# SeanChenxy/TDRN

Hardware: AMD Instinct MI355X
Metric: frames/sec/GPU @320x320 dualrefinedet_vggbn; box Linf vs CPU ref (higher is better)
Workload: dtype bf16; 1 GPU; dualrefinedet_vggbn 320x320 multihead, bf16, batch 32 per GPU, forward + Detect(top_k 200, conf 0.01, nms 0.45), synthetic VOC-shaped frames + synthetic weights; global_batch=32, parallelism=frame-sharded x1, no per-frame collective, launch=eager, resident_batches=4, steps_in_flight=2

## Files before the change

### include/tdrn_hip.h

```cpp
#ifndef TDRN_HIP_H
#define TDRN_HIP_H

#include <stddef.h>
#include <stdint.h>

#ifdef __cplusplus
extern "C" {
#endif

#define TDRN_API __attribute__((visibility("default")))

#define TDRN_OK 0
#define TDRN_E_ARG (-1)
#define TDRN_E_SHAPE (-2)
#define TDRN_E_WORKSPACE (-3)
#define TDRN_E_UNSUPPORTED (-4)
#define TDRN_E_PARAM (-5)
#define TDRN_E_STATE (-6)
#define TDRN_E_VALUE (-7)
#define TDRN_E_DEVICE (-8)

TDRN_API const char *tdrn_version(void);
TDRN_API const char *tdrn_error_string(int code);

// ... 47 lines not shown
TDRN_API int tdrn_batch_norm_backward(const float *input, const float *grad_output, const float *weight, const float *bias,
                                      const float *save_mean, const float *save_invstd, float *grad_input, float *grad_weight,
                                      float *grad_bias, int N, int C, int H, int W, int training, int relu, float scale,
                                      void *workspace, size_t workspace_bytes, void *stream);


TDRN_API size_t tdrn_nms_workspace_bytes(int n);
TDRN_API int tdrn_nms(const float *dets, int n, double thresh, int strict_gt, int32_t *keep_out,
                      int32_t *num_out, void *workspace, size_t workspace_bytes, void *stream);

TDRN_API int tdrn_nms_topk(const float *dets, int n, float overlap, float min_score, int top_k,
                           int32_t *keep_out, int32_t *num_out, void *workspace,
                           size_t workspace_bytes, void *stream);

TDRN_API size_t tdrn_nms_topk_classes_workspace_bytes(int n, int num_classes);
TDRN_API int tdrn_nms_topk_classes(const float *boxes, const float *scores, int n, int num_classes, int first_class,
                                   float overlap, float min_score, int top_k, int32_t *keep_out, int32_t *num_out,
                                   void *workspace, size_t workspace_bytes, void *stream);

TDRN_API int tdrn_roi_resample(const float *feature, int C, int H, int W, const int32_t *cells, int n, int S, float *out,
                               void *stream);
TDRN_API int tdrn_ota_similarity(const float *boxes, const float *roi, int n, int F, const float *rows, const int32_t *row_off,
                                 int m, float *best, int32_t *arg, void *stream);

TDRN_API int tdrn_gpu_nms_host(int *keep_out, int *num_out, const float *boxes_host,
                               int boxes_num, int boxes_dim, float nms_overlap_thresh,
                               int device_id);

TDRN_API int tdrn_decode(const float *loc, const float *priors, int P, float var0, float var1,
                         float *boxes_out, void *stream);
TDRN_API int tdrn_center_size(const float *boxes, int P, float *out, void *stream);

TDRN_API int tdrn_encode(const float *matched, const float *priors, int P, float var0, float var1, float *out, void *stream);
TDRN_API size_t tdrn_match_workspace_bytes(int B, int P, int max_truths);
TDRN_API int tdrn_match(const float *truths, const int32_t *truth_off, int T_total, int max_truths, int B,
                        const float *priors, int P, const float *arm_loc, float threshold, float var0, float var1,
                        float *loc_t, int32_t *conf_t, void *workspace, size_t workspace_bytes, void *stream);
TDRN_API size_t tdrn_multibox_loss_workspace_bytes(int B, int P, int C);
TDRN_API int tdrn_multibox_loss_forward(const float *loc, const float *conf, const float *loc_t, const int32_t *conf_t,
                                        int B, int P, int C, int negpos_ratio, float *loss_out, uint8_t *sel,
                                        int32_t *num_pos, void *workspace, size_t workspace_bytes, void *stream);
TDRN_API int tdrn_multibox_loss_backward(const float *loc, const float *conf, const float *loc_t, const int32_t *conf_t,
                                         const uint8_t *sel, const int32_t *num_pos, const float *grad_loss, int B,
                                         int P, int C, float *grad_loc, float *grad_conf, void *stream);

#define TDRN_AUGMENT_MAX_TRUTHS 512
#define TDRN_AUGMENT_MAX_ROUNDS 32
#define TDRN_AUGMENT_MAX_SIZE 2048
#define TDRN_AUGMENT_CROP_FALLBACK 1
#define TDRN_AUGMENT_TAPE_EXHAUSTED 2
typedef struct {
    float brightness;
    float contrast_pre;
    float contrast_post;
    float saturation;
    float hue;
    int32_t perm[3];
    int32_t canvas_w, canvas_h, img_x, img_y;
    int32_t crop_x0, crop_y0, crop_x1, crop_y1;
    int32_t cropped;
    int32_t mirror;
    int32_t kept;
    int32_t status;
} tdrn_augment_params;
typedef struct {
    const uint8_t *data;
    int32_t h, w;
} tdrn_augment_image;
TDRN_API int tdrn_augment_sample(const int32_t *hw, const double *truths, const int32_t *truth_off, int T_total, int max_truths,
                                 int B, uint64_t seed, const int64_t *sample_ids, const double *tape, const int32_t *tape_off,
                                 tdrn_augment_params *params, float *out_truths, int32_t *out_off, void *stream);
TDRN_API int tdrn_augment_apply(const tdrn_augment_image *images, const tdrn_augment_params *params, int B, const float *mean,
                                int S, int to_rgb, float *out, void *stream);

#define TDRN_AUGMENT_TRANS_FALLBACK 4
typedef struct {
    tdrn_augment_params base;
    double shift_x, shift_y;
    int32_t trans_x, trans_y;
    int32_t attempts;
    int32_t reserved;
} tdrn_augment_pair_params;
TDRN_API int tdrn_augment_pair_sample(const int32_t *hw, const double *truths, const double *truths_t, const int32_t *truth_off,
                                      int T_total, int max_truths, int B, double max_trans_ratio, uint64_t seed,
                                      const int64_t *sample_ids, const double *tape, const int32_t *tape_off,
                                      tdrn_augment_pair_params *params, float *out_truths, float *out_truths_t,
                                      int32_t *out_off, void *stream);
TDRN_API int tdrn_augment_pair_apply(const tdrn_augment_image *images, const tdrn_augment_image *images_t,
                                     const tdrn_augment_pair_params *params, int B, const float *mean, int S, int to_rgb,
                                     float *out, float *out_t, void *stream);

TDRN_API int tdrn_prior_box(int n_maps, const int *feature_maps, double image_size,
                            const double *steps, const double *min_sizes,
                            const double *max_sizes, int n_max_sizes, const int *ar_count,
                            const double *ars, int clip, int flip, float *out_host);

TDRN_API size_t tdrn_detect_workspace_bytes(int B, int P, int C, int top_k);
TDRN_API int tdrn_detect(const float *loc, const float *conf, const float *priors,
                         const float *arm_loc, const float *scale_host, int B, int P, int C,
                         int top_k, float conf_thresh, double nms_thresh, float *out,
                         int32_t *counts_out, void *workspace, size_t workspace_bytes,
                         void *stream);
TDRN_API int tdrn_detect_dev_scale(const float *loc, const float *conf, const float *priors,
                                   const float *arm_loc, const float *scale_dev, int B, int P, int C,
                                   int top_k, float conf_thresh, double nms_thresh, float *out,
                                   int32_t *counts_out, void *workspace, size_t workspace_bytes,
                                   void *stream);

TDRN_API int tdrn_preprocess(const uint8_t *frames, int B, int H0, int W0, int S, const float mean_bgr[3],
                             int to_rgb, float *out, void *stream);
TDRN_API int tdrn_preprocess_u8(const uint8_t *frames, int B, int H0, int W0, int S, int to_rgb, uint8_t *out, void *stream);

typedef enum {
    TDRN_DRN_VGGBN = 0,
    TDRN_DRN_MOBILENET = 1,
    TDRN_SSD4SCALE_MOBILE = 2,
    TDRN_REFINEDET_VGG = 3,
    TDRN_SSD4SCALE_VGG = 4
} tdrn_model;

typedef struct {
    int model;
    int size;
    int num_classes;
    int c7_channel;
    int def_groups;
    int bn;
    int multihead;
    int deform;
    int test_phase;
    int dtype;
    int use_refine;
    int plan_flags;
    int reserved[4];
} tdrn_net_config;

#define TDRN_PLAN_NO_FUSE_FIRST 1
#define TDRN_PLAN_NO_LATE_SIDE  2
#define TDRN_PLAN_ONE_STREAM    4
#define TDRN_PLAN_NO_DEFORM_TS  8
#define TDRN_PLAN_CHAIN         16
#define TDRN_PLAN_NO_CONV_PP    32
#define TDRN_PLAN_NO_PP_SK      64
#define TDRN_PLAN_NO_CONV_PATCH 128
#define TDRN_PLAN_DWPW          512
#define TDRN_PLAN_NO_PW1X1      1024
#define TDRN_PLAN_NO_DW_SLIDE   2048
#define TDRN_PLAN_DW_SLIDE_ALL  4096
#define TDRN_PLAN_NO_CONV_WS    8192
#define TDRN_PLAN_NO_YGEMM_V2  16384
#define TDRN_PLAN_NO_HEAD3X3   32768
#define TDRN_PLAN_TS_ONE_RANGE  65536
#define TDRN_PLAN_NO_PATCH_TAIL 131072
#define TDRN_PLAN_FAULT_HANDOFF 256

typedef struct tdrn_net tdrn_net;

TDRN_API int tdrn_net_create(const tdrn_net_config *cfg, tdrn_net **out);
TDRN_API void tdrn_net_destroy(tdrn_net *net);

TDRN_API int tdrn_net_param_count(const tdrn_net *net);
TDRN_API int tdrn_net_param_info(const tdrn_net *net, int index, const char **name,
                                 int64_t shape[4], int *ndim);
TDRN_API int tdrn_net_set_param(tdrn_net *net, const char *name, const float *data_host,
                                int64_t numel);

TDRN_API size_t tdrn_net_weight_bytes(const tdrn_net *net);
TDRN_API size_t tdrn_net_workspace_bytes(const tdrn_net *net, int batch);
TDRN_API int tdrn_net_num_priors(const tdrn_net *net);

TDRN_API int tdrn_net_pack_weights(tdrn_net *net, void *weights_dev, size_t weights_bytes,
                                   void *stream);
TDRN_API int tdrn_net_adopt_weights(tdrn_net *net);

typedef struct {
    const float *x;
    int batch;
    float *arm_loc;
    float *odm_loc;
    float *conf;
    float *offsets[4];
    const float *ref_loc[4];
    float *loc_maps[4];
    void *reserved[4];
} tdrn_net_io;
typedef struct {
    const uint8_t *planes;
    float mean[3];
} tdrn_u8_frames;

TDRN_API int tdrn_net_forward(tdrn_net *net, const void *weights_dev, void *workspace,
                              size_t workspace_bytes, const tdrn_net_io *io, void *stream);

TDRN_API int tdrn_net_check(tdrn_net *net, unsigned *detail);

typedef struct {
    char name[48];
    int launches;
    double flops;
    double bytes;
    double ms;
} tdrn_kernel_stat;
TDRN_API int tdrn_net_profile(tdrn_net *net, int enable);
TDRN_API int tdrn_net_kernel_stats(tdrn_net *net, tdrn_kernel_stat *out, int max_entries);
TDRN_API int tdrn_net_op_stats(tdrn_net *net, tdrn_kernel_stat *out, int max_entries);
TDRN_API int tdrn_net_op_timeline(tdrn_net *net, float *start_ms, float *end_ms, int *lane, int max_entries);

typedef struct {
    int kind;
    int in, out, res;
    int pool;
    int off, y;
    int k, stride, pad, dil, relu, ceil_mode, splitk, groups;
    int out_kind;
    int level;
    int n_branches, k2, pad2, off_c0[2];
    int y_tap_major;
    int fused_first;
    int fused_dw;
    char w[48], b[48], bn[48], w2[48], b2[48];
    int y_groups;
} tdrn_op_info;
TDRN_API int tdrn_net_op_count(const tdrn_net *net);
TDRN_API int tdrn_net_op_info(const tdrn_net *net, int index, tdrn_op_info *out);

TDRN_API int tdrn_net_tensor_count(const tdrn_net *net);
TDRN_API int tdrn_net_tensor_info(const tdrn_net *net, int index, const char **label, int *C, int *H,
                                  int *W);
TDRN_API int tdrn_net_read_tensor(const tdrn_net *net, const void *workspace, int batch, int index,
                                  float *out_dev, void *stream);
TDRN_API int tdrn_net_write_tensor(const tdrn_net *net, void *workspace, int batch, int index,
                                   const float *in_dev, void *stream);
TDRN_API int tdrn_net_forward_from(tdrn_net *net, const void *weights_dev, void *workspace,
                                   size_t workspace_bytes, const tdrn_net_io *io, int first_op, void *stream);

#ifdef __cplusplus
}
#endif
#endif
```

### tdrn_amd/_lib.py

```python
import ctypes as C
import os

_HERE = os.path.dirname(os.path.abspath(__file__))
LIB_PATH = os.environ.get("TDRN_LIB_PATH") or os.path.join(_HERE, "lib", "libtdrn_hip.so")

F32, BF16, F16 = 0, 1, 2
DTYPES = {"fp32": F32, "f32": F32, "float32": F32, "bf16": BF16, "bfloat16": BF16, "fp16": F16,
          "f16": F16, "float16": F16, "half": F16}
DRN_VGGBN, DRN_MOBILENET, SSD4SCALE_MOBILE, REFINEDET_VGG, SSD4SCALE_VGG = range(5)

E_VALUE = -7


class TdrnError(RuntimeError):
    def __init__(self, code, what=""):
        self.code = code
        super().__init__("%s (tdrn error %d)%s" % (error_string(code), code,
                                                    (": " + what) if what else ""))


class NetConfig(C.Structure):
    _fields_ = [("model", C.c_int), ("size", C.c_int), ("num_classes", C.c_int),
                ("c7_channel", C.c_int), ("def_groups", C.c_int), ("bn", C.c_int),
                ("multihead", C.c_int), ("deform", C.c_int), ("test_phase", C.c_int),
                ("dtype", C.c_int), ("use_refine", C.c_int), ("plan_flags", C.c_int), ("reserved", C.c_int * 4)]


PLAN_NO_FUSE_FIRST, PLAN_NO_LATE_SIDE, PLAN_ONE_STREAM, PLAN_NO_DEFORM_TS, PLAN_CHAIN = 1, 2, 4, 8, 16
PLAN_NO_CONV_PP, PLAN_NO_PP_SK, PLAN_NO_CONV_PATCH, PLAN_FAULT_HANDOFF, PLAN_DWPW, PLAN_NO_PW1X1 = 32, 64, 128, 256, 512, 1024
PLAN_NO_DW_SLIDE, PLAN_DW_SLIDE_ALL, PLAN_NO_CONV_WS, PLAN_NO_YGEMM_V2, PLAN_NO_HEAD3X3, PLAN_TS_ONE_RANGE = 2048, 4096, 8192, 16384, 32768, 65536
PLAN_NO_PATCH_TAIL = 131072
E_DEVICE = -8


class NetIO(C.Structure):
    _fields_ = [("x", C.c_void_p), ("batch", C.c_int), ("arm_loc", C.c_void_p),
                ("odm_loc", C.c_void_p), ("conf", C.c_void_p), ("offsets", C.c_void_p * 4),
                ("ref_loc", C.c_void_p * 4), ("loc_maps", C.c_void_p * 4),
                ("reserved", C.c_void_p * 4)]


class KernelStat(C.Structure):
    _fields_ = [("name", C.c_char * 48), ("launches", C.c_int), ("flops", C.c_double),
                ("bytes", C.c_double), ("ms", C.c_double)]


class U8FramesABI(C.Structure):
    _fields_ = [("planes", C.c_void_p), ("mean", C.c_float * 3)]


class OpInfo(C.Structure):
    _fields_ = [("kind", C.c_int), ("in_", C.c_int), ("out", C.c_int), ("res", C.c_int), ("pool", C.c_int), ("off", C.c_int),
                ("y", C.c_int), ("k", C.c_int), ("stride", C.c_int), ("pad", C.c_int), ("dil", C.c_int), ("relu", C.c_int),
                ("ceil_mode", C.c_int), ("splitk", C.c_int), ("groups", C.c_int), ("out_kind", C.c_int), ("level", C.c_int),
                ("n_branches", C.c_int), ("k2", C.c_int), ("pad2", C.c_int), ("off_c0", C.c_int * 2), ("y_tap_major", C.c_int),
                ("fused_first", C.c_int), ("fused_dw", C.c_int), ("w", C.c_char * 48), ("b", C.c_char * 48), ("bn", C.c_char * 48), ("w2", C.c_char * 48),
                ("b2", C.c_char * 48), ("y_groups", C.c_int)]


class AugmentParams(C.Structure):
    _fields_ = [("brightness", C.c_float), ("contrast_pre", C.c_float), ("contrast_post", C.c_float), ("saturation", C.c_float),
                ("hue", C.c_float), ("perm", C.c_int32 * 3), ("canvas_w", C.c_int32), ("canvas_h", C.c_int32),
                ("img_x", C.c_int32), ("img_y", C.c_int32), ("crop_x0", C.c_int32), ("crop_y0", C.c_int32),
                ("crop_x1", C.c_int32), ("crop_y1", C.c_int32), ("cropped", C.c_int32), ("mirror", C.c_int32),
                ("kept", C.c_int32), ("status", C.c_int32)]


class AugmentImage(C.Structure):
    _fields_ = [("data", C.c_void_p), ("h", C.c_int32), ("w", C.c_int32)]


class AugmentPairParams(C.Structure):
    _fields_ = [("base", AugmentParams), ("shift_x", C.c_double), ("shift_y", C.c_double), ("trans_x", C.c_int32),
                ("trans_y", C.c_int32), ("attempts", C.c_int32), ("reserved", C.c_int32)]


AUGMENT_MAX_TRUTHS, AUGMENT_MAX_SIZE = 512, 2048
AUGMENT_CROP_FALLBACK, AUGMENT_TAPE_EXHAUSTED, AUGMENT_TRANS_FALLBACK = 1, 2, 4

OP_KINDS = ("first_conv", "conv", "conv_transpose", "depthwise", "maxpool", "l2norm", "offset_conv", "deform_heads", "other")

_lib = None

_SIGS = {
    "tdrn_version": (C.c_char_p, []),
    "tdrn_error_string": (C.c_char_p, [C.c_int]),
    "tdrn_deform_conv_workspace_bytes": (C.c_size_t, [C.c_int] * 15),
    "tdrn_deform_conv_forward": (C.c_int, [C.c_void_p] * 4 + [C.c_int] * 15 + [C.c_void_p, C.c_size_t, C.c_void_p]),
    "tdrn_deform_conv_backward_workspace_bytes": (C.c_size_t, [C.c_int] * 14),
    "tdrn_deform_conv_backward_input": (C.c_int, [C.c_void_p] * 6 + [C.c_int] * 14 + [C.c_void_p, C.c_size_t, C.c_void_p]),
    "tdrn_deform_conv_backward_parameters": (C.c_int, [C.c_void_p] * 4 + [C.c_int] * 14 + [C.c_float, C.c_void_p, C.c_size_t,
                                                                                            C.c_void_p]),
    "tdrn_conv2d_workspace_bytes": (C.c_size_t, [C.c_int] * 14),
    "tdrn_conv2d_forward": (C.c_int, [C.c_void_p] * 4 + [C.c_int] * 14 + [C.c_void_p, C.c_size_t, C.c_void_p]),
    "tdrn_conv2d_backward_input": (C.c_int, [C.c_void_p] * 3 + [C.c_int] * 14 + [C.c_void_p, C.c_size_t, C.c_void_p]),
    "tdrn_conv2d_backward_parameters": (C.c_int, [C.c_void_p] * 4 + [C.c_int] * 13 + [C.c_float, C.c_int, C.c_void_p, C.c_size_t,
                                                                                       C.c_void_p]),
    "tdrn_batch_norm_workspace_bytes": (C.c_size_t, [C.c_int] * 4),
    "tdrn_batch_norm_forward": (C.c_int, [C.c_void_p] * 8 + [C.c_int] * 5 + [C.c_float, C.c_float, C.c_int, C.c_void_p, C.c_size_t,
                                                                             C.c_void_p]),
    "tdrn_batch_norm_backward": (C.c_int, [C.c_void_p] * 9 + [C.c_int] * 6 + [C.c_float, C.c_void_p, C.c_size_t, C.c_void_p]),
    "tdrn_nms_workspace_bytes": (C.c_size_t, [C.c_int]),
    "tdrn_nms": (C.c_int, [C.c_void_p, C.c_int, C.c_double, C.c_int, C.c_void_p, C.c_void_p,
                           C.c_void_p, C.c_size_t, C.c_void_p]),
    "tdrn_nms_topk": (C.c_int, [C.c_void_p, C.c_int, C.c_float, C.c_float, C.c_int, C.c_void_p, C.c_void_p,
                                C.c_void_p, C.c_size_t, C.c_void_p]),
    "tdrn_gpu_nms_host": (C.c_int, [C.c_void_p, C.c_void_p, C.c_void_p, C.c_int, C.c_int, C.c_float, C.c_int]),
    "tdrn_decode": (C.c_int, [C.c_void_p, C.c_void_p, C.c_int, C.c_float, C.c_float, C.c_void_p, C.c_void_p]),
    "tdrn_center_size": (C.c_int, [C.c_void_p, C.c_int, C.c_void_p, C.c_void_p]),
    "tdrn_encode": (C.c_int, [C.c_void_p, C.c_void_p, C.c_int, C.c_float, C.c_float, C.c_void_p, C.c_void_p]),
    "tdrn_match_workspace_bytes": (C.c_size_t, [C.c_int] * 3),
    "tdrn_match": (C.c_int, [C.c_void_p, C.c_void_p, C.c_int, C.c_int, C.c_int, C.c_void_p, C.c_int, C.c_void_p, C.c_float,
                             C.c_float, C.c_float, C.c_void_p, C.c_void_p, C.c_void_p, C.c_size_t, C.c_void_p]),
    "tdrn_multibox_loss_workspace_bytes": (C.c_size_t, [C.c_int] * 3),
    "tdrn_multibox_loss_forward": (C.c_int, [C.c_void_p] * 4 + [C.c_int] * 4 + [C.c_void_p] * 4 + [C.c_size_t, C.c_void_p]),
    "tdrn_multibox_loss_backward": (C.c_int, [C.c_void_p] * 7 + [C.c_int] * 3 + [C.c_void_p] * 3),
    "tdrn_augment_sample": (C.c_int, [C.c_void_p] * 3 + [C.c_int] * 3 + [C.c_uint64] + [C.c_void_p] * 7),
    "tdrn_augment_apply": (C.c_int, [C.c_void_p, C.c_void_p, C.c_int, C.c_void_p, C.c_int, C.c_int, C.c_void_p, C.c_void_p]),
    "tdrn_augment_pair_sample": (C.c_int, [C.c_void_p] * 4 + [C.c_int] * 3 + [C.c_double, C.c_uint64] + [C.c_void_p] * 8),
    "tdrn_augment_pair_apply": (C.c_int, [C.c_void_p] * 3 + [C.c_int, C.c_void_p, C.c_int, C.c_int] + [C.c_void_p] * 3),
    "tdrn_prior_box": (C.c_int, [C.c_int, C.c_void_p, C.c_double, C.c_void_p, C.c_void_p, C.c_void_p,
                                 C.c_int, C.c_void_p, C.c_void_p, C.c_int, C.c_int, C.c_void_p]),
    "tdrn_nms_topk_classes_workspace_bytes": (C.c_size_t, [C.c_int, C.c_int]),
    "tdrn_nms_topk_classes": (C.c_int, [C.c_void_p, C.c_void_p, C.c_int, C.c_int, C.c_int, C.c_float, C.c_float, C.c_int, C.c_void_p,
                                        C.c_void_p, C.c_void_p, C.c_size_t, C.c_void_p]),
    "tdrn_roi_resample": (C.c_int, [C.c_void_p, C.c_int, C.c_int, C.c_int, C.c_void_p, C.c_int, C.c_int, C.c_void_p, C.c_void_p]),
    "tdrn_ota_similarity": (C.c_int, [C.c_void_p, C.c_void_p, C.c_int, C.c_int, C.c_void_p, C.c_void_p, C.c_int, C.c_void_p, C.c_void_p,
                                      C.c_void_p]),
    "tdrn_preprocess": (C.c_int, [C.c_void_p, C.c_int, C.c_int, C.c_int, C.c_int, C.c_void_p, C.c_int, C.c_void_p, C.c_void_p]),
    "tdrn_preprocess_u8": (C.c_int, [C.c_void_p, C.c_int, C.c_int, C.c_int, C.c_int, C.c_int, C.c_void_p, C.c_void_p]),
    "tdrn_detect_workspace_bytes": (C.c_size_t, [C.c_int] * 4),
    "tdrn_detect": (C.c_int, [C.c_void_p] * 5 + [C.c_int] * 4 + [C.c_float, C.c_double, C.c_void_p,
                                                                  C.c_void_p, C.c_void_p, C.c_size_t, C.c_void_p]),
    "tdrn_detect_dev_scale": (C.c_int, [C.c_void_p] * 5 + [C.c_int] * 4 + [C.c_float, C.c_double, C.c_void_p,
                                                                            C.c_void_p, C.c_void_p, C.c_size_t, C.c_void_p]),
    "tdrn_net_create": (C.c_int, [C.POINTER(NetConfig), C.POINTER(C.c_void_p)]),
    "tdrn_net_destroy": (None, [C.c_void_p]),
    "tdrn_net_param_count": (C.c_int, [C.c_void_p]),
    "tdrn_net_param_info": (C.c_int, [C.c_void_p, C.c_int, C.POINTER(C.c_char_p), C.POINTER(C.c_int64 * 4),
                                      C.POINTER(C.c_int)]),
    "tdrn_net_set_param": (C.c_int, [C.c_void_p, C.c_char_p, C.c_void_p, C.c_int64]),
    "tdrn_net_weight_bytes": (C.c_size_t, [C.c_void_p]),
    "tdrn_net_workspace_bytes": (C.c_size_t, [C.c_void_p, C.c_int]),
    "tdrn_net_num_priors": (C.c_int, [C.c_void_p]),
    "tdrn_net_pack_weights": (C.c_int, [C.c_void_p, C.c_void_p, C.c_size_t, C.c_void_p]),
    "tdrn_net_adopt_weights": (C.c_int, [C.c_void_p]),
    "tdrn_net_forward": (C.c_int, [C.c_void_p, C.c_void_p, C.c_void_p, C.c_size_t, C.POINTER(NetIO), C.c_void_p]),
    "tdrn_net_check": (C.c_int, [C.c_void_p, C.POINTER(C.c_uint)]),
    "tdrn_net_op_count": (C.c_int, [C.c_void_p]),
    "tdrn_net_op_info": (C.c_int, [C.c_void_p, C.c_int, C.POINTER(OpInfo)]),
    "tdrn_net_tensor_count": (C.c_int, [C.c_void_p]),
    "tdrn_net_tensor_info": (C.c_int, [C.c_void_p, C.c_int, C.POINTER(C.c_char_p), C.POINTER(C.c_int),
                                       C.POINTER(C.c_int), C.POINTER(C.c_int)]),
    "tdrn_net_read_tensor": (C.c_int, [C.c_void_p, C.c_void_p, C.c_int, C.c_int, C.c_void_p, C.c_void_p]),
    "tdrn_net_write_tensor": (C.c_int, [C.c_void_p, C.c_void_p, C.c_int, C.c_int, C.c_void_p, C.c_void_p]),
    "tdrn_net_forward_from": (C.c_int, [C.c_void_p, C.c_void_p, C.c_void_p, C.c_size_t, C.POINTER(NetIO), C.c_int, C.c_void_p]),
    "tdrn_net_profile": (C.c_int, [C.c_void_p, C.c_int]),
    "tdrn_net_kernel_stats": (C.c_int, [C.c_void_p, C.POINTER(KernelStat), C.c_int]),
    "tdrn_net_op_stats": (C.c_int, [C.c_void_p, C.POINTER(KernelStat), C.c_int]),
    "tdrn_net_op_timeline": (C.c_int, [C.c_void_p, C.POINTER(C.c_float), C.POINTER(C.c_float), C.POINTER(C.c_int), C.c_int]),
}
EXPORTS = tuple(_SIGS)


def lib():
    global _lib
    if _lib is None:
        if not os.path.exists(LIB_PATH):
            raise ImportError(
                "libtdrn_hip.so is missing (%s): build it with `python -c 'import __graft_entry__ as g; "
                "g.build()'` or `make -C tdrn_amd/csrc`.  tdrn_amd has no CPU fallback." % LIB_PATH)
        try:
            import torch
            if torch.cuda.is_available():
                torch.cuda.init()
        except ImportError:
            pass
        l = C.CDLL(LIB_PATH)
        for name, (res, args) in _SIGS.items():
            fn = getattr(l, name)
            fn.restype = res
            fn.argtypes = args
        _lib = l
    return _lib


def error_string(code):
    try:
        return lib().tdrn_error_string(int(code)).decode()
    except Exception:
        return "tdrn error"


def check(rc, what=""):
    if rc != 0:
        if rc == E_VALUE:
            raise ValueError("nms_threshold must be non negative.")
        raise TdrnError(rc, what)


def ptr(t):
    return None if t is None else C.c_void_p(t.data_ptr())


def aligned16(t):
    return t if t is None or t.data_ptr() % 16 == 0 else t.clone()


def current_stream(device=None):
    import torch
    return C.c_void_p(torch.cuda.current_stream(device).cuda_stream)


def require_cuda(t, name="tensor"):
    if not t.is_cuda:
        raise NotImplementedError(
            "%s must live on the GPU: tdrn_amd runs only through libtdrn_hip.so on an MI355X "
            "(no CPU path; the reference's ConvOffset2dFunction raises here too, "
            "model/networks.py:632-633)" % name)
```

### tdrn_amd/csrc/common.h

```cpp
#pragma once
#include <hip/hip_runtime.h>
#include <stdint.h>

#include "../../include/tdrn_hip.h"

#include <cstdlib>

namespace tdrn {

inline int dev_ablate_env(const char *name)
{
#ifdef TDRN_DEV_ABLATE
    const char *e = getenv(name);
    return e ? atoi(e) : 0;
#else
    (void)name;
    return 0;
#endif
}

typedef __attribute__((ext_vector_type(4))) float f32x4;
typedef __attribute__((ext_vector_type(16))) float f32x16;
typedef __attribute__((ext_vector_type(8))) short i16x8;
typedef __attribute__((ext_vector_type(8))) _Float16 f16x8;
typedef __attribute__((ext_vector_type(4))) int i32x4;
typedef __attribute__((ext_vector_type(4))) unsigned u32x4;

struct bf16_t { unsigned short v; };
struct f16_t { unsigned short v; };

template <typename T> struct elem_traits;
template <> struct elem_traits<float> { static constexpr int bytes = 4; static constexpr int per16 = 4; };
template <> struct elem_traits<bf16_t> { static constexpr int bytes = 2; static constexpr int per16 = 8; };
template <> struct elem_traits<f16_t> { static constexpr int bytes = 2; static constexpr int per16 = 8; };

__device__ __forceinline__ float bf16_to_f32(unsigned short h) { return __uint_as_float(((unsigned)h) << 16); }
__device__ __forceinline__ unsigned short f32_to_bf16(float f)
{
    __bf16 b = (__bf16)f;
    return __builtin_bit_cast(unsigned short, b);
}
__device__ __forceinline__ float f16_to_f32(unsigned short h) { return (float)__builtin_bit_cast(_Float16, h); }
__device__ __forceinline__ unsigned short f32_to_f16(float f) { return __builtin_bit_cast(unsigned short, (_Float16)f); }

template <typename T> __device__ __forceinline__ float to_f32(const T &);
template <> __device__ __forceinline__ float to_f32<float>(const float &x) { return x; }
template <> __device__ __forceinline__ float to_f32<bf16_t>(const bf16_t &x) { return bf16_to_f32(x.v); }
template <> __device__ __forceinline__ float to_f32<f16_t>(const f16_t &x) { return f16_to_f32(x.v); }
template <typename T> __device__ __forceinline__ T from_f32(float);
template <> __device__ __forceinline__ float from_f32<float>(float x) { return x; }
template <> __device__ __forceinline__ bf16_t from_f32<bf16_t>(float x) { return bf16_t{f32_to_bf16(x)}; }
template <> __device__ __forceinline__ f16_t from_f32<f16_t>(float x) { return f16_t{f32_to_f16(x)}; }

template <typename T> __device__ __forceinline__ void unpack16(const u32x4 &raw, float *out);
template <> __device__ __forceinline__ void unpack16<float>(const u32x4 &raw, float *out)
{
#pragma unroll
    for (int i = 0; i < 4; ++i) out[i] = __uint_as_float(raw[i]);
}
template <> __device__ __forceinline__ void unpack16<bf16_t>(const u32x4 &raw, float *out)
{
#pragma unroll
    for (int i = 0; i < 4; ++i) {
        out[2 * i] = __uint_as_float(raw[i] << 16);
        out[2 * i + 1] = __uint_as_float(raw[i] & 0xffff0000u);
    }
}
template <> __device__ __forceinline__ void unpack16<f16_t>(const u32x4 &raw, float *out)
{
#pragma unroll
    for (int i = 0; i < 4; ++i) {
        out[2 * i] = f16_to_f32((unsigned short)(raw[i] & 0xffffu));
        out[2 * i + 1] = f16_to_f32((unsigned short)(raw[i] >> 16));
    }
}
template <typename T> __device__ __forceinline__ u32x4 pack16(const float *in);
template <> __device__ __forceinline__ u32x4 pack16<float>(const float *in)
{
    u32x4 r;
#pragma unroll
    for (int i = 0; i < 4; ++i) r[i] = __float_as_uint(in[i]);
    return r;
}
__device__ __forceinline__ unsigned pack2_bf16(float a, float b)
{
    typedef __bf16 bf2 __attribute__((ext_vector_type(2)));
    typedef float fl2 __attribute__((ext_vector_type(2)));
    return __builtin_bit_cast(unsigned, __builtin_convertvector(fl2{a, b}, bf2));
}
__device__ __forceinline__ unsigned pack2_f16(float a, float b)
{
    typedef _Float16 h2 __attribute__((ext_vector_type(2)));
    typedef float fl2 __attribute__((ext_vector_type(2)));
    return __builtin_bit_cast(unsigned, __builtin_convertvector(fl2{a, b}, h2));
}
template <typename T> __device__ __forceinline__ unsigned pack2(float a, float b);
template <> __device__ __forceinline__ unsigned pack2<bf16_t>(float a, float b) { return pack2_bf16(a, b); }
template <> __device__ __forceinline__ unsigned pack2<f16_t>(float a, float b) { return pack2_f16(a, b); }
template <> __device__ __forceinline__ u32x4 pack16<bf16_t>(const float *in)
{
    u32x4 r;
#pragma unroll
    for (int i = 0; i < 4; ++i) r[i] = pack2_bf16(in[2 * i], in[2 * i + 1]);
    return r;
}
template <> __device__ __forceinline__ u32x4 pack16<f16_t>(const float *in)
{
    u32x4 r;
#pragma unroll
    for (int i = 0; i < 4; ++i) r[i] = pack2_f16(in[2 * i], in[2 * i + 1]);
    return r;
}

inline int hip_status(hipError_t e) { return e == hipSuccess ? TDRN_OK : (int)e; }
#define TDRN_HIP_TRY(expr)                                   \
    do {                                                     \
        hipError_t _e = (expr);                              \
        if (_e != hipSuccess) return (int)_e;                \
    } while (0)
#define TDRN_TRY(expr)                                       \
    do {                                                     \
        int _s = (expr);                                     \
        if (_s != TDRN_OK) return _s;                        \
    } while (0)

inline size_t align_up(size_t v, size_t a) { return (v + a - 1) / a * a; }
inline int cdiv(int a, int b) { return (a + b - 1) / b; }
inline int dtype_bytes(int dt) { return dt == TDRN_F32 ? 4 : 2; }

unsigned short host_f32_to_bf16(float f);
unsigned short host_f32_to_f16(float f);

}
```

### tdrn_amd/csrc/deform.hip

```cpp
#include <algorithm>

#include "deform_sampler.h"
#include "kernels.h"
#include "mfma_prims.h"

namespace tdrn {

struct DeformBranchP {
    const float *off;
    const char *w;
    int off_stride, kh, kw, G;
    int pad_h, pad_w, stride_h, stride_w, dil_h, dil_w;
    int off_rows, off_row0;
};
struct DeformParams {
    const char *in, *zero;
    DeformBranchP br[2];
    int n_branches;
    int M, H, W, Cin, Ho, Wo, Cout, Npad, split;
    float *out0, *out1;
    long long o0_bs, o0_ps, o1_bs, o1_ps;
    int accumulate;
    int g_begin, g_end;
};
// ... 171 lines not shown
    auto compute = [&](int buf) {
        const char *wsb = smem + buf * STAGE;
        const char *psb = wsb + BN * 128;
#pragma unroll
        for (int kk = 0; kk < 4; ++kk) {
            const int ch = ((2 * kk + hh) ^ sw) << 4;
            const u32x4 pf = *(const u32x4 *)(psb + (wave * 32 + r32) * 128 + ch);
#pragma unroll
            for (int ci = 0; ci < NTL; ++ci) {
                const u32x4 wf = *(const u32x4 *)(wsb + (ci * 32 + r32) * 128 + ch);
                Mma32<DT>::run(wf, pf, acc[ci]);
            }
        }
    };

    fetch_offsets(0, 0, 0, p.g_begin);
    tap_params();
    issue(0);
    latch_weights();
    finish(0);
    asm volatile("s_waitcnt vmcnt(0)" ::: "memory");
    __syncthreads();
    int cur = 0;
    bool more = true;
    while (more) {
        more = advance();
        if (more) {
            issue(cur ^ 1);
            latch_weights();
        }
        compute(cur);
        if (more) finish(cur ^ 1);
        asm volatile("s_waitcnt vmcnt(0)" ::: "memory");
        __syncthreads();
        cur ^= 1;
    }

#pragma unroll
    for (int ci = 0; ci < NTL; ++ci)
#pragma unroll
        for (int q = 0; q < 4; ++q) {
            f32x4 v;
#pragma unroll
            for (int j = 0; j < 4; ++j) v[j] = acc[ci][4 * q + j];
            *(f32x4 *)(smem + (wave * 32 + r32) * CS + (ci * 32 + 8 * q + 4 * hh) * 4) = v;
        }
    __syncthreads();
    for (int idx = t; idx < BM * p.Cout; idx += NT) {
        const int row = idx / p.Cout, c = idx - row * p.Cout;
        const int m = m0 + row;
        if (m >= p.M) break;
        const int b = m / HoWo, pix = m - b * HoWo;
        const float v = *(const float *)(smem + row * CS + c * 4);
        float *dst = c < p.split ? p.out0 + b * p.o0_bs + pix * p.o0_ps + c : p.out1 + b * p.o1_bs + pix * p.o1_ps + (c - p.split);
        if (p.accumulate) atomicAdd(dst, v);
        else *dst = v;
    }
}

int deform_n_pad(int cout) { return (int)align_up((size_t)cout, 32); }

template <typename DT> static int launch_deform_dt(const DeformMulti &mp, int ntl, hipStream_t s)
{
    dim3 grid((unsigned)(8 * ((mp.block_start[mp.n] + 7) / 8)));
    switch (ntl) {
        case 1: hipLaunchKernelGGL((deform_gemm_kernel<DT, 1>), grid, dim3(256), 0, s, mp); break;
        case 2: hipLaunchKernelGGL((deform_gemm_kernel<DT, 2>), grid, dim3(256), 0, s, mp); break;
        case 3: hipLaunchKernelGGL((deform_gemm_kernel<DT, 3>), grid, dim3(256), 0, s, mp); break;
        case 4: hipLaunchKernelGGL((deform_gemm_kernel<DT, 4>), grid, dim3(256), 0, s, mp); break;
        default: return TDRN_E_UNSUPPORTED;
    }
    return hip_status(hipGetLastError());
}

static int fill_params(const DeformArgs &a, DeformParams &p)
{
    if (!a.in || !a.out0 || a.n_branches < 1 || a.n_branches > 2) return TDRN_E_ARG;
    const int es = dtype_bytes(a.dtype), ck = 128 / es;
    if (a.Npad % 32 || a.Npad > 128 || a.Cout > a.Npad || a.Cout < 1) return TDRN_E_UNSUPPORTED;
    if (a.split < a.Cout && !a.out1) return TDRN_E_ARG;
    if ((long long)a.B * a.H * a.W * a.Cin * es >= (1ll << 32)) return TDRN_E_UNSUPPORTED;
    p.in = (const char *)a.in;
    p.zero = (const char *)a.zero_page;
    p.n_branches = a.n_branches;
    for (int i = 0; i < a.n_branches; ++i) {
        const DeformBranch &b = a.br[i];
        if (!b.off || !b.w || b.G < 1 || a.Cin % b.G || (a.Cin / b.G) % ck) return TDRN_E_UNSUPPORTED;
        if (b.kh < 1 || b.kw < 1 || b.stride < 1 || b.dil < 1) return TDRN_E_SHAPE;
        p.br[i] = DeformBranchP{b.off, (const char *)b.w, b.off_stride, b.kh, b.kw, b.G,
                                b.pad, b.pad_w < 0 ? b.pad : b.pad_w, b.stride, b.stride_w < 1 ? b.stride : b.stride_w,
                                b.dil, b.dil_w < 1 ? b.dil : b.dil_w, b.off_rows, b.off_row0};
        if (b.off_rows < 0 || b.off_row0 < 0) return TDRN_E_ARG;
    }
    if (a.n_branches == 1) p.br[1] = p.br[0];
    p.M = a.B * a.Ho * a.Wo;
    p.H = a.H; p.W = a.W; p.Cin = a.Cin; p.Ho = a.Ho; p.Wo = a.Wo; p.Cout = a.Cout; p.Npad = a.Npad;
    p.split = a.split > a.Cout ? a.Cout : a.split;
    p.out0 = a.out0; p.out1 = a.out1;
    p.o0_bs = a.o0_bs; p.o0_ps = a.o0_ps; p.o1_bs = a.o1_bs; p.o1_ps = a.o1_ps;
    return TDRN_OK;
}

int launch_deform_multi(const DeformArgs *args, int n, hipStream_t s, int split_branches)
{
    if (!args || n < 1 || n > 4) return TDRN_E_ARG;
    DeformMulti mp;
    mp.n = 0;
    mp.block_start[0] = 0;
    for (int pass = 0; pass < 2; ++pass) {
        for (int i = 0; i < n; ++i) {
            if (args[i].dtype != args[0].dtype || args[i].Npad != args[0].Npad) return TDRN_E_UNSUPPORTED;
            DeformArgs a = args[i];
            const bool two = a.n_branches == 2 && split_branches == 1;
            const bool halves = split_branches == 2 && a.n_branches == 1 && a.br[0].G >= 2 && a.br[0].G % 2 == 0;
            if (!two && !halves && pass == 1) continue;
            if (two) {
                const int t0 = a.br[0].kh * a.br[0].kw, t1 = a.br[1].kh * a.br[1].kw;
                const int longer = t1 > t0 ? 1 : 0;
                a.br[0] = args[i].br[pass == 0 ? longer : 1 - longer];
                a.n_branches = 1;
            }
            DeformParams p;
            TDRN_TRY(fill_params(a, p));
            p.accumulate = (two || halves) ? 1 : 0;
            p.g_begin = 0;
            p.g_end = a.br[0].G;
            if (halves) {
                p.g_begin = pass == 0 ? 0 : a.br[0].G / 2;
                p.g_end = pass == 0 ? a.br[0].G / 2 : a.br[0].G;
            }
            if (p.M <= 0) continue;
            if (mp.n >= kMaxDeformProblems) return TDRN_E_UNSUPPORTED;
            mp.p[mp.n] = p;
            mp.block_start[mp.n + 1] = mp.block_start[mp.n] + cdiv(p.M, 128);
            ++mp.n;
        }
    }
    if (mp.n == 0) return TDRN_OK;
    for (int i = mp.n; i < kMaxDeformProblems; ++i) { mp.p[i] = mp.p[0]; mp.block_start[i + 1] = mp.block_start[mp.n]; }
    switch (args[0].dtype) {
        case TDRN_F32: return launch_deform_dt<float>(mp, args[0].Npad / 32, s);
        case TDRN_BF16: return launch_deform_dt<bf16_t>(mp, args[0].Npad / 32, s);
        case TDRN_F16: return launch_deform_dt<f16_t>(mp, args[0].Npad / 32, s);
    }
    return TDRN_E_ARG;
}

int launch_deform(const DeformArgs &a, hipStream_t s) { return launch_deform_multi(&a, 1, s, 0); }

struct SampleBranchP {
    const float *off;
    int off_stride, kh, kw, pad_h, pad_w, dil_h, dil_w, col0;
    int off_rows, off_row0;
};
struct SampleParams {
    const char *y;
    SampleBranchP br[2];
    int n_branches, n_taps;
    int M, H, W, ycs, Cout, split;
    int tap_major;
    float *out0, *out1;
    long long o0_bs, o0_ps, o1_bs, o1_ps;
};
struct SampleMulti {
    SampleParams p[4];
    int block_start[5];
    int n;
};
constexpr int kSampleCols = 80;

template <typename DT>
__global__ __launch_bounds__(256) void deform_sample_kernel(const SampleMulti mp)
{
    const int nblk = (int)gridDim.x, xq = nblk >> 3, xr = nblk & 7, xcd = (int)blockIdx.x & 7;
    const int blk = (xcd < xr ? xcd * (xq + 1) : xr * (xq + 1) + (xcd - xr) * xq) + ((int)blockIdx.x >> 3);
    int prob = 0;
#pragma unroll
    for (int i = 1; i < 4; ++i)
        if (i < mp.n && blk >= mp.block_start[i]) prob = i;
    const SampleParams &p = mp.p[prob];
    constexpr int MAXR = 34 * 4;
    __shared__ uint2 s_ow[4][MAXR + 8];
    __shared__ float s_red[4][6][kSampleCols];
    const int lane = threadIdx.x & 63, wave = threadIdx.x >> 6;
    const int m = (blk - mp.block_start[prob]) * 4 + wave;
    if (m >= p.M) return;
    const int HW = p.H * p.W;
    const int b = m / HW, rem = m - b * HW, ho = rem / p.W, wo = rem - ho * p.W;
    const int nrows = p.n_taps * 4;
    if (lane < p.n_taps) {
        const int brn = (p.n_branches == 2 && lane >= p.br[0].kh * p.br[0].kw) ? 1 : 0;
        const SampleBranchP &B = p.br[brn];
        const int tl = lane - (brn ? p.br[0].kh * p.br[0].kw : 0);
        const int ti = tl / B.kw, tj = tl - ti * B.kw;
        const int orow = B.off_rows ? (m + B.off_row0) % B.off_rows : m;
        const float *op = B.off + (size_t)orow * B.off_stride + 2 * tl;
        const float offset_h = op[0], offset_w = op[1];
        float w1 = 0.f, w2 = 0.f, w3 = 0.f, w4 = 0.f;
        int q1 = 0, q2 = 0, q3 = 0, q4 = 0;
        const int h_in = ho - B.pad_h, w_in = wo - B.pad_w;
        const float h_im = (float)(h_in + ti * B.dil_h) + offset_h;
        const float w_im = (float)(w_in + tj * B.dil_w) + offset_w;
        if (h_im >= 0.f && w_im >= 0.f && h_im < (float)p.H && w_im < (float)p.W) {
            float h = (float)(ti * B.dil_h) + offset_h;
            float w = (float)(tj * B.dil_w) + offset_w;
            const int height = p.H - h_in, width = p.W - w_in;
            int h_low = (int)floorf(h), w_low = (int)floorf(w), h_high, w_high;
            if (h_low >= height - 1) { h_high = h_low = height - 1; h = (float)h_low; } else { h_high = h_low + 1; }
            if (w_low >= width - 1) { w_high = w_low = width - 1; w = (float)w_low; } else { w_high = w_low + 1; }
            const float lh = h - (float)h_low, lw = w - (float)w_low;
            const float hh = 1.f - lh, hw = 1.f - lw;
            w1 = hh * hw; w2 = hh * lw; w3 = lh * hw; w4 = lh * lw;
            const int r0 = min(max(h_in + h_low, 0), p.H - 1), r1 = min(max(h_in + h_high, 0), p.H - 1);
            const int c0 = min(max(w_in + w_low, 0), p.W - 1), c1 = min(max(w_in + w_high, 0), p.W - 1);
            q1 = r0 * p.W + c0; q2 = r0 * p.W + c1; q3 = r1 * p.W + c0; q4 = r1 * p.W + c1;
        }
        const unsigned colb = p.tap_major ? (unsigned)(B.col0 + tl) * (unsigned)p.M * (unsigned)(kSampleCols * 2) : (unsigned)(deform_y_col(B.col0 + tl) * 2);
        const unsigned rowb = p.tap_major ? (unsigned)(kSampleCols * 2) : (unsigned)(p.ycs * 2);
        const unsigned img = (unsigned)(b * HW);
        s_ow[wave][4 * lane + 0] = make_uint2((img + q1) * rowb + colb, __float_as_uint(w1));
        s_ow[wave][4 * lane + 1] = make_uint2((img + q2) * rowb + colb, __float_as_uint(w2));
        s_ow[wave][4 * lane + 2] = make_uint2((img + q3) * rowb + colb, __float_as_uint(w3));
        s_ow[wave][4 * lane + 3] = make_uint2((img + q4) * rowb + colb, __float_as_uint(w4));
        if (lane == p.n_taps - 1)
            for (int r = nrows; r < 36 * ((nrows + 35) / 36); ++r) s_ow[wave][r] = make_uint2((img + q4) * rowb + colb, 0u);
    }
    __builtin_amdgcn_s_waitcnt(0xC07F);
    __builtin_amdgcn_wave_barrier();
    const int j = lane / 10, c = lane - 10 * j;
    float acc[8] = {0.f, 0.f, 0.f, 0.f, 0.f, 0.f, 0.f, 0.f};
    if (lane < 60) {
        const int nb = (nrows + 35) / 36;
        const __attribute__((address_space(1))) char *yb = (const __attribute__((address_space(1))) char *)p.y;
        for (int ib = 0; ib < nb; ++ib) {
            u32x4 raw[6];
            float wgt[6];
#pragma unroll
            for (int u = 0; u < 6; ++u) {
                const uint2 ow = s_ow[wave][6 * (6 * ib + u) + j];
                wgt[u] = __uint_as_float(ow.y);
                raw[u] = *(const __attribute__((address_space(1))) u32x4 *)(yb + (ow.x + (unsigned)(c * 16)));
            }
#pragma unroll
            for (int u = 0; u < 6; ++u) {
                float v[8];
                unpack16<DT>(raw[u], v);
#pragma unroll
                for (int e = 0; e < 8; ++e) acc[e] = fmaf(wgt[u], v[e], acc[e]);
            }
        }
#pragma unroll
        for (int e = 0; e < 8; ++e) s_red[wave][j][c * 8 + e] = acc[e];
    }
    __builtin_amdgcn_s_waitcnt(0xC07F);
    __builtin_amdgcn_wave_barrier();
    for (int co = lane; co < p.Cout; co += 64) {
        float v = s_red[wave][0][co];
#pragma unroll
        for (int jj = 1; jj < 6; ++jj) v += s_red[wave][jj][co];
        float *dst = co < p.split ? p.out0 + b * p.o0_bs + rem * p.o0_ps + co : p.out1 + b * p.o1_bs + rem * p.o1_ps + (co - p.split);
        *dst = v;
    }
}

struct YGemmParams {
    const char *x;
    const char *w;
    char *y;
    int M, N, ycs, parts, tiles_per_part, taps;
};

struct YGemmMulti {
    YGemmParams p[4];
    int block_start[5];
    int n;
#ifdef TDRN_YG_STAMP
    unsigned *stamps;
#endif
};
#ifdef TDRN_YG_STAMP
#define YG_STAMP_DECL unsigned long long st_t = __builtin_amdgcn_s_memtime(); unsigned st_acc[6] = {0, 0, 0, 0, 0, 0};
#define YG_STAMP(k) do { const unsigned long long t_ = __builtin_amdgcn_s_memtime(); st_acc[k] += (unsigned)(t_ - st_t); st_t = t_; } while (0)
#define YG_STAMP_FLUSH do { st_acc[5] = (unsigned)nt; if (lane == 0) for (int k_ = 0; k_ < 6; ++k_) mp.stamps[((size_t)blockIdx.x * 8 + wave) * 6 + k_] = st_acc[k_]; } while (0)
#else
#define YG_STAMP_DECL
#define YG_STAMP(k) do { } while (0)
#define YG_STAMP_FLUSH do { } while (0)
#endif

template <typename DT>
__global__ __launch_bounds__(512, 4) void ygemm_k256_kernel(const YGemmMulti mp)
{
    int prob = 0;
#pragma unroll
    for (int i = 1; i < 4; ++i)
        if (i < mp.n && (int)blockIdx.x >= mp.block_start[i]) prob = i;
    const YGemmParams &p = mp.p[prob];
    const int local_blk = (int)blockIdx.x - mp.block_start[prob];
    const int ncg = p.N / 256;
    constexpr int NW = 8;
    constexpr int NT = NW * 64;
    constexpr int TP = 32;
    constexpr int TBYTES = TP * 512;
    constexpr int SROW = 512 + 16;
    constexpr int PPW = 16 / NW;
    __shared__ __attribute__((aligned(16))) char smem[2 * TBYTES];
    __shared__ __attribute__((aligned(16))) char sst[TP * SROW];
    const int lane = threadIdx.x & 63, wave = __builtin_amdgcn_readfirstlane(threadIdx.x >> 6);
    const int r32 = lane & 31, hh = lane >> 5;
    const int part = local_blk / ncg, cg = local_blk - part * ncg;
    const int col0 = cg * 256 + wave * 32;
    u32x4 wf[16];
    {
        const char *wr = p.w + ((size_t)(col0 + r32) * 256 + 8 * hh) * 2;
#pragma unroll
        for (int kk = 0; kk < 16; ++kk) wf[kk] = *(const u32x4 *)(wr + kk * 32);
    }
    const int t0 = part * p.tiles_per_part;
    int nt = (p.M + TP - 1) / TP - t0;
    nt = nt < p.tiles_per_part ? nt : p.tiles_per_part;
    if (nt <= 0) return;
    YG_STAMP_DECL

    const unsigned smem_lds = lds_addr(smem);
    auto stage = [&](int t, int buf) {
        const long long mb = (long long)(t0 + t) * TP;
        const char *sb = p.x + (size_t)mb * 512;
#pragma unroll
        for (int j = 0; j < PPW; ++j) {
            const int piece = PPW * wave + j;
            const int row = 2 * piece + (lane >> 5), cpos = lane & 31;
            int r = row;
            if (mb + r >= p.M) r = (int)(p.M - 1 - mb);
            const unsigned voff = (unsigned)(r * 512 + ((cpos ^ (row & 31)) << 4));
            lds_dma16(sb, voff, __builtin_amdgcn_readfirstlane(smem_lds + buf * TBYTES + piece * 1024));
        }
    };
    stage(0, 0);
    YG_STAMP(0);
    constexpr int NSTR = 32 * 32 / NT;
    int nst_prev = NSTR;
    if (p.taps > 0) {
        nst_prev = 0;
        for (int it = wave; it < 18; it += NW) nst_prev += (cg * 3 + it / 6) < p.taps ? 1 : 0;
    }
    for (int t = 0; t < nt; ++t) {
        const int buf = t & 1;
        if (t + 1 < nt) {
            stage(t + 1, buf ^ 1);
            switch ((t == 0 ? 0 : nst_prev) + PPW) {
                case 2: asm volatile("s_waitcnt vmcnt(2)" ::: "memory"); break;
                case 3: asm volatile("s_waitcnt vmcnt(3)" ::: "memory"); break;
                case 4: asm volatile("s_waitcnt vmcnt(4)" ::: "memory"); break;
                case 5: asm volatile("s_waitcnt vmcnt(5)" ::: "memory"); break;
                case 6: asm volatile("s_waitcnt vmcnt(6)" ::: "memory"); break;
                case 7: asm volatile("s_waitcnt vmcnt(7)" ::: "memory"); break;
                case 8: asm volatile("s_waitcnt vmcnt(8)" ::: "memory"); break;
                default: asm volatile("s_waitcnt vmcnt(9)" ::: "memory"); break;
            }
        } else {
            asm volatile("s_waitcnt vmcnt(0)" ::: "memory");
        }
        YG_STAMP(1);
        __builtin_amdgcn_s_barrier();
        asm volatile("" ::: "memory");
        YG_STAMP(2);
        f32x16 acc;
#pragma unroll
        for (int e = 0; e < 16; ++e) acc[e] = 0.f;
        const char *ab = smem + buf * TBYTES + r32 * 512;
#pragma unroll
        for (int kk = 0; kk < 16; ++kk) {
            const u32x4 a = *(const u32x4 *)(ab + (((2 * kk + hh) ^ r32) << 4));
            Mma32<DT>::run(wf[kk], a, acc);
        }
        {
            const unsigned sa = (unsigned)(unsigned long long)(__attribute__((address_space(3))) char *)sst + (unsigned)(r32 * SROW + (wave * 32 + 4 * hh) * 2);
#pragma unroll
            for (int g = 0; g < 4; ++g) {
                const uint2 v = make_uint2(pack2<DT>(acc[4 * g], acc[4 * g + 1]), pack2<DT>(acc[4 * g + 2], acc[4 * g + 3]));
                asm volatile("ds_write_b64 %0, %1 offset:%2" ::"v"(sa), "v"(v), "n"(16 * g) : "memory");
            }
        }
        asm volatile("s_waitcnt lgkmcnt(0)" ::: "memory");
        __builtin_amdgcn_s_waitcnt(0xC07F);
        YG_STAMP(3);
        __builtin_amdgcn_s_barrier();
        asm volatile("" ::: "memory");
        YG_STAMP(2);
        if (p.taps > 0) {
            const int px = lane / 10, k = lane - 10 * px;
            for (int it = wave; it < 18; it += NW) {
                const int sgi = it / 6, pg = it - sgi * 6;
                const int tap = cg * 3 + sgi;
                const int row = pg * 6 + px;
                const long long m = (long long)(t0 + t) * TP + row;
                if (lane < 60 && row < TP && tap < p.taps && m < p.M)
                    *(u32x4 *)(p.y + ((size_t)tap * p.M + (size_t)m) * 160 + k * 16) = *(const u32x4 *)(sst + row * SROW + (sgi * 10 + k) * 16);
            }
        } else {
#pragma unroll
            for (int q = 0; q < NSTR; ++q) {
                const int row = (threadIdx.x >> 5) + (NT / 32) * q, ch = threadIdx.x & 31;
                const long long m = (long long)(t0 + t) * TP + row;
                if (m < p.M) *(u32x4 *)(p.y + ((size_t)m * p.ycs + cg * 256) * 2 + ch * 16) = *(const u32x4 *)(sst + row * SROW + ch * 16);
            }
        }
        YG_STAMP(4);
    }
    YG_STAMP_FLUSH;
}

template <typename DT>
__global__ __launch_bounds__(512, 4) void ygemm_k256_v2_kernel(const YGemmMulti mp)
// ... 101 lines not shown
            if (kk == 5 || kk == 10 || kk == 15) carry_store((kk - 5) / 5, rows_prev, sv);
            __builtin_amdgcn_sched_barrier(0);
        }
        {
            const unsigned sa = (unsigned)(unsigned long long)(__attribute__((address_space(3))) char *)sst + (unsigned)(buf * SBYTES) + sw;
#pragma unroll
            for (int g = 0; g < 4; ++g) {
                const uint2 v = make_uint2(pack2<DT>(acc[4 * g], acc[4 * g + 1]), pack2<DT>(acc[4 * g + 2], acc[4 * g + 3]));
                asm volatile("ds_write_b64 %0, %1 offset:%2" ::"v"(sa), "v"(v), "n"(16 * g) : "memory");
            }
        }
        YG_STAMP(3);
        if (t + 1 < nt) {
            switch (t > 0 ? nst : 0) {
                case 0: asm volatile("s_waitcnt vmcnt(0) lgkmcnt(0)" ::: "memory"); break;
                case 1: asm volatile("s_waitcnt vmcnt(1) lgkmcnt(0)" ::: "memory"); break;
                case 2: asm volatile("s_waitcnt vmcnt(2) lgkmcnt(0)" ::: "memory"); break;
                default: asm volatile("s_waitcnt vmcnt(3) lgkmcnt(0)" ::: "memory"); break;
            }
        } else {
            asm volatile("s_waitcnt lgkmcnt(0)" ::: "memory");
        }
        YG_STAMP(4);
        __builtin_amdgcn_s_barrier();
        asm volatile("" ::: "memory");
        YG_STAMP(2);
    }
    {
        const int left = p.M - (t0 + nt - 1) * TP;
        const int rows = left < TP ? left : TP;
#pragma unroll
        for (int j = 0; j < 3; ++j) {
            const u32x4 v = carry_read(j, (nt - 1) & 1);
            carry_store(j, rows, v);
        }
    }
    YG_STAMP_FLUSH;
}

int ygemm_supported(int Cin, int ycols, int dtype) { return dtype != TDRN_F32 && Cin == 256 && ycols % 256 == 0; }

static int ygemm_fill(const YGemmProblem &q, int dtype, YGemmParams &p, int &blocks)
{
    if (!ygemm_supported(256, q.N, dtype) || q.M <= 0 || q.M >= (1ll << 31)) return TDRN_E_UNSUPPORTED;
    p.x = (const char *)q.x; p.w = (const char *)q.w; p.y = (char *)q.y;
    p.M = (int)q.M; p.N = q.N; p.ycs = q.ycs; p.taps = q.taps;
    if (q.taps > 0 && (deform_sample_cols(q.taps) > q.N || (long long)q.taps * q.M * 160 >= (1ll << 32))) return TDRN_E_UNSUPPORTED;
    const int tiles = (int)((q.M + 31) / 32), cgs = q.N / 256;
    const int kSlots = 512, max_parts = (tiles + 7) / 8 > 1 ? (tiles + 7) / 8 : 1;
    int parts = 1;
    long long best = -1;
    for (int r = 1; r <= 3; ++r) {
        int c = kSlots * r / cgs;
        c = c > max_parts ? max_parts : (c < 1 ? 1 : c);
        const long long rounds = ((long long)cgs * c + kSlots - 1) / kSlots, cost = rounds * ((tiles + c - 1) / c);
        if (best < 0 || cost < best) { best = cost; parts = c; }
    }
    p.parts = parts;
    p.tiles_per_part = (tiles + parts - 1) / parts;
    blocks = cgs * parts;
    return TDRN_OK;
}

int launch_ygemm_multi(const YGemmProblem *pr, int n, int dtype, hipStream_t s, int kdisable)
{
    if (!pr || n < 1 || n > 4) return TDRN_E_ARG;
    YGemmMulti mp;
    mp.n = 0;
    mp.block_start[0] = 0;
    int order[4] = {0, 1, 2, 3};
    for (int i = 0; i < n; ++i)
        for (int j = i + 1; j < n; ++j)
            if (pr[order[j]].M > pr[order[i]].M) { const int t = order[i]; order[i] = order[j]; order[j] = t; }
    for (int i = 0; i < n; ++i) {
        if (pr[order[i]].M <= 0) continue;
        int blocks = 0;
        TDRN_TRY(ygemm_fill(pr[order[i]], dtype, mp.p[mp.n], blocks));
        mp.block_start[mp.n + 1] = mp.block_start[mp.n] + blocks;
        ++mp.n;
    }
    if (mp.n == 0) return TDRN_OK;
    for (int i = mp.n; i < 4; ++i) { mp.p[i] = mp.p[0]; mp.block_start[i + 1] = mp.block_start[mp.n]; }
    dim3 grid((unsigned)mp.block_start[mp.n]);
#ifdef TDRN_YG_STAMP
    static unsigned *stamps = nullptr;
    static int calls = 0;
    const size_t nst = (size_t)grid.x * 8 * 6;
    if (!stamps) TDRN_HIP_TRY(hipMalloc((void **)&stamps, 4096 * 8 * 6 * sizeof(unsigned)));
    TDRN_HIP_TRY(hipMemsetAsync(stamps, 0, nst * sizeof(unsigned), s));
    mp.stamps = stamps;
    struct Report {
        hipStream_t s; size_t n; unsigned *d; YGemmMulti &mp; int *calls;
        ~Report() {
            if (++*calls != 5) return;
            (void)hipStreamSynchronize(s);
            std::vector<unsigned> h(n);
            (void)hipMemcpy(h.data(), d, n * sizeof(unsigned), hipMemcpyDeviceToHost);
            for (int pr = 0; pr < mp.n; ++pr) {
                double a[5] = {0, 0, 0, 0, 0}, tiles = 0, waves = 0;
                for (int b = mp.block_start[pr]; b < mp.block_start[pr + 1]; ++b)
                    for (int w = 0; w < 8; ++w) {
                        const unsigned *q = &h[((size_t)b * 8 + w) * 6];
                        if (!q[5]) continue;
                        for (int k = 0; k < 5; ++k) a[k] += q[k];
                        tiles += q[5]; waves += 1;
                    }
                if (waves == 0) continue;
                fprintf(stderr, "yg_stamp problem %d M %d blocks %d tiles/wg %.1f | per wave: prologue %.0f | per tile: landing %.0f barriers %.0f mma+stage %.0f stores %.0f (ticks of s_memtime)\n",
                        pr, mp.p[pr].M, mp.block_start[pr + 1] - mp.block_start[pr], tiles / waves, a[0] / waves, a[1] / tiles, a[2] / tiles, a[3] / tiles, a[4] / tiles);
            }
        }
    } report{s, nst, stamps, mp, &calls};
#endif
    bool tapmajor = true;
    for (int i = 0; i < mp.n; ++i) tapmajor = tapmajor && mp.p[i].taps > 0;
    if (!(kdisable & KOFF_YGEMM_V2) && tapmajor) {
        if (dtype == TDRN_BF16) hipLaunchKernelGGL((ygemm_k256_v2_kernel<bf16_t>), grid, dim3(512), 0, s, mp);
        else hipLaunchKernelGGL((ygemm_k256_v2_kernel<f16_t>), grid, dim3(512), 0, s, mp);
    } else {
        if (dtype == TDRN_BF16) hipLaunchKernelGGL((ygemm_k256_kernel<bf16_t>), grid, dim3(512), 0, s, mp);
        else hipLaunchKernelGGL((ygemm_k256_kernel<f16_t>), grid, dim3(512), 0, s, mp);
    }
    return hip_status(hipGetLastError());
}

int launch_ygemm(const void *x, const void *w, void *y, long long M, int N, int ycs, int dtype, hipStream_t s, int taps)
{
    const YGemmProblem q{x, w, y, M, N, ycs, taps};
    return launch_ygemm_multi(&q, 1, dtype, s);
}

int deform_sample_supported(const DeformArgs &a)
{
    if (a.dtype == TDRN_F32 || a.n_branches < 1 || a.n_branches > 2 || a.Cout > kSampleCols || a.Ho != a.H || a.Wo != a.W) return 0;
    int taps = 0;
    for (int i = 0; i < a.n_branches; ++i) {
        const DeformBranch &b = a.br[i];
        if (b.G != 1 || b.stride != 1 || (b.stride_w >= 1 && b.stride_w != 1)) return 0;
        taps += b.kh * b.kw;
    }
    return taps <= 34 ? taps : 0;
}
int deform_sample_cols(int taps) { return ((taps + 2) / 3) * 256; }
int deform_ts_max_batch(int H, int W, int ycs, int taps)
{
    const long long hw = (long long)H * W;
    const long long per = std::max((long long)taps * 160, (long long)ycs * 2) * hw;
    long long b = ((1ll << 32) - 1) / per;
    const long long bm = ((1ll << 31) - 1) / hw;
    b = b < bm ? b : bm;
    return (int)(b > (1 << 20) ? (1 << 20) : b);
}

int launch_deform_sample_multi(const DeformArgs *args, const void *const *y, const int *ycs, int n, hipStream_t s, int tap_major)
{
    if (!args || n < 1 || n > 4) return TDRN_E_ARG;
    SampleMulti mp;
    mp.n = 0;
    mp.block_start[0] = 0;
    for (int i = 0; i < n; ++i) {
        const DeformArgs &a = args[i];
        const int taps = deform_sample_supported(a);
        if (!taps || a.dtype != args[0].dtype) return TDRN_E_UNSUPPORTED;
        if ((long long)a.B * a.H * a.W * ycs[i] * 2 >= (1ll << 32)) return TDRN_E_UNSUPPORTED;
        SampleParams p;
        p.y = (const char *)y[i];
        p.n_branches = a.n_branches; p.n_taps = taps;
        int col0 = 0;
        for (int k = 0; k < a.n_branches; ++k) {
            const DeformBranch &b = a.br[k];
            p.br[k] = SampleBranchP{b.off, b.off_stride, b.kh, b.kw, b.pad, b.pad_w < 0 ? b.pad : b.pad_w, b.dil, b.dil_w < 1 ? b.dil : b.dil_w, col0, b.off_rows, b.off_row0};
            col0 += b.kh * b.kw;
        }
        if (a.n_branches == 1) p.br[1] = p.br[0];
        p.M = a.B * a.H * a.W; p.H = a.H; p.W = a.W; p.ycs = ycs[i]; p.Cout = a.Cout; p.tap_major = tap_major;
        p.split = a.split > a.Cout ? a.Cout : a.split;
        p.out0 = a.out0; p.out1 = a.out1;
        p.o0_bs = a.o0_bs; p.o0_ps = a.o0_ps; p.o1_bs = a.o1_bs; p.o1_ps = a.o1_ps;
        if (p.M <= 0) continue;
        mp.p[mp.n] = p;
        mp.block_start[mp.n + 1] = mp.block_start[mp.n] + cdiv(p.M, 4);
        ++mp.n;
    }
    if (mp.n == 0) return TDRN_OK;
    for (int i = mp.n; i < 4; ++i) { mp.p[i] = mp.p[0]; mp.block_start[i + 1] = mp.block_start[mp.n]; }
    dim3 grid((unsigned)mp.block_start[mp.n]);
    if (args[0].dtype == TDRN_BF16) hipLaunchKernelGGL((deform_sample_kernel<bf16_t>), grid, dim3(256), 0, s, mp);
    else hipLaunchKernelGGL((deform_sample_kernel<f16_t>), grid, dim3(256), 0, s, mp);
    return hip_status(hipGetLastError());
}

}
```

### tdrn_amd/csrc/kernels.h

```cpp
#pragma once
#include <cmath>

#include "common.h"

namespace tdrn {

constexpr size_t kZeroPageBytes = 256;

int allow_big_lds(const void *kernel);

enum KernelOff {
    KOFF_CONV_PP = 1,
    KOFF_PP_SK = 2,
    KOFF_CONV_PATCH = 4,
    KOFF_PW1X1 = 8,
    KOFF_DW_SLIDE = 16,
    KOFF_DW_STRIP_SMALL = 32,
    KOFF_CONV_WS = 64,
    KOFF_YGEMM_V2 = 128,
    KOFF_HEAD3X3 = 256,
    KOFF_TS_RANGES = 512,
    KOFF_PATCH_TAIL = 1024,
};

struct ConvArgs {
    const void *in = nullptr, *w = nullptr, *res = nullptr, *zero_page = nullptr;
    const float *bias = nullptr;
    void *out = nullptr;
    int B = 0, H = 0, W = 0, Cin = 0;
    int Ho = 0, Wo = 0, Cout = 0, Npad = 0;
    int kh = 1, kw = 1, stride = 1, pad = 0, dil = 1;
    int relu = 0, out_f32 = 0, phases = 1;
    int splitk = 1;
    void *partial = nullptr;
    long long o_bs = 0, o_rs = 0, o_cs = 0, o_base = 0, o_pr = 0, o_pc = 0;
    int dtype = TDRN_BF16;
    const float *fuse_x = nullptr, *fuse_w = nullptr, *fuse_b = nullptr;
    int fuse_cout = 0;
    const unsigned char *fuse_x8 = nullptr;
    float fuse_mean[3] = {0.f, 0.f, 0.f};
    void *sk_ws = nullptr;
    bool sk_flags_zero = false;
    int kdisable = 0;
    unsigned *status = nullptr;
    int fault_handoff = 0;
};
enum ConvKernel { CONV_IGEMM, CONV_PATCH, CONV_PP, CONV_WS, CONV_HEAD3X3, CONV_PW1X1, CONV_NONE };
ConvKernel conv_route(const ConvArgs &a, bool pooled);
const char *conv_kernel_name(ConvKernel k);
int launch_conv(const ConvArgs &a, hipStream_t s, void *out_pool = nullptr);
int conv_splitk_choice(const ConvArgs &a);
int launch_conv_igemm(const ConvArgs &a, hipStream_t s);
int igemm_splitk_choice(const ConvArgs &a);
size_t conv_splitk_bytes(const ConvArgs &a, int splits);
struct ChainLayer { ConvArgs a; int dep[2] = {-1, -1}; };
int conv_chain_supported(const ConvArgs &a);
int conv_chain_max_layers();
size_t conv_chain_ctr_bytes();
int launch_conv_chain(const ChainLayer *layers, int n, unsigned *ctr, hipStream_t s, unsigned *status = nullptr);
bool head3x3_takes(const ConvArgs &a, bool pooled);
int launch_head3x3(const ConvArgs &a, hipStream_t s);
inline int conv3x3_tile_mode(const ConvArgs &a, int slots)
{
    if (a.kh != 3 || a.kw != 3 || a.stride != 1 || a.pad != 1 || a.dil != 1 || a.phases != 1 || a.out_f32 || a.res) return 0;
    if (a.Ho != a.H || a.Wo != a.W || a.Npad % 64) return 0;
    if (a.o_rs != (long long)a.Wo * a.o_cs || a.o_bs != (long long)a.Ho * a.Wo * a.o_cs || a.o_base) return 0;
    if (a.W % 32 == 0 && a.H % 8 == 0) return 32;
    if (a.W % 16 == 0 && a.H % 16 == 0) return 16;
    return 2 * a.W + 2 + 256 <= slots * 8 ? -1 : 0;
}
inline bool conv3x3_input_fits(const ConvArgs &a) { return a.fuse_x || (long long)a.B * a.H * a.W * a.Cin * dtype_bytes(a.dtype) < (1ll << 32); }
bool patch_takes(const ConvArgs &a, bool pooled);
int launch_conv3x3_patch(const ConvArgs &a, void *out_pool, hipStream_t s);
bool pp_takes_geometry(const ConvArgs &a);
bool pp_takes(const ConvArgs &a, bool pooled);
int launch_conv3x3_pp(const ConvArgs &a, hipStream_t s);
size_t conv_pp_sk_bytes();
bool ws_takes(const ConvArgs &a, bool pooled);
int launch_conv3x3_ws(const ConvArgs &a, void *out_pool, hipStream_t s);
inline int persistent_grid(int items) { return items >= 256 ? 256 : ((items + 7) / 8) * 8; }
inline void conv_tiles(int B, int H, int W, int tw, int px, int &tiles_x, int &tiles_per_img, int &m_tiles)
{
    tiles_x = tw ? W / tw : 0;
    tiles_per_img = tw ? tiles_x * (H / (px / tw)) : 0;
    m_tiles = tw ? B * tiles_per_img : cdiv(B * H * W, 256);
}
int conv_n_pad(int cout);
constexpr int kChanPad = 64;

int launch_first_conv(const float *x, const float *w, const float *bias, void *out, int B, int S,
                      int stride, int Cout, int Cpad, int relu, int dtype, hipStream_t s);
int launch_maxpool2(const void *in, void *out, int B, int H, int W, int C, int ceil_mode, int dtype,
                    hipStream_t s);
int launch_l2norm(const void *in, const float *w, void *out, long long pixels, int C, int dtype,
                  hipStream_t s);
int launch_dwconv3(const void *in, const float *w, const float *bias, void *out, int B, int H, int W,
                   int C, int stride, int relu, int dtype, hipStream_t s, int kdisable = 0);
struct DwPwArgs {
    const void *in = nullptr, *w = nullptr;
    const float *wdw = nullptr, *bdw = nullptr, *bias = nullptr;
    void *out = nullptr;
    int B = 0, H = 0, W = 0, Cin = 0, Cout = 0, Npad = 0, Cs = 0;
    int stride = 1, relu_dw = 1, relu = 1, dtype = TDRN_BF16;
};
int dwpw_supported(const DwPwArgs &a);
int launch_dwpw(const DwPwArgs &a, hipStream_t s);
bool pw1x1_takes(const ConvArgs &a, bool pooled);
int launch_pw1x1(const ConvArgs &a, hipStream_t s);
int launch_softmax_rows(const float *in, float *out, long long R, int C, hipStream_t s);
int launch_offset_conv(const float *loc, long long loc_bs, long long loc_ps, const float *w,
                       const float *bias, float *off, int B, int HW, int n_in, int n_out,
                       hipStream_t s);
struct OffsetProblem { const float *loc; long long loc_bs, loc_ps; const float *w, *bias; float *off; int B, HW, n_out, blk0; };
struct OffsetMulti { OffsetProblem pr[4]; int n; };
int launch_offset_conv_multi(const OffsetProblem *pr, int n, hipStream_t s);
int launch_nchw_to_nhwc(const float *in, void *out, int B, int C, int HW, int Cpad, int dtype,
                        hipStream_t s);
int launch_nchw_to_nhwc_grouped(const float *in, void *out, int B, int C, int HW, int G, int cpg_pad, int dtype,
                                hipStream_t s);
int launch_repack_oihw(const float *w, void *out, int Cout, int Npad, int Cin, int taps, int G, int cpg_pad, int dtype,
                       hipStream_t s);
int launch_nhwc_to_nchw_f32(const float *in, long long in_bs, long long in_ps, float *out, int B,
                            int C, int HW, hipStream_t s);
int launch_nhwc_any_to_nchw_f32(const void *in, int dtype, int Cpad, float *out, int B, int C, int HW, hipStream_t s);
int launch_preprocess(const unsigned char *in, int B, int H0, int W0, int S, const float *mean_bgr, int to_rgb, float *out,
                      hipStream_t s);
int launch_preprocess_u8(const unsigned char *in, int B, int H0, int W0, int S, int to_rgb, unsigned char *out, hipStream_t s);
int launch_u8_planes_to_f32(const unsigned char *in, int B, int S, const float *mean, float *out, hipStream_t s);
int launch_fill_zero(void *p, size_t bytes, hipStream_t s);

struct DeformBranch {
    const float *off = nullptr;
    int off_stride = 0;
    const void *w = nullptr;
    int kh = 3, kw = 3, pad = 1, stride = 1, dil = 1, G = 1;
    int pad_w = -1, stride_w = -1, dil_w = -1;
    int off_rows = 0, off_row0 = 0;
};
struct DeformArgs {
    const void *in = nullptr, *zero_page = nullptr;
    DeformBranch br[2];
    int n_branches = 1;
    int B = 0, H = 0, W = 0, Cin = 0, Ho = 0, Wo = 0, Cout = 0, Npad = 0;
    float *out0 = nullptr, *out1 = nullptr;
    int split = 0;
    long long o0_bs = 0, o0_ps = 0, o1_bs = 0, o1_ps = 0;
    int dtype = TDRN_BF16;
};
int launch_deform(const DeformArgs &a, hipStream_t s);
int launch_deform_multi(const DeformArgs *args, int n, hipStream_t s, int split_branches);
int deform_n_pad(int cout);
struct DeformBwdGeom { int N, Cin, H, W, Cout, kh, kw, sh, sw, ph, pw, dh, dw, G, Ho, Wo; };
int deform_bwd_cpg64(const DeformBwdGeom &g);
int deform_bwd_data_px(const DeformBwdGeom &g);
int launch_deform_bwd_data(const DeformBwdGeom &g, const float *in_nhwc, const float *off, const float *gout, const float *wr,
                           float *gin_nhwc, float *goff, hipStream_t s);
int launch_deform_bwd_input_add(const DeformBwdGeom &g, const float *gin_nhwc, float *grad_input, hipStream_t s);
void deform_bwd_weight_splits(const DeformBwdGeom &g, int &splits, int &per_split);
int launch_deform_bwd_weight(const DeformBwdGeom &g, const float *in_nhwc, const float *off, const float *gout, float *slab, float *grad_weight,
                             float scale, hipStream_t s);
struct ConvBwdGeom { int N, Cin, H, W, Cout, k, pad, dil, Ho, Wo; };
int conv_bwd_cpad(int c);
void conv_wgrad_splits(const ConvBwdGeom &g, int &splits, int &per_split);
size_t conv_wgrad_slab_bytes(const ConvBwdGeom &g);
int launch_conv_wgrad(const ConvBwdGeom &g, const void *x_nhwc, const void *go_nhwc, const void *zero_page, void *slab, float *grad_weight,
                      float *grad_bias, float scale, int dtype, hipStream_t s);
int launch_repack_oihw_dgrad(const float *w, void *out, int Cout, int Cin, int Npad, int taps, int dtype, hipStream_t s);
void batch_norm_splits(int N, int C, int HW, int &splits, int &per_split);
size_t batch_norm_workspace_bytes(int N, int C, int HW);
int launch_batch_norm_forward(const float *input, const float *weight, const float *bias, float *running_mean, float *running_var,
                              float *output, float *save_mean, float *save_invstd, int N, int C, int HW, int training, float momentum,
                              float eps, int relu, void *ws, hipStream_t s);
int launch_batch_norm_backward(const float *input, const float *grad_output, const float *weight, const float *bias, const float *save_mean,
                               const float *save_invstd, float *grad_input, float *grad_weight, float *grad_bias, int N, int C, int HW,
                               int training, int relu, float scale, void *ws, hipStream_t s);
int deform_sample_supported(const DeformArgs &a);
int deform_sample_cols(int taps);
constexpr int deform_y_col(int tap) { return (tap / 3) * 256 + (tap % 3) * 80; }
int deform_ts_max_batch(int H, int W, int ycs, int taps);
int launch_deform_sample_multi(const DeformArgs *args, const void *const *y, const int *ycs, int n, hipStream_t s, int tap_major = 0);
int ygemm_supported(int Cin, int ycols, int dtype);
int launch_ygemm(const void *x, const void *w, void *y, long long M, int N, int ycs, int dtype, hipStream_t s, int taps = 0);
struct YGemmProblem { const void *x, *w; void *y; long long M; int N, ycs, taps; };
int launch_ygemm_multi(const YGemmProblem *pr, int n, int dtype, hipStream_t s, int kdisable = 0);

int launch_decode(const float *loc, const float *priors, int P, float v0, float v1, float *out,
                  hipStream_t s);
int launch_center_size(const float *boxes, int P, float *out, hipStream_t s);
size_t detect_workspace_bytes(int B, int P, int C, int top_k);
int launch_detect(const float *loc, const float *conf, const float *priors, const float *arm_loc,
                  const float *scale4, int scale_on_device, int B, int P, int C, int top_k, float conf_thresh,
                  double nms_thresh, float *out, int32_t *counts, void *ws, size_t ws_bytes,
                  hipStream_t s);
size_t nms_workspace_bytes(int n);
size_t nms_classes_workspace_bytes(int n, int C);
int launch_roi_resample(const float *feat, int C, int H, int W, const int32_t *cells, int n, int S, float *out, hipStream_t s);
int launch_ota_similarity(const float *boxes, const float *roi, int n, int F, const float *rows, const int32_t *row_off, int m, float *best,
                          int32_t *arg, hipStream_t s);
int launch_nms_classes(const float *boxes, const float *scores, int n, int C, int first_class, float overlap, float min_score, int top_k,
                       int32_t *keep_out, int32_t *num_out, void *ws, size_t ws_bytes, hipStream_t s);
int launch_nms(const float *dets, int n, double thresh, int strict_gt, int presorted,
               int32_t *keep_out, int32_t *num_out, void *ws, size_t ws_bytes, hipStream_t s,
               int plain_rule = 0, float min_score = -INFINITY, int pre_top_k = 0);

constexpr int kMaxMatchTruths = 512;
constexpr int kMaxLossClasses = 1024;
size_t match_workspace_bytes(int B, int P, int max_truths);
int launch_match(const float *truths, const int32_t *truth_off, int T_total, int max_truths, int B, const float *priors, int P,
                 const float *arm_loc, float threshold, float var0, float var1, float *loc_t, int32_t *conf_t, void *ws,
                 size_t ws_bytes, hipStream_t s);
int launch_encode(const float *matched, const float *priors, int P, float v0, float v1, float *out, hipStream_t s);
size_t multibox_loss_workspace_bytes(int B, int P, int C);
int launch_multibox_loss_forward(const float *loc, const float *conf, const float *loc_t, const int32_t *conf_t, int B, int P,
                                 int C, int negpos_ratio, float *loss_out, uint8_t *sel, int32_t *num_pos, void *ws,
                                 size_t ws_bytes, hipStream_t s);
int launch_multibox_loss_backward(const float *loc, const float *conf, const float *loc_t, const int32_t *conf_t,
                                  const uint8_t *sel, const int32_t *num_pos, const float *grad_loss, int B, int P, int C,
                                  float *grad_loc, float *grad_conf, hipStream_t s);

int launch_augment_sample(const int32_t *hw, const double *truths, const int32_t *truth_off, int T_total, int max_truths, int B,
                          uint64_t seed, const int64_t *sample_ids, const double *tape, const int32_t *tape_off,
                          tdrn_augment_params *params, float *out_truths, int32_t *out_off, hipStream_t s);
int launch_augment_apply(const tdrn_augment_image *images, const tdrn_augment_params *params, int B, const float *mean, int S,
                         int to_rgb, float *out, hipStream_t s);

int launch_augment_pair_sample(const int32_t *hw, const double *truths, const double *truths_t, const int32_t *truth_off,
                               int T_total, int max_truths, int B, double max_trans_ratio, uint64_t seed,
                               const int64_t *sample_ids, const double *tape, const int32_t *tape_off,
                               tdrn_augment_pair_params *params, float *out_truths, float *out_truths_t, int32_t *out_off,
                               hipStream_t s);
int launch_augment_pair_apply(const tdrn_augment_image *images, const tdrn_augment_image *images_t,
                              const tdrn_augment_pair_params *params, int B, const float *mean, int S, int to_rgb, float *out,
                              float *out_t, hipStream_t s);

}
```

### tdrn_amd/csrc/layers.hip

```cpp
#include <atomic>
#include <type_traits>

#include "kernels.h"

namespace tdrn {

template <typename DT>
__global__ __launch_bounds__(256) void first_conv_kernel(const float *__restrict__ x, const float *__restrict__ w,
                                                         const float *__restrict__ bias, char *__restrict__ out,
                                                         int B, int S, int So, int stride, int Cout, int Cpad, int relu)
{
    constexpr int P16 = elem_traits<DT>::per16;
    constexpr int ES = elem_traits<DT>::bytes;
    __shared__ __attribute__((aligned(16))) char tile[256 * (64 * ES + 16)];
    constexpr int TS = 64 * ES + 16;
    const long long total = (long long)B * So * So;
    const long long pix0 = (long long)blockIdx.x * 256;
    const long long pix = pix0 + threadIdx.x;
    const bool live = pix < total;
    float v[27];
    if (live) {
        const int b = (int)(pix / (So * So));
        const int rem = (int)(pix - (long long)b * So * So);
        const int ho = rem / So, wo = rem - ho * So;
// ... 447 lines not shown
    constexpr int NCOL = (TW - 1) * STRIDE + 3;
    const int cpr = C / P16;
    const int wg = (Wo + TW - 1) / TW;
    const long long total = (long long)B * nseg * wg * cpr;
    const long long i = (long long)blockIdx.x * blockDim.x + threadIdx.x;
    if (i >= total) return;
    const int ch = (int)(i % cpr);
    long long r = i / cpr;
    const int sg = (int)(r % wg);
    r /= wg;
    const int seg = (int)(r % nseg);
    const int b = (int)(r / nseg);
    float wt[9][P16], bs[P16];
#pragma unroll
    for (int t = 0; t < 9; ++t)
#pragma unroll
        for (int j = 0; j < P16; ++j) wt[t][j] = w[(size_t)t * C + ch * P16 + j];
#pragma unroll
    for (int j = 0; j < P16; ++j) bs[j] = bias[ch * P16 + j];
    const int wo0 = sg * TW;
    const int ho0 = seg * TH, ho1 = ho0 + TH < Ho ? ho0 + TH : Ho;
    const char *colp = in + ((size_t)b * H * W) * C * ES + (size_t)ch * 16;
    struct Row { u32x4 v[NCOL]; };
    auto load_row = [&](int hi) -> Row {
        Row q;
        const bool rok = (unsigned)hi < (unsigned)H;
        const char *rowp = colp + (size_t)(rok ? hi : 0) * W * C * ES;
#pragma unroll
        for (int c = 0; c < NCOL; ++c) {
            const int wi = wo0 * STRIDE - 1 + c;
            q.v[c] = (rok && (unsigned)wi < (unsigned)W) ? *(const u32x4 *)(rowp + (size_t)wi * C * ES) : u32x4{0u, 0u, 0u, 0u};
        }
        return q;
    };
    float acc[TW][P16];
    auto add_row = [&](const Row &q, int rr, int hi) {
        if ((unsigned)hi >= (unsigned)H) return;
#pragma unroll
        for (int c = 0; c < NCOL; ++c) {
            float v[P16];
            unpack16<DT>(q.v[c], v);
#pragma unroll
            for (int o = 0; o < TW; ++o) {
                const int t = c - o * STRIDE;
                if (t >= 0 && t < 3) {
#pragma unroll
                    for (int j = 0; j < P16; ++j) acc[o][j] = fmaf(wt[rr * 3 + t][j], v[j], acc[o][j]);
                }
            }
        }
    };
    auto finish = [&](int ho) {
#pragma unroll
        for (int o = 0; o < TW; ++o) {
            if (wo0 + o >= Wo) break;
            if (relu) {
#pragma unroll
                for (int j = 0; j < P16; ++j) acc[o][j] = fmaxf(acc[o][j], 0.f);
            }
            *(u32x4 *)(out + ((((size_t)b * Ho + ho) * Wo + wo0 + o) * C + (size_t)ch * P16) * ES) = pack16<DT>(acc[o]);
        }
    };
    auto start = [&]() {
#pragma unroll
        for (int o = 0; o < TW; ++o)
#pragma unroll
            for (int j = 0; j < P16; ++j) acc[o][j] = bs[j];
    };
    if (STRIDE == 1) {
        Row ra = load_row(ho0 - 1), rb = load_row(ho0), rc = load_row(ho0 + 1);
#pragma unroll 1
        for (int ho = ho0; ho < ho1; ++ho) {
            start();
            add_row(ra, 0, ho - 1);
            ra = load_row(ho + 2 < ho1 + 1 ? ho + 2 : -1);
            add_row(rb, 1, ho);
            add_row(rc, 2, ho + 1);
            finish(ho);
            const Row t = rb;
            rb = rc; rc = ra; ra = t;
        }
    } else {
        Row ra = load_row(2 * ho0 - 1), rb = load_row(2 * ho0), rc = load_row(2 * ho0 + 1);
#pragma unroll 1
        for (int ho = ho0; ho < ho1; ++ho) {
            const bool more = ho + 1 < ho1;
            Row nb = load_row(more ? 2 * ho + 2 : -1), nc = load_row(more ? 2 * ho + 3 : -1);
            start();
            add_row(ra, 0, 2 * ho - 1);
            add_row(rb, 1, 2 * ho);
            add_row(rc, 2, 2 * ho + 1);
            finish(ho);
            ra = rc; rb = nb; rc = nc;
        }
    }
}

int launch_dwconv3(const void *in, const float *w, const float *bias, void *out, int B, int H, int W, int C,
                   int stride, int relu, int dtype, hipStream_t s, int kdisable)
{
    const int Ho = (H + 2 - 3) / stride + 1, Wo = (W + 2 - 3) / stride + 1;
    const int per16 = 16 / dtype_bytes(dtype);
    if (C % per16) return TDRN_E_UNSUPPORTED;
    if (!(kdisable & KOFF_DW_SLIDE) && (stride == 1 || stride == 2) && Wo >= 4) {
        const int tw = stride == 1 ? 4 : 2;
        const long long per_row = (long long)B * ((Wo + tw - 1) / tw) * (C / per16);
        int th = 0;
        for (int t = 8; t >= 2 && !th; t >>= 1)
            if (per_row * ((Ho + t - 1) / t) >= 768ll * 256) th = t;
        if (kdisable & KOFF_DW_STRIP_SMALL) th = 8;
        if (th) {
            const int nseg = (Ho + th - 1) / th;
            dim3 grid((unsigned)((per_row * nseg + 255) / 256));
#define LD(DT)                                                                                                                          \
    do {                                                                                                                                \
        if (stride == 1) hipLaunchKernelGGL((dwconv3_slide_kernel<DT, 1, 4>), grid, dim3(256), 0, s, (const char *)in, w, bias, (char *)out, B, H, W, Ho, Wo, C, relu, th, nseg); \
        else hipLaunchKernelGGL((dwconv3_slide_kernel<DT, 2, 2>), grid, dim3(256), 0, s, (const char *)in, w, bias, (char *)out, B, H, W, Ho, Wo, C, relu, th, nseg);             \
    } while (0)
            if (dtype == TDRN_F32) LD(float); else if (dtype == TDRN_BF16) LD(bf16_t); else LD(f16_t);
#undef LD
            return hip_status(hipGetLastError());
        }
    }
    if ((stride == 1 || stride == 2) && Wo >= 4) {
        const long long total = (long long)B * Ho * ((Wo + 3) / 4) * (C / per16);
        dim3 grid((unsigned)((total + 255) / 256 > 8192 ? 8192 : (total + 255) / 256));
#define LS(DT)                                                                                                                         \
    do {                                                                                                                               \
        if (stride == 1) hipLaunchKernelGGL((dwconv3_strip_kernel<DT, 1>), grid, dim3(256), 0, s, (const char *)in, w, bias, (char *)out, B, H, W, Ho, Wo, C, relu); \
        else hipLaunchKernelGGL((dwconv3_strip_kernel<DT, 2>), grid, dim3(256), 0, s, (const char *)in, w, bias, (char *)out, B, H, W, Ho, Wo, C, relu);             \
    } while (0)
        if (dtype == TDRN_F32) LS(float); else if (dtype == TDRN_BF16) LS(bf16_t); else LS(f16_t);
#undef LS
        return hip_status(hipGetLastError());
    }
    const long long total = (long long)B * Ho * Wo * (C / per16);
    dim3 grid((unsigned)((total + 255) / 256 > 16384 ? 16384 : (total + 255) / 256));
#define L(DT) hipLaunchKernelGGL((dwconv3_kernel<DT>), grid, dim3(256), 0, s, (const char *)in, w, bias, (char *)out, B, H, W, Ho, Wo, C, stride, relu)
    if (dtype == TDRN_F32) L(float); else if (dtype == TDRN_BF16) L(bf16_t); else L(f16_t);
#undef L
    return hip_status(hipGetLastError());
}

__global__ __launch_bounds__(256) void softmax_rows_kernel(const float *__restrict__ in, float *__restrict__ out,
                                                           long long R, int C, int rb)
{
    extern __shared__ __attribute__((aligned(16))) float sm[];
    const long long r0 = (long long)blockIdx.x * rb;
    const int rows = (int)((R - r0) < rb ? (R - r0) : rb);
    const int n = rows * C;
    const int ld = C | 1;
    for (int i = threadIdx.x; i < n; i += 256) sm[(i / C) * ld + (i % C)] = in[r0 * C + i];
    __syncthreads();
    if ((int)threadIdx.x < rows) {
        float *row = sm + threadIdx.x * ld;
        float m = row[0];
        for (int c = 1; c < C; ++c) m = fmaxf(m, row[c]);
        float ssum = 0.f;
        for (int c = 0; c < C; ++c) {
            const float e = expf(row[c] - m);
            row[c] = e;
            ssum += e;
        }
        for (int c = 0; c < C; ++c) row[c] = row[c] / ssum;
    }
    __syncthreads();
    for (int i = threadIdx.x; i < n; i += 256) out[r0 * C + i] = sm[(i / C) * ld + (i % C)];
}

int launch_softmax_rows(const float *in, float *out, long long R, int C, hipStream_t s)
{
    if (C < 1 || C > 255) return TDRN_E_UNSUPPORTED;
    if (R <= 0) return TDRN_OK;
    const int rb = C <= 59 ? 256 : (C <= 119 ? 128 : 64);
    dim3 grid((unsigned)((R + rb - 1) / rb));
    hipLaunchKernelGGL(softmax_rows_kernel, grid, dim3(256), rb * (size_t)(C | 1) * sizeof(float), s, in, out, R, C, rb);
    return hip_status(hipGetLastError());
}

__global__ __launch_bounds__(256) void offset_conv_kernel(const float *__restrict__ loc, long long loc_bs,
                                                          long long loc_ps, const float *__restrict__ w,
                                                          const float *__restrict__ bias, float *__restrict__ off,
                                                          int B, int HW, int n_in, int n_out)
{
    __shared__ float s_w[128 * 16], s_b[128], s_l[64 * 16];
    const int t = threadIdx.x;
    const long long M = (long long)B * HW;
    const int oc0 = blockIdx.y * 128;
    const int nc = n_out - oc0 < 128 ? n_out - oc0 : 128;
    for (int i = t; i < nc * n_in; i += 256) s_w[i] = w[oc0 * n_in + i];
    for (int i = t; i < nc; i += 256) s_b[i] = bias ? bias[oc0 + i] : 0.f;
    for (long long m0 = (long long)blockIdx.x * 64; m0 < M; m0 += (long long)gridDim.x * 64) {
        __syncthreads();
        for (int i = t; i < 64 * n_in; i += 256) {
            const int r = i / n_in, j = i - r * n_in;
            const long long m = m0 + r;
            float v = 0.f;
            if (m < M) {
                const int b = (int)(m / HW), pix = (int)(m - (long long)b * HW);
                v = loc[b * loc_bs + pix * loc_ps + j];
            }
            s_l[i] = v;
        }
        __syncthreads();
        const int rows = M - m0 < 64 ? (int)(M - m0) : 64;
        const int total = rows * nc;
        float *dst = off + m0 * n_out + oc0;
        for (int idx = t; idx < total; idx += 256) {
            const int r = idx / nc, o = idx - r * nc;
            float acc = s_b[o];
            for (int j = 0; j < n_in; ++j) acc = fmaf(s_w[o * n_in + j], s_l[r * n_in + j], acc);
            dst[(long long)r * n_out + o] = acc;
        }
    }
}

int launch_offset_conv(const float *loc, long long loc_bs, long long loc_ps, const float *w, const float *bias,
                       float *off, int B, int HW, int n_in, int n_out, hipStream_t s)
{
    const long long M = (long long)B * HW;
    if (M <= 0 || n_out <= 0) return TDRN_OK;
    if (n_in > 16) return TDRN_E_UNSUPPORTED;
    const long long blocks = (M + 63) / 64;
    dim3 grid((unsigned)(blocks > 4096 ? 4096 : blocks), (unsigned)((n_out + 127) / 128));
    hipLaunchKernelGGL(offset_conv_kernel, grid, dim3(256), 0, s, loc, loc_bs, loc_ps, w, bias, off, B, HW, n_in, n_out);
    return hip_status(hipGetLastError());
}

__global__ __launch_bounds__(256) void offset_conv_multi_kernel(const OffsetMulti mp)
{
    __shared__ float s_w[128 * 16], s_b[128], s_l[64 * 16];
    const int t = threadIdx.x;
    int q = 0;
#pragma unroll
    for (int i = 1; i < 4; ++i)
        if (i < mp.n && (int)blockIdx.x >= mp.pr[i].blk0) q = i;
    const OffsetProblem &pr = mp.pr[q];
    const int n_in = 12, n_out = pr.n_out;
    const int oc0 = blockIdx.y * 128;
    if (oc0 >= n_out) return;
    const int nc = n_out - oc0 < 128 ? n_out - oc0 : 128;
    const long long M = (long long)pr.B * pr.HW;
    const long long m0 = (long long)((int)blockIdx.x - pr.blk0) * 64;
    for (int i = t; i < nc * n_in; i += 256) s_w[i] = pr.w[oc0 * n_in + i];
    for (int i = t; i < nc; i += 256) s_b[i] = pr.bias ? pr.bias[oc0 + i] : 0.f;
    for (int i = t; i < 64 * n_in; i += 256) {
        const int r = i / n_in, j = i - r * n_in;
        const long long m = m0 + r;
        float v = 0.f;
        if (m < M) {
            const int b = (int)(m / pr.HW), pix = (int)(m - (long long)b * pr.HW);
            v = pr.loc[b * pr.loc_bs + pix * pr.loc_ps + j];
        }
        s_l[i] = v;
    }
    __syncthreads();
    const int rows = M - m0 < 64 ? (int)(M - m0) : 64;
    const int total = rows * nc;
    float *dst = pr.off + m0 * n_out + oc0;
    for (int idx = t; idx < total; idx += 256) {
        const int r = idx / nc, o = idx - r * nc;
        float acc = s_b[o];
        for (int j = 0; j < n_in; ++j) acc = fmaf(s_w[o * n_in + j], s_l[r * n_in + j], acc);
        dst[(long long)r * n_out + o] = acc;
    }
}

int launch_offset_conv_multi(const OffsetProblem *pr, int n, hipStream_t s)
{
    if (n <= 0) return TDRN_OK;
    if (n > 4) return TDRN_E_ARG;
    OffsetMulti mp;
    mp.n = 0;
    int blocks = 0, max_out = 0;
    for (int i = 0; i < n; ++i) {
        const long long M = (long long)pr[i].B * pr[i].HW;
        if (M <= 0 || pr[i].n_out <= 0) continue;
        const long long b = (M + 63) / 64;
        if (blocks + b >= (1ll << 30)) return TDRN_E_UNSUPPORTED;
        mp.pr[mp.n] = pr[i];
        mp.pr[mp.n].blk0 = blocks;
        blocks += (int)b;
        max_out = pr[i].n_out > max_out ? pr[i].n_out : max_out;
        ++mp.n;
    }
    if (!mp.n) return TDRN_OK;
    hipLaunchKernelGGL(offset_conv_multi_kernel, dim3((unsigned)blocks, (unsigned)((max_out + 127) / 128)), dim3(256), 0, s, mp);
    return hip_status(hipGetLastError());
}

template <typename DT>
__global__ __launch_bounds__(256) void nchw_to_nhwc_kernel(const float *__restrict__ in, char *__restrict__ out, int B,
                                                           int C, int HW, int G, int cpg_pad)
{
    constexpr int ES = elem_traits<DT>::bytes;
    const int Cpad = G * cpg_pad, cpg = C / G;
    const long long total = (long long)B * HW * Cpad;
    for (long long i = (long long)blockIdx.x * blockDim.x + threadIdx.x; i < total; i += (long long)gridDim.x * blockDim.x) {
        const int cp = (int)(i % Cpad);
        const long long m = i / Cpad;
        const int b = (int)(m / HW), pix = (int)(m - (long long)b * HW);
        const int g = cp / cpg_pad, cl = cp - g * cpg_pad;
        const float v = cl < cpg ? in[((size_t)b * C + g * cpg + cl) * HW + pix] : 0.f;
        *(DT *)(out + (size_t)i * ES) = from_f32<DT>(v);
    }
}

int launch_nchw_to_nhwc_grouped(const float *in, void *out, int B, int C, int HW, int G, int cpg_pad, int dtype,
                                hipStream_t s)
{
    const long long total = (long long)B * HW * G * cpg_pad;
    if (total <= 0) return TDRN_OK;
    if (G < 1 || C % G) return TDRN_E_ARG;
    dim3 grid((unsigned)((total + 255) / 256 > 16384 ? 16384 : (total + 255) / 256));
#define L(DT) hipLaunchKernelGGL((nchw_to_nhwc_kernel<DT>), grid, dim3(256), 0, s, in, (char *)out, B, C, HW, G, cpg_pad)
    if (dtype == TDRN_F32) L(float); else if (dtype == TDRN_BF16) L(bf16_t); else L(f16_t);
#undef L
    return hip_status(hipGetLastError());
// ... 216 lines not shown
```

### tdrn_amd/csrc/net.h

```cpp
#pragma once
#include "net_plan.h"

struct tdrn_net : tdrn::Plan {
    tdrn::StagedParams staged;
    bool weights_ready = false;
    int profile = 0;
    std::vector<hipEvent_t> ev;
    std::vector<int> ev_stat;
    std::vector<int> ev_op;
    tdrn_kernel_stat stats[tdrn::ST_COUNT];
    int last_batch = 0;
    const void *offs_ws = nullptr;
    int offs_batch = 0, offs_key_batch = 0;
    int dev = -1;
    unsigned *status = nullptr;
    bool lanes_ready = false;
    hipStream_t side[tdrn::kLanes - 1] = {nullptr, nullptr, nullptr};
    hipEvent_t ev_fork = nullptr, ev_zero = nullptr, ev_skz = nullptr, ev_join[tdrn::kLanes - 1] = {nullptr, nullptr, nullptr};
    std::vector<hipEvent_t> tensor_ev;
    int first_op = 0;

    int init_lanes();
    int check_status(unsigned *detail);
    int collect_stats(tdrn_kernel_stat *out, int max_entries);
};

namespace tdrn {
namespace pool {
int cur_dev();
int get_timing_event(int dev, hipEvent_t *e);
int get_status(unsigned **w);
}
int run_forward(tdrn_net &n, const void *blob, void *ws, size_t ws_bytes, const tdrn_net_io *io, hipStream_t s0);
}
```

### tdrn_amd/csrc/net.hip

```cpp
#include <cstring>
#include <mutex>

#include "net.h"

namespace tdrn {

namespace pool {
std::mutex mu;
std::map<int, std::vector<hipStream_t>> streams;
std::map<int, std::vector<hipEvent_t>> events;
std::map<int, std::vector<hipEvent_t>> timing_events;
std::vector<unsigned *> status_words;
int cur_dev()
{
    int d = 0;
    (void)hipGetDevice(&d);
    return d;
}
template <class H, class Create>
int get(std::map<int, std::vector<H>> &m, int dev, H *h, Create create)
{
    {
        std::lock_guard<std::mutex> g(mu);
        auto &v = m[dev];
        if (!v.empty()) { *h = v.back(); v.pop_back(); return TDRN_OK; }
    }
    return hip_status(create(h));
}
template <class H>
void put(std::map<int, std::vector<H>> &m, int dev, H h) { if (h) { std::lock_guard<std::mutex> g(mu); m[dev].push_back(h); } }
int get_stream(int dev, hipStream_t *s) { return get(streams, dev, s, [](hipStream_t *p) { return hipStreamCreateWithFlags(p, hipStreamNonBlocking); }); }
int get_event(int dev, hipEvent_t *e) { return get(events, dev, e, [](hipEvent_t *p) { return hipEventCreateWithFlags(p, hipEventDisableTiming); }); }
int get_timing_event(int dev, hipEvent_t *e) { return get(timing_events, dev, e, [](hipEvent_t *p) { return hipEventCreate(p); }); }
int get_status(unsigned **w)
{
    {
        std::lock_guard<std::mutex> g(mu);
        if (!status_words.empty()) { *w = status_words.back(); status_words.pop_back(); memset(*w, 0, 64); return TDRN_OK; }
    }
    void *p = nullptr;
    TDRN_HIP_TRY(hipHostMalloc(&p, 64, hipHostMallocMapped | hipHostMallocPortable));
    memset(p, 0, 64);
    *w = (unsigned *)p;
    return TDRN_OK;
}
void put_status(unsigned *w) { if (w) { std::lock_guard<std::mutex> g(mu); status_words.push_back(w); } }
}

namespace {
const char *kStatNames[] = {"conv_igemm_mfma", "first_conv", "maxpool2x2", "l2norm", "dwconv3x3", "offset_conv1x1",
                            "deform_gemm_mfma", "softmax21", "layout", "conv3x3_patch_mfma", "dwpw_mfma"};
}
}

using namespace tdrn;

int tdrn_net::init_lanes()
{
    if (lanes_ready) return TDRN_OK;
    for (int i = 0; i < kLanes - 1; ++i) {
        TDRN_TRY(pool::get_stream(dev, &side[i]));
        TDRN_TRY(pool::get_event(dev, &ev_join[i]));
    }
    TDRN_TRY(pool::get_event(dev, &ev_fork));
    TDRN_TRY(pool::get_event(dev, &ev_zero));
    TDRN_TRY(pool::get_event(dev, &ev_skz));
    tensor_ev.assign(tensors.size(), nullptr);
    for (size_t t = 0; t < tensors.size(); ++t)
        if (tensor_shared[t]) TDRN_TRY(pool::get_event(dev, &tensor_ev[t]));
    lanes_ready = true;
    return TDRN_OK;
}

int tdrn_net::check_status(unsigned *detail)
{
    unsigned d = 0;
    if (status) {
        volatile unsigned *w = status;
        d = (w[0] ? 1u : 0u) | (w[1] ? 2u : 0u);
        if (d) { w[0] = 0; w[1] = 0; }
    }
    if (detail) *detail = d;
    return d ? TDRN_E_DEVICE : TDRN_OK;
}

int tdrn_net::collect_stats(tdrn_kernel_stat *out, int max_entries)
{
    for (int i = 0; i < ST_COUNT; ++i) {
        memset(&stats[i], 0, sizeof(stats[i]));
        strncpy(stats[i].name, kStatNames[i], sizeof(stats[i].name) - 1);
    }
    for (size_t i = 0; i < ops.size(); ++i) {
        const Op &o = ops[i];
        if (launch_head(i)) stats[o.stat].launches += 1;
        stats[o.stat].flops += o.flops * last_batch;
        stats[o.stat].bytes += o.bytes * last_batch;
    }
    for (size_t i = 0; i < ev_stat.size(); ++i) {
        float ms = 0.f;
        TDRN_HIP_TRY(hipEventSynchronize(ev[2 * i + 1]));
        TDRN_HIP_TRY(hipEventElapsedTime(&ms, ev[2 * i], ev[2 * i + 1]));
        stats[ev_stat[i]].ms += ms;
    }
    int n = 0;
    for (int i = 0; i < ST_COUNT && n < max_entries; ++i)
        if (stats[i].launches) out[n++] = stats[i];
    return n;
}

extern "C" {

int tdrn_net_create(const tdrn_net_config *cfg, tdrn_net **out)
{
    if (!cfg || !out) return TDRN_E_ARG;
    tdrn_net *n = new tdrn_net();
    n->cfg = *cfg;
    const int rc = n->build();
    if (rc != TDRN_OK) {
        delete n;
        return rc;
    }
    *out = n;
    return TDRN_OK;
}

void tdrn_net_destroy(tdrn_net *net)
{
    if (!net) return;
    const int d = net->dev;
    for (hipEvent_t e : net->ev) pool::put(pool::timing_events, d, e);
    for (hipEvent_t e : net->tensor_ev) pool::put(pool::events, d, e);
    for (int i = 0; i < kLanes - 1; ++i) {
        pool::put(pool::events, d, net->ev_join[i]);
        pool::put(pool::streams, d, net->side[i]);
    }
    pool::put(pool::events, d, net->ev_fork);
    pool::put(pool::events, d, net->ev_zero);
    pool::put(pool::events, d, net->ev_skz);
    pool::put_status(net->status);
    delete net;
}

int tdrn_net_param_count(const tdrn_net *net) { return net ? (int)net->params.size() : TDRN_E_ARG; }

int tdrn_net_param_info(const tdrn_net *net, int index, const char **name, int64_t shape[4], int *ndim)
{
    if (!net || index < 0 || index >= (int)net->params.size()) return TDRN_E_ARG;
    const ParamSpec &p = net->params[index];
    if (name) *name = p.name.c_str();
    if (ndim) *ndim = (int)p.shape.size();
    if (shape)
        for (size_t i = 0; i < 4; ++i) shape[i] = i < p.shape.size() ? p.shape[i] : 1;
    return TDRN_OK;
}

int tdrn_net_set_param(tdrn_net *net, const char *name, const float *data_host, int64_t numel)
{
    if (!net || !name || !data_host) return TDRN_E_ARG;
    auto it = net->param_index.find(name);
    if (it == net->param_index.end()) return TDRN_E_PARAM;
    int64_t want = 1;
    for (int64_t d : net->params[it->second].shape) want *= d;
    if (want != numel) return TDRN_E_PARAM;
    net->staged[name].assign(data_host, data_host + numel);
    net->weights_ready = false;
    return TDRN_OK;
}

size_t tdrn_net_weight_bytes(const tdrn_net *net) { return net ? net->blob_bytes : 0; }
size_t tdrn_net_workspace_bytes(const tdrn_net *net, int batch) { return net && batch > 0 ? net->ws_per_sample * (size_t)batch + net->ws_fixed : 0; }
int tdrn_net_num_priors(const tdrn_net *net) { return net ? net->P : TDRN_E_ARG; }

int tdrn_net_pack_weights(tdrn_net *net, void *weights_dev, size_t weights_bytes, void *stream)
{
    if (!net || !weights_dev) return TDRN_E_ARG;
    if (weights_bytes < net->blob_bytes) return TDRN_E_WORKSPACE;
    for (const ParamSpec &p : net->params)
        if (!net->staged.count(p.name)) return TDRN_E_PARAM;
    std::vector<char> host;
    TDRN_TRY(pack_weights(*net, net->staged, host));
    hipStream_t s = (hipStream_t)stream;
    TDRN_HIP_TRY(hipMemcpyAsync(weights_dev, host.data(), host.size(), hipMemcpyHostToDevice, s));
    TDRN_HIP_TRY(hipStreamSynchronize(s));
    net->weights_ready = true;
    net->staged.clear();
    return TDRN_OK;
}

int tdrn_net_adopt_weights(tdrn_net *net)
{
    if (!net) return TDRN_E_ARG;
    net->weights_ready = true;
    return TDRN_OK;
}

int tdrn_net_forward(tdrn_net *net, const void *weights_dev, void *workspace, size_t workspace_bytes, const tdrn_net_io *io,
                     void *stream)
{
    if (!net) return TDRN_E_ARG;
    return run_forward(*net, weights_dev, workspace, workspace_bytes, io, (hipStream_t)stream);
}

int tdrn_net_check(tdrn_net *net, unsigned *detail)
{
    if (!net) return TDRN_E_ARG;
    return net->check_status(detail);
}

int tdrn_net_op_count(const tdrn_net *net) { return net ? (int)net->ops.size() : TDRN_E_ARG; }

int tdrn_net_op_info(const tdrn_net *net, int index, tdrn_op_info *out)
{
    if (!net || !out || index < 0 || index >= (int)net->ops.size()) return TDRN_E_ARG;
    const Op &o = net->ops[index];
    memset(out, 0, sizeof(*out));
    switch (o.kind) {
        case OP_FIRST: out->kind = 0; break;
        case OP_CONV: out->kind = o.phases == 4 ? 2 : 1; break;
        case OP_DW: out->kind = 3; break;
        case OP_POOL: out->kind = 4; break;
        case OP_L2NORM: out->kind = 5; break;
        case OP_OFFSET: out->kind = 6; break;
        case OP_DEFORM: out->kind = 7; break;
        default: out->kind = 8; break;
    }
    out->in = o.in; out->out = o.out; out->res = o.res; out->pool = o.pool_t; out->off = o.off_t; out->y = o.y_t;
    out->k = o.k; out->stride = o.stride; out->pad = o.pad; out->dil = o.dil; out->relu = o.relu; out->ceil_mode = o.ceil;
    out->splitk = o.splitk; out->groups = o.G; out->out_kind = o.out_kind; out->level = o.scale;
    out->n_branches = o.n_branches; out->k2 = o.k2; out->pad2 = o.pad2; out->off_c0[0] = o.off_c0[0]; out->off_c0[1] = o.off_c0[1];
    if (o.kind == OP_DEFORM && o.y_t >= 0) {
        out->y_tap_major = net->y_tap_major ? 1 : 0;
        out->y_groups = o.y_groups;
    }
    out->fused_first = (index == net->fuse_first) ? 1 : 0;
    out->fused_dw = o.fused_dw;
    auto cp = [](char *d, const std::string &v) { strncpy(d, v.c_str(), 47); };
    cp(out->w, o.w); cp(out->b, o.b); cp(out->bn, o.bn); cp(out->w2, o.w2); cp(out->b2, o.b2);
    return TDRN_OK;
}

int tdrn_net_tensor_count(const tdrn_net *net) { return net ? (int)net->tensors.size() : TDRN_E_ARG; }

int tdrn_net_tensor_info(const tdrn_net *net, int index, const char **label, int *C, int *H, int *W)
{
    if (!net || index < 0 || index >= (int)net->tensors.size()) return TDRN_E_ARG;
    const Tensor &t = net->tensors[index];
    if (label) *label = t.label.c_str();
    if (C) *C = t.C;
    if (H) *H = t.H;
    if (W) *W = t.W;
    return TDRN_OK;
}

int tdrn_net_read_tensor(const tdrn_net *net, const void *workspace, int batch, int index, float *out_dev, void *stream)
{
    if (!net || !workspace || !out_dev || batch <= 0 || index < 0 || index >= (int)net->tensors.size()) return TDRN_E_ARG;
    const Tensor &t = net->tensors[index];
    return launch_nhwc_any_to_nchw_f32((const char *)workspace + t.off * (size_t)batch, t.f32 ? TDRN_F32 : net->cfg.dtype,
                                       t.Cpad, out_dev, batch, t.C, t.H * t.W, (hipStream_t)stream);
}

int tdrn_net_write_tensor(const tdrn_net *net, void *workspace, int batch, int index, const float *in_dev, void *stream)
{
    if (!net || !workspace || !in_dev || batch <= 0 || index < 0 || index >= (int)net->tensors.size()) return TDRN_E_ARG;
    const Tensor &t = net->tensors[index];
    return launch_nchw_to_nhwc(in_dev, (char *)workspace + t.off * (size_t)batch, batch, t.C, t.H * t.W, t.Cpad,
                               t.f32 ? TDRN_F32 : net->cfg.dtype, (hipStream_t)stream);
}

int tdrn_net_forward_from(tdrn_net *net, const void *weights_dev, void *workspace, size_t workspace_bytes, const tdrn_net_io *io,
                          int first_op, void *stream)
{
    if (!net || first_op < 0 || first_op > (int)net->ops.size()) return TDRN_E_ARG;
    if (net->use_lanes) return TDRN_E_STATE;
    net->first_op = first_op;
    const int rc = run_forward(*net, weights_dev, workspace, workspace_bytes, io, (hipStream_t)stream);
    net->first_op = 0;
    return rc;
}

int tdrn_net_profile(tdrn_net *net, int enable)
{
    if (!net) return TDRN_E_ARG;
    net->profile = enable < 0 ? 0 : (enable > 2 ? 2 : enable);
    return TDRN_OK;
}

int tdrn_net_op_stats(tdrn_net *net, tdrn_kernel_stat *out, int max_entries)
{
    if (!net || !out || max_entries <= 0) return TDRN_E_ARG;
    int n = 0;
    for (size_t i = 0; i < net->ev_op.size() && n < max_entries; ++i) {
        const Op &o = net->ops[net->ev_op[i]];
        float ms = 0.f;
        TDRN_HIP_TRY(hipEventSynchronize(net->ev[2 * i + 1]));
        TDRN_HIP_TRY(hipEventElapsedTime(&ms, net->ev[2 * i], net->ev[2 * i + 1]));
        tdrn_kernel_stat &k = out[n++];
        memset(&k, 0, sizeof(k));
        std::string name = std::string(kStatNames[o.stat]) + ":" + (o.w.empty() ? (o.in >= 0 ? net->tensors[o.in].label : "") : o.w);
        if (o.kind == OP_CONV && o.chain == 0) name = "conv_chain:" + o.w + "+" + std::to_string(net->chain_ops.size() - 1);
        strncpy(k.name, name.c_str(), sizeof(k.name) - 1);
        k.launches = 1;
        k.flops = o.flops * net->last_batch;
        k.bytes = o.bytes * net->last_batch;
        if (o.kind == OP_CONV && o.chain == 0)
            for (size_t j = 1; j < net->chain_ops.size(); ++j) {
                k.flops += net->ops[net->chain_ops[j]].flops * net->last_batch;
                k.bytes += net->ops[net->chain_ops[j]].bytes * net->last_batch;
            }
        if (o.kind == OP_DEFORM)
            for (int j = net->ev_op[i] - 1; j >= 0 && net->ops[j].kind == OP_DEFORM; --j) {
                k.flops += net->ops[j].flops * net->last_batch;
                k.bytes += net->ops[j].bytes * net->last_batch;
            }
        k.ms = ms;
    }
    return n;
}

int tdrn_net_op_timeline(tdrn_net *net, float *start_ms, float *end_ms, int *lane, int max_entries)
{
    if (!net || !start_ms || !end_ms || max_entries <= 0) return TDRN_E_ARG;
    int n = 0;
    for (size_t i = 0; i < net->ev_op.size() && n < max_entries; ++i, ++n) {
        TDRN_HIP_TRY(hipEventSynchronize(net->ev[2 * i + 1]));
        TDRN_HIP_TRY(hipEventElapsedTime(&start_ms[n], net->ev[0], net->ev[2 * i]));
        TDRN_HIP_TRY(hipEventElapsedTime(&end_ms[n], net->ev[0], net->ev[2 * i + 1]));
        if (lane) lane[n] = net->profile == 2 && net->use_lanes ? net->ops[net->ev_op[i]].lane : 0;
    }
    return n;
}

int tdrn_net_kernel_stats(tdrn_net *net, tdrn_kernel_stat *out, int max_entries)
{
    if (!net || !out || max_entries <= 0) return TDRN_E_ARG;
    return net->collect_stats(out, max_entries);
}

}
```

### tdrn_amd/csrc/net_plan.h

```cpp
#pragma once
#include <map>
#include <string>
#include <vector>

#include "kernels.h"

namespace tdrn {

enum OpKind { OP_FIRST, OP_CONV, OP_POOL, OP_L2NORM, OP_DW, OP_OFFSET, OP_DEFORM, OP_SOFTMAX, OP_OFF_OUT, OP_LOC_OUT,
              OP_REFLOC_IN };
enum OutKind { OUT_TENSOR = 0, OUT_ARM_LOC = 1, OUT_ODM_LOC = 2, OUT_CONF = 3 };
enum { ST_CONV, ST_FIRST, ST_POOL, ST_L2, ST_DW, ST_OFFSET, ST_DEFORM, ST_SOFTMAX, ST_LAYOUT, ST_CONV3, ST_DWPW, ST_COUNT };

struct Tensor { int C, Cpad, H, W; bool f32; size_t off;  std::string label; };
struct ParamSpec { std::string name; std::vector<int64_t> shape; };
using StagedParams = std::map<std::string, std::vector<float>>;

struct Op {
    OpKind kind;
    int in = -1, out = -1, res = -1;
    int Cin = 0, Cout = 0, Npad = 0, k = 1, stride = 1, pad = 0, dil = 1, relu = 0, phases = 1, ceil = 0;
    int out_kind = OUT_TENSOR, scale = 0, hw = 0;
    int G = 1, n_branches = 1, k2 = 0, pad2 = 0;
    int taps = 0;
    int split = 0;
    int off_t = -1, off_c0[2] = {0, 0}, off_n = 0;
    int loc_src = OUT_ARM_LOC;
    std::string w, b, bn, w2, b2;
    size_t w_off = 0, b_off = 0, w2_off = 0;
    int y_t = -1, y_cols = 0;
    int y_groups = 1;
    size_t wt_off = 0, bt_off = 0;
    double flops = 0, bytes = 0;
    int stat = 0;
    int lane = 0;
    int pool_t = -1;
    int splitk = 1;
    bool chain_tag = false;
    int chain = -1;
    int fused_dw = 0;
    size_t chain_partial = 0;
};

constexpr int kLanes = 4;
constexpr int kPlanRefBatch = 32;
constexpr size_t kTailCtl = 256;

struct Plan {
    tdrn_net_config cfg{};
    int es = 2;
    std::vector<Tensor> tensors;
    std::vector<ParamSpec> params;
    std::map<std::string, size_t> param_index;
    std::vector<Op> ops;
    size_t ws_per_sample = 0, blob_bytes = kZeroPageBytes;
    size_t ws_fixed = 0;
    int P = 0, fm[4] = {0, 0, 0, 0}, scale_off[5] = {0, 0, 0, 0, 0};
    size_t splitk_off[kLanes] = {0, 0, 0, 0};
    int t_late = -1;
    std::vector<int> chain_ops;
    size_t chain_partial_off = 0;
    bool pp_sk_planned = false;
    int fuse_first = -1;
    int x_t = -1;
    bool late_side = true;
    bool use_lanes = true;
    bool y_tap_major = true;
    int kdisable = 0, fault_handoff = 0;
    std::vector<int> tensor_lane;
    std::vector<char> tensor_shared;

    int build();
    int producer_of(int t) const;
    int readers_of(int t) const;
    void conv_geometry(const Op &o, int B, ConvArgs &a) const;
    ConvArgs conv_question(const Op &o, int B) const;
    bool launch_continues(size_t i) const
    {
        return i + 1 < ops.size() && ops[i + 1].kind == ops[i].kind && (ops[i].kind == OP_DEFORM || ops[i].kind == OP_OFFSET);
    }
    bool launch_head(size_t i) const
    {
        const Op &o = ops[i];
        return !(i > 0 && launch_continues(i - 1)) && !(o.kind == OP_CONV && (o.chain > 0 || o.fused_dw));
    }

private:
    int cur_lane = 0, plan_error = TDRN_OK;
    int T(int C, int H, int W, bool f32 = false);
    void P_(const std::string &name, std::vector<int64_t> shape);
    void bn_params(const std::string &bn, int C);
    int push(Op &o, const std::string &l = "") { o.lane = cur_lane; if (!l.empty()) label(o.out, l); ops.push_back(o); return o.out; }
    void label(int t, const std::string &l) { if (t >= 0) tensors[t].label = l; }
    size_t blob(size_t bytes);
    int first_conv(const std::string &w, bool bias, const std::string &bn, int Cout, int stride, int S);
    int conv(int in, const std::string &w, bool bias, const std::string &bn, int Cout, int k, int stride, int pad, int dil,
             int relu, int res = -1, int out_kind = OUT_TENSOR, int scale = 0, const std::string &w2 = "", int k2 = 0);
    int conv_transpose2(int in, const std::string &w, bool bias, int Cout, int res, int relu);
    bool can_fuse_pool(int in) const;
    int pool(int in, int ceil_mode, bool in_needed_elsewhere = false);
    int l2norm(int in, const std::string &name);
    int dwconv(int in, const std::string &w, const std::string &bn, int stride);
    int conv_dw(int in, const std::string &name, int Cout, int stride);
    int offset_conv(int scale, int H, int W, const std::string &w1, const std::string &w2, bool bias, int n1, int n2,
                    int loc_src, int ref_tensor = -1);
    void deform_heads(int in, int off_t, int scale, int G, const std::string &loc1, const std::string &conf1,
                      const std::string &loc2, const std::string &conf2, int off_c1, int out_loc_kind);
    void softmax_op();
    void offsets_out(int scale, int off_t, int n);
    void loc_maps_out(int scale);
    int ref_loc_in(int scale, int H, int W);
    void set_pyramid(int s0);
    void vgg_trunk(int S, bool bn, int c7, int &c43, int &c53, int &fc7);
    void vgg_sources(int src[4]);
    void tcb(const int src[4], bool bias, int odm[4]);
    void drn_heads(const int src[4], const int odm[4], bool bias);
    void mobilenet_sources(int S, int c7, bool extras_bias, int src[4]);
    int build_drn(bool mobile);
    int build_refinedet_vgg();
    int build_ssd4scale(bool mobile);
    void alias_u8_input();
    void hoist_l2norm_to_side_lanes();
    void plan_fuse_first();
    void plan_splitk();
    void plan_chain();
    void place_splitk_slabs();
    void plan_dwpw();
    void plan_workspace_tail();
    void mark_shared_tensors();
};

int pack_weights(const Plan &p, const StagedParams &staged, std::vector<char> &host);

}
```

### tdrn_amd/csrc/net_plan.hip

```cpp
#include <algorithm>
#include <cstdlib>

#include "net_plan.h"

namespace tdrn {

int Plan::T(int C, int H, int W, bool f32)
{
    Tensor t;
    t.C = C; t.H = H; t.W = W; t.f32 = f32;
    t.Cpad = f32 ? C : (int)align_up((size_t)C, kChanPad);
    t.off = ws_per_sample;
    ws_per_sample += align_up((size_t)t.Cpad * H * W * (f32 ? 4 : es), 256);
    tensors.push_back(t);
    return (int)tensors.size() - 1;
}
void Plan::P_(const std::string &name, std::vector<int64_t> shape)
{
    param_index[name] = params.size();
    params.push_back(ParamSpec{name, std::move(shape)});
}
void Plan::bn_params(const std::string &bn, int C)
{
    P_(bn + ".weight", {C}); P_(bn + ".bias", {C}); P_(bn + ".running_mean", {C}); P_(bn + ".running_var", {C});
// ... 450 lines not shown
        tensors.push_back(t);
        x_t = (int)tensors.size() - 1;
    } else {
        x_t = T(3, cfg.size, cfg.size, true);
    }
}

void Plan::hoist_l2norm_to_side_lanes()
{
    int side = 1;
    for (size_t i = 0; i < ops.size(); ++i) {
        if (ops[i].kind != OP_L2NORM) continue;
        const int prod = producer_of(ops[i].in);
        if (prod < 0) continue;
        Op o = ops[i];
        o.lane = side;
        side = side == 1 ? 2 : 1;
        ops.erase(ops.begin() + (long)i);
        ops.insert(ops.begin() + prod + 1, o);
    }
}

void Plan::plan_fuse_first()
{
    fuse_first = -1;
    if ((cfg.plan_flags & TDRN_PLAN_NO_FUSE_FIRST) || ops.size() <= 1 || ops[0].kind != OP_FIRST || ops[1].kind != OP_CONV || ops[0].stride != 1 ||
        tensors[ops[0].out].Cpad != 64) return;
    const Op &c = ops[1];
    const Tensor &ti = tensors[ops[0].out];
    fuse_first = 1;
    if (c.in != ops[0].out || readers_of(ops[0].out) != 1 || c.out_kind != OUT_TENSOR || c.lane != 0 || ti.H != ti.W ||
        !patch_takes(conv_question(c, 0), c.pool_t >= 0)) fuse_first = -1;
    if (fuse_first >= 0) {
        ops[1].flops += ops[0].flops;
        ops[1].bytes += 3.0 * ops[0].hw * ops[0].hw * 4 - (double)ti.H * ti.W * ti.Cpad * es;
        ops[0].flops = 0; ops[0].bytes = 0;
    }
}

void Plan::plan_splitk()
{
    for (Op &o : ops) {
        if (o.kind == OP_CONV && o.pool_t >= 0) o.stat = ST_CONV3;
        if (o.kind != OP_CONV || o.pool_t >= 0) continue;
        ConvArgs a;
        conv_geometry(o, kPlanRefBatch, a);
        a.out_f32 = o.out_kind != OUT_TENSOR;
        o.splitk = conv_splitk_choice(a);
        a = conv_question(o, kPlanRefBatch);
        const ConvKernel k = conv_route(a, false);
        const bool direct = k == CONV_PATCH || k == CONV_PP;
        if (direct) o.stat = ST_CONV3;
        if (o.chain_tag && !(o.out_kind == OUT_TENSOR && !direct && conv_chain_supported(a))) o.chain_tag = false;
    }
}

void Plan::plan_chain()
{
    chain_ops.clear();
    const bool chain_on = (cfg.plan_flags & TDRN_PLAN_CHAIN) != 0;
    int first = -1;
    for (size_t i = 0; i < ops.size() && chain_on; ++i) {
        Op &o = ops[i];
        if (o.kind != OP_CONV || !o.chain_tag || (int)chain_ops.size() == conv_chain_max_layers()) continue;
        bool ok = true;
        for (int t : {o.in, o.res}) {
            if (t < 0) continue;
            const int prod = producer_of(t);
            const bool member = prod >= 0 && ops[prod].chain >= 0;
            if (!member && first >= 0 && prod > first) ok = false;
        }
        if (!ok) continue;
        if (first < 0) first = (int)i;
        o.chain = (int)chain_ops.size();
        chain_ops.push_back((int)i);
    }
    if (chain_ops.size() < 3) {
        for (int i : chain_ops) ops[i].chain = -1;
        chain_ops.clear();
    }
    std::vector<int> level(ops.size(), 0);
    for (size_t k = 0; k < chain_ops.size(); ++k)
        for (int t : {ops[chain_ops[k]].in, ops[chain_ops[k]].res})
            for (size_t j = 0; j < k; ++j)
                if (t >= 0 && ops[chain_ops[j]].out == t && level[chain_ops[j]] + 1 > level[chain_ops[k]]) level[chain_ops[k]] = level[chain_ops[j]] + 1;
    std::stable_sort(chain_ops.begin(), chain_ops.end(), [&](int a, int b) { return level[a] < level[b]; });
    for (size_t k = 0; k < chain_ops.size(); ++k) ops[chain_ops[k]].chain = (int)k;
}

void Plan::place_splitk_slabs()
{
    size_t lane_bytes[kLanes] = {0, 0, 0, 0};
    size_t chain_bytes = 0;
    for (Op &o : ops) {
        if (o.kind != OP_CONV || o.pool_t >= 0 || o.splitk <= 1) continue;
        const size_t per_sample = align_up((size_t)o.splitk * o.phases * (o.hw >> 16) * (o.hw & 0xffff) * o.Npad * sizeof(float), 256);
        if (o.chain >= 0) {
            o.chain_partial = chain_bytes;
            chain_bytes += per_sample;
        } else if (per_sample > lane_bytes[o.lane]) {
            lane_bytes[o.lane] = per_sample;
        }
    }
    for (int i : chain_ops) ops[i].lane = 0;
    chain_partial_off = ws_per_sample;
    ws_per_sample += chain_bytes;
    if (const char *pd = getenv("TDRN_PLAN_DUMP")) {
        if (atoi(pd))
            for (const Op &o : ops)
                if (o.kind == OP_CONV)
                    fprintf(stderr, "plan: %-28s lane %d  %dx%d k%d s%d d%d  Cin %4d Cout %4d  splitk %d  %s/%s  chain %d\n", o.w.c_str(), o.lane,
                            o.hw >> 16, o.hw & 0xffff, o.k, o.stride, o.dil, o.Cin, o.Cout, o.splitk, conv_kernel_name(conv_route(conv_question(o, 1), o.pool_t >= 0)),
                            conv_kernel_name(conv_route(conv_question(o, kPlanRefBatch), o.pool_t >= 0)), o.chain);
    }
    for (int l = 0; l < kLanes; ++l) {
        splitk_off[l] = ws_per_sample;
        ws_per_sample += lane_bytes[l];
    }
}

void Plan::plan_dwpw()
{
    if (cfg.dtype == TDRN_F32 || !(cfg.plan_flags & TDRN_PLAN_DWPW)) return;
    for (size_t i = 0; i + 1 < ops.size(); ++i) {
        Op &d = ops[i];
        Op &c = ops[i + 1];
        if (d.kind != OP_DW || c.kind != OP_CONV || c.in != d.out || c.k != 1 || c.stride != 1 || c.pad != 0 || c.phases != 1 || c.res >= 0 ||
            c.out_kind != OUT_TENSOR || c.splitk != 1 || c.lane != d.lane || c.pool_t >= 0 || c.chain >= 0) continue;
        if (readers_of(d.out) != 1) continue;
        const Tensor &ti = tensors[d.in];
        DwPwArgs a;
        a.B = 1; a.H = ti.H; a.W = ti.W; a.Cin = c.Cin; a.Cout = c.Cout; a.Npad = c.Npad; a.Cs = tensors[c.out].Cpad;
        a.stride = d.stride; a.dtype = cfg.dtype;
        if (ti.Cpad != c.Cin || !dwpw_supported(a)) continue;
        d.fused_dw = 1; c.fused_dw = 1;
        d.stat = ST_DWPW;
        d.flops += c.flops;
        d.bytes = (double)ti.H * ti.W * ti.Cpad * es + (double)ti.H * ti.W * tensors[c.out].Cpad * es;
        c.flops = 0; c.bytes = 0;
    }
}

void Plan::plan_workspace_tail()
{
    ws_fixed = 0;
    pp_sk_planned = false;
    for (const Op &o : ops) {
        if (o.kind != OP_CONV || o.stat != ST_CONV3 || o.lane != 0) continue;
        ConvArgs a = conv_question(o, 0);
        a.kdisable = 0;
        pp_sk_planned = pp_sk_planned || pp_takes_geometry(a);
    }
    if (pp_sk_planned || !chain_ops.empty()) ws_fixed = kTailCtl + (pp_sk_planned ? align_up(conv_pp_sk_bytes(), 256) : 1024);
}

void Plan::mark_shared_tensors()
{
    tensor_lane.assign(tensors.size(), 0);
    tensor_shared.assign(tensors.size(), 0);
    for (const Op &o : ops) {
        if (o.out >= 0) tensor_lane[o.out] = o.lane;
        if (o.pool_t >= 0) tensor_lane[o.pool_t] = o.lane;
    }
    for (const Op &o : ops)
        for (int t : {o.in, o.res, o.off_t})
            if (t >= 0 && tensor_lane[t] != o.lane) tensor_shared[t] = 1;
}

int Plan::build()
{
    es = dtype_bytes(cfg.dtype);
    static const struct { int plan_flag, koff; } kSwitches[] = {
        {TDRN_PLAN_NO_CONV_PP, KOFF_CONV_PP},       {TDRN_PLAN_NO_PP_SK, KOFF_PP_SK},
        {TDRN_PLAN_NO_CONV_PATCH, KOFF_CONV_PATCH}, {TDRN_PLAN_NO_PW1X1, KOFF_PW1X1},
        {TDRN_PLAN_NO_DW_SLIDE, KOFF_DW_SLIDE},     {TDRN_PLAN_DW_SLIDE_ALL, KOFF_DW_STRIP_SMALL},
        {TDRN_PLAN_NO_CONV_WS, KOFF_CONV_WS},       {TDRN_PLAN_NO_YGEMM_V2, KOFF_YGEMM_V2},
        {TDRN_PLAN_NO_HEAD3X3, KOFF_HEAD3X3},       {TDRN_PLAN_TS_ONE_RANGE, KOFF_TS_RANGES},
        {TDRN_PLAN_NO_PATCH_TAIL, KOFF_PATCH_TAIL},
    };
    kdisable = 0;
    for (const auto &sw : kSwitches)
        if (cfg.plan_flags & sw.plan_flag) kdisable |= sw.koff;
    fault_handoff = (cfg.plan_flags & TDRN_PLAN_FAULT_HANDOFF) ? 1 : 0;
    late_side = !(cfg.plan_flags & TDRN_PLAN_NO_LATE_SIDE);
    use_lanes = !(cfg.plan_flags & TDRN_PLAN_ONE_STREAM);
    if (cfg.size < 128 || cfg.size > 1280 || cfg.size % 64 != 0) return TDRN_E_ARG;
    if (cfg.num_classes < 2 || cfg.num_classes > 21 * 4) return TDRN_E_ARG;
    if (cfg.dtype < 0 || cfg.dtype > 2) return TDRN_E_ARG;
    if (cfg.def_groups < 1) return TDRN_E_ARG;
    int rc;
    switch (cfg.model) {
        case TDRN_DRN_VGGBN: rc = build_drn(false); break;
        case TDRN_DRN_MOBILENET: rc = build_drn(true); break;
        case TDRN_SSD4SCALE_MOBILE: rc = build_ssd4scale(true); break;
        case TDRN_SSD4SCALE_VGG: rc = build_ssd4scale(false); break;
        case TDRN_REFINEDET_VGG: rc = build_refinedet_vgg(); break;
        default: return TDRN_E_UNSUPPORTED;
    }
    if (rc != TDRN_OK) return rc;
    if (plan_error != TDRN_OK) return plan_error;
    alias_u8_input();
    hoist_l2norm_to_side_lanes();
    plan_fuse_first();
    plan_splitk();
    plan_chain();
    place_splitk_slabs();
    plan_dwpw();
    plan_workspace_tail();
    y_tap_major = true;
    for (const Op &d : ops)
        if (d.kind == OP_DEFORM && d.y_t >= 0 && !ygemm_supported(d.Cin, d.y_cols, cfg.dtype)) y_tap_major = false;
    mark_shared_tensors();
    return TDRN_OK;
}

}
```

### tdrn_amd/csrc/net_run.hip

```cpp
#include "net.h"

namespace tdrn {
namespace {

struct Run {
    tdrn_net &n;
    const Plan &p;
    const void *blob; void *ws; size_t ws_bytes; const tdrn_net_io *io; hipStream_t s0;
    const char *wb = nullptr;
    const tdrn_u8_frames *u8 = nullptr;
    const float *xin = nullptr;
    int B = 0, C = 0;
    int Bk = 0;
    bool lanes = false, join_on = false, reuse_offsets = false;
    bool lane_used[kLanes] = {true, false, false, false};
    bool zeroed_early = false, skz_pending = false, dwpw_done = false;
    char *tail = nullptr;
    DeformArgs dargs[4];
    int ts_op[4] = {-1, -1, -1, -1}, n_dargs = 0;
    OffsetProblem oq[4];
    int oq_op[4], n_oq = 0;
    size_t evi = 0;
    int offset_ops_enqueued = 0;

    Run(tdrn_net &net, const void *blob_, void *ws_, size_t ws_bytes_, const tdrn_net_io *io_, hipStream_t s)
        : n(net), p(net), blob(blob_), ws(ws_), ws_bytes(ws_bytes_), io(io_), s0(s) {}
    ~Run() { (void)join(); }
    int join()
    {
        if (!join_on) return TDRN_OK;
        join_on = false;
        int rc = TDRN_OK;
        for (int l = 1; l < kLanes; ++l)
            if (lane_used[l]) {
                hipError_t e = hipEventRecord(n.ev_join[l - 1], n.side[l - 1]);
                if (e == hipSuccess) e = hipStreamWaitEvent(s0, n.ev_join[l - 1], 0);
                if (e != hipSuccess && rc == TDRN_OK) rc = (int)e;
            }
        return rc;
    }

    char *tptr(int id) const { return (char *)ws + p.tensors[id].off * (size_t)B; }
    float *loc_out(const Op &o) const { return o.out_kind == OUT_ARM_LOC ? io->arm_loc : io->odm_loc; }
    bool launch_open(const Op &o) const { return (o.kind == OP_DEFORM && n_dargs > 0) || (o.kind == OP_OFFSET && n_oq > 0); }
    int record(int t, hipStream_t s) const
    {
        if (lanes && t >= 0 && p.tensor_shared[t]) TDRN_HIP_TRY(hipEventRecord(n.tensor_ev[t], s));
        return TDRN_OK;
    }

    int check_args()
    {
        if (!n.weights_ready) return TDRN_E_STATE;
        if (!blob || !ws || !io || io->batch <= 0) return TDRN_E_ARG;
        u8 = (const tdrn_u8_frames *)io->reserved[3];
        if (u8 ? !u8->planes : !io->x) return TDRN_E_ARG;
        xin = u8 ? nullptr : io->x;
        B = io->batch;
        if (ws_bytes < p.ws_per_sample * (size_t)B + p.ws_fixed) return TDRN_E_WORKSPACE;
        if (!io->conf) return TDRN_E_ARG;
        const int d = pool::cur_dev();
        if (n.dev < 0) n.dev = d;
        else if (n.dev != d) return TDRN_E_STATE;
        if (p.ws_fixed) {
            if (!n.status) TDRN_TRY(pool::get_status(&n.status));
            TDRN_TRY(n.check_status(nullptr));
        }
        const bool is_drn = p.cfg.model == TDRN_DRN_VGGBN || p.cfg.model == TDRN_DRN_MOBILENET || p.cfg.model == TDRN_REFINEDET_VGG;
        const bool has_arm = p.cfg.model != TDRN_REFINEDET_VGG || p.cfg.use_refine;
        if (is_drn && !io->odm_loc) return TDRN_E_ARG;
        if (has_arm && !io->arm_loc) return TDRN_E_ARG;
        wb = (const char *)blob;
        C = p.cfg.num_classes;
        n.last_batch = B;
        return TDRN_OK;
    }

    int fork()
    {
        if (n.profile && n.ev.size() < 2 * p.ops.size()) {
            const size_t old = n.ev.size();
            n.ev.resize(2 * p.ops.size());
            for (size_t i = old; i < n.ev.size(); ++i) TDRN_TRY(pool::get_timing_event(n.dev, &n.ev[i]));
        }
        n.ev_stat.clear();
        n.ev_op.clear();
        lanes = p.use_lanes && n.profile != 1;
        if (lanes) {
            TDRN_TRY(n.init_lanes());
            TDRN_HIP_TRY(hipEventRecord(n.ev_fork, s0));
        }
        join_on = lanes;
        return TDRN_OK;
    }

    int open_lane(int lane, hipStream_t s)
    {
        if (!lane_used[lane]) TDRN_HIP_TRY(hipStreamWaitEvent(s, n.ev_fork, 0));
        lane_used[lane] = true;
        return TDRN_OK;
    }

    int zero_split_outputs(const Op &o, hipStream_t s) const
    {
        TDRN_HIP_TRY(hipMemsetAsync(loc_out(o), 0, (size_t)B * p.P * 4 * sizeof(float), s));
        TDRN_HIP_TRY(hipMemsetAsync(io->conf, 0, (size_t)B * p.P * C * sizeof(float), s));
        return TDRN_OK;
    }

    int zero_early()
    {
        if (lanes) {
            const Op *dsplit = nullptr;
            int n_deform_groups = 0;
            for (size_t k = 0; k < p.ops.size(); ++k)
                if (p.ops[k].kind == OP_DEFORM) {
                    if (p.ops[k].split && p.ops[k].y_t < 0 && !dsplit) dsplit = &p.ops[k];
                    if (k == 0 || p.ops[k - 1].kind != OP_DEFORM) ++n_deform_groups;
                }
            if (dsplit && n_deform_groups == 1) {
                TDRN_TRY(open_lane(1, n.side[0]));
                TDRN_TRY(zero_split_outputs(*dsplit, n.side[0]));
                TDRN_HIP_TRY(hipEventRecord(n.ev_zero, n.side[0]));
                zeroed_early = true;
            }
        }
        tail = (char *)ws + p.ws_per_sample * (size_t)B;
        if (!p.ws_fixed) return TDRN_OK;
        if (lanes) {
            TDRN_TRY(open_lane(1, n.side[0]));
            TDRN_HIP_TRY(hipMemsetAsync(tail, 0, kTailCtl + 1024, n.side[0]));
            TDRN_HIP_TRY(hipEventRecord(n.ev_skz, n.side[0]));
            skz_pending = true;
        } else {
            TDRN_HIP_TRY(hipMemsetAsync(tail, 0, kTailCtl + 1024, s0));
        }
        return TDRN_OK;
    }

    int check_reuse()
    {
        reuse_offsets = p.cfg.deform && io->reserved[0] != nullptr;
        if (reuse_offsets && (n.offs_ws != ws || n.offs_batch != B)) return TDRN_E_STATE;
        Bk = B;
        if (io->reserved[1]) {
            const long long kb = (long long)(intptr_t)io->reserved[1];
            if (!p.cfg.deform || kb < 1 || kb > B || B % kb) return TDRN_E_ARG;
            Bk = (int)kb;
        }
        if (reuse_offsets && n.offs_key_batch != Bk) return TDRN_E_STATE;
        if (p.cfg.deform && !reuse_offsets) { n.offs_ws = nullptr; n.offs_batch = 0; n.offs_key_batch = 0; }
        return TDRN_OK;
    }

    int prologue()
    {
        TDRN_TRY(check_args());
        TDRN_TRY(fork());
        TDRN_TRY(zero_early());
        return check_reuse();
    }

    int epilogue()
    {
        const int jrc = join();
        int offset_ops_planned = 0;
        for (const Op &d : p.ops) offset_ops_planned += d.kind == OP_OFFSET;
        if (jrc == TDRN_OK && p.cfg.deform && !reuse_offsets && offset_ops_planned > 0 && offset_ops_enqueued == offset_ops_planned) {
            n.offs_ws = ws; n.offs_batch = B; n.offs_key_batch = Bk;
        }
        return jrc;
    }

    bool skipped(size_t oi)
    {
        const Op &o = p.ops[oi];
        if (o.kind == OP_CONV && o.fused_dw && dwpw_done) { dwpw_done = false; return true; }
        if (o.kind == OP_OFF_OUT && !io->offsets[o.scale]) return true;
        if (o.kind == OP_LOC_OUT && !io->loc_maps[o.scale]) return true;
        if (reuse_offsets && (o.kind == OP_REFLOC_IN || o.kind == OP_OFFSET)) return true;
        if (o.kind == OP_FIRST && p.fuse_first >= 0) return true;
        if (o.kind == OP_CONV && o.chain > 0) return true;
        return (int)oi < n.first_op;
    }

    int stream_for(const Op &o, int &lane, hipStream_t &s)
    {
        lane = lanes ? o.lane : 0;
        s = lane == 0 ? s0 : n.side[lane - 1];
        if (!lanes) return TDRN_OK;
        TDRN_TRY(open_lane(lane, s));
        for (int t : {o.in, o.res, o.off_t})
            if (t >= 0 && p.tensor_lane[t] != lane) TDRN_HIP_TRY(hipStreamWaitEvent(s, n.tensor_ev[t], 0));
        if (p.late_side && lane != 0 && (o.kind == OP_CONV || o.kind == OP_OFFSET) && p.t_late >= 0 && p.tensor_shared[p.t_late])
            TDRN_HIP_TRY(hipStreamWaitEvent(s, n.tensor_ev[p.t_late], 0));
        return TDRN_OK;
    }

    int wait_tail_zeroed()
    {
        if (!skz_pending) return TDRN_OK;
        TDRN_HIP_TRY(hipStreamWaitEvent(s0, n.ev_skz, 0));
        skz_pending = false;
        return TDRN_OK;
    }

    void conv_args(const Op &o, ConvArgs &a) const
    {
        p.conv_geometry(o, B, a);
        a.in = tptr(o.in); a.w = wb + o.w_off; a.bias = (const float *)(wb + o.b_off); a.zero_page = wb;
        a.relu = o.relu;
        a.status = n.status; a.fault_handoff = p.fault_handoff;
        if (o.out_kind == OUT_TENSOR) {
            const Tensor &to = p.tensors[o.out];
            a.out = tptr(o.out);
            if (o.res >= 0) a.res = tptr(o.res);
            a.o_cs = to.Cpad;
            if (o.phases == 4) {
                a.o_bs = (long long)to.H * to.W * to.Cpad; a.o_rs = 2ll * to.W * to.Cpad; a.o_cs = 2ll * to.Cpad;
                a.o_pr = (long long)to.W * to.Cpad; a.o_pc = to.Cpad;
            } else {
                a.o_bs = (long long)to.H * to.W * to.Cpad; a.o_rs = (long long)to.W * to.Cpad;
            }
        } else {
            const int per = o.out_kind == OUT_CONF ? 3 * C : 12;
            const int per_prior = o.out_kind == OUT_CONF ? C : 4;
            a.out = o.out_kind == OUT_CONF ? io->conf : loc_out(o); a.out_f32 = 1;
            a.o_base = (long long)p.scale_off[o.scale] * per_prior;
            a.o_bs = (long long)p.P * per_prior; a.o_rs = (long long)a.Wo * per; a.o_cs = per;
        }
        if (o.splitk > 1) {
            a.splitk = o.splitk;
            a.partial = (char *)ws + (o.chain >= 0 ? p.chain_partial_off + o.chain_partial : p.splitk_off[o.lane]) * (size_t)B;
        }
    }

    int ensure_f32_input(hipStream_t s)
    {
        if (xin) return TDRN_OK;
        TDRN_TRY(launch_u8_planes_to_f32(u8->planes, B, p.cfg.size, u8->mean, (float *)tptr(p.x_t), s));
        xin = (const float *)tptr(p.x_t);
        return TDRN_OK;
    }

    int launch_first(const Op &f, hipStream_t s) const
    {
        return launch_first_conv(xin, (const float *)(wb + f.w_off), (const float *)(wb + f.b_off), tptr(f.out), B, f.hw, f.stride, f.Cout,
                                 p.tensors[f.out].Cpad, f.relu, p.cfg.dtype, s);
    }

    int run_conv_chain(hipStream_t s)
    {
        ChainLayer cl[16];
        const int nl = (int)p.chain_ops.size();
        for (int k = 0; k < nl; ++k) {
            const Op &m = p.ops[p.chain_ops[k]];
            conv_args(m, cl[k].a);
            int nd = 0;
            for (int t : {m.in, m.res}) {
                if (t < 0) continue;
                int dep = -1;
                for (int j = 0; j < k; ++j)
                    if (p.ops[p.chain_ops[j]].out == t) dep = j;
                if (dep >= 0) cl[k].dep[nd++] = dep;
                else if (lanes && p.tensor_lane[t] != 0) TDRN_HIP_TRY(hipStreamWaitEvent(s, n.tensor_ev[t], 0));
            }
        }
        TDRN_TRY(wait_tail_zeroed());
        TDRN_TRY(launch_conv_chain(cl, nl, (unsigned *)tail, s, n.status));
        for (int k = 1; k < nl; ++k) TDRN_TRY(record(p.ops[p.chain_ops[k]].out, s));
        return TDRN_OK;
    }

    int run_conv(size_t oi, hipStream_t s)
    {
        const Op &o = p.ops[oi];
        const bool pooled = o.pool_t >= 0;
        ConvArgs a;
        conv_args(o, a);
        if (o.lane == 0 && p.pp_sk_planned) {
            a.sk_ws = tail + kTailCtl;
            a.sk_flags_zero = true;
            if (skz_pending && pp_takes_geometry(a)) TDRN_TRY(wait_tail_zeroed());
        }
        if ((int)oi == p.fuse_first) {
            const Op &f = p.ops[0];
            a.fuse_w = (const float *)(wb + f.w_off); a.fuse_b = (const float *)(wb + f.b_off);
            a.fuse_cout = f.Cout;
            if (!xin) {
                a.fuse_x8 = u8->planes; a.fuse_mean[0] = u8->mean[0]; a.fuse_mean[1] = u8->mean[1]; a.fuse_mean[2] = u8->mean[2];
                if (conv_route(a, pooled) != CONV_WS) {
                    a.fuse_x8 = nullptr;
                    TDRN_TRY(ensure_f32_input(s));
                }
            }
            a.fuse_x = xin;
            if (conv_route(a, pooled) == CONV_NONE) {
                TDRN_TRY(launch_first(f, s));
                a.fuse_x = nullptr; a.fuse_w = nullptr; a.fuse_b = nullptr; a.fuse_cout = 0;
            }
        }
        return launch_conv(a, s, pooled ? tptr(o.pool_t) : nullptr);
    }

    int run_dw(size_t oi, hipStream_t s)
    {
        const Op &o = p.ops[oi];
        const Tensor &ti = p.tensors[o.in];
        if (o.fused_dw) {
            const Op &c = p.ops[oi + 1];
            DwPwArgs a;
            a.in = tptr(o.in); a.w = wb + c.w_off; a.wdw = (const float *)(wb + o.w_off); a.bdw = (const float *)(wb + o.b_off);
            a.bias = (const float *)(wb + c.b_off); a.out = tptr(c.out);
            a.B = B; a.H = ti.H; a.W = ti.W; a.Cin = c.Cin; a.Cout = c.Cout; a.Npad = c.Npad; a.Cs = p.tensors[c.out].Cpad;
            a.stride = o.stride; a.relu_dw = o.relu; a.relu = c.relu; a.dtype = p.cfg.dtype;
            if (dwpw_supported(a)) {
                dwpw_done = true;
                TDRN_TRY(launch_dwpw(a, s));
                return record(c.out, s);
            }
        }
        return launch_dwconv3(tptr(o.in), (const float *)(wb + o.w_off), (const float *)(wb + o.b_off), tptr(o.out), B, ti.H, ti.W, ti.Cpad,
                              o.stride, o.relu, p.cfg.dtype, s, p.kdisable);
    }

    int run_offset(size_t oi, int lane, hipStream_t s)
    {
        const Op &o = p.ops[oi];
        const float *loc;
        long long bs, ps;
        if (o.in >= 0) { loc = (const float *)tptr(o.in); bs = (long long)o.hw * 12; ps = 12; }
        else { loc = io->arm_loc + (size_t)p.scale_off[o.scale] * 4; bs = (long long)p.P * 4; ps = 12; }
        oq[n_oq] = OffsetProblem{loc, bs, ps, (const float *)(wb + o.w_off), (const float *)(wb + o.b_off),
                                 (float *)tptr(o.out), o.in >= 0 ? Bk : B, o.hw, o.off_n, 0};
        oq_op[n_oq++] = (int)oi;
        if (p.launch_continues(oi) && n_oq < 4 && (lanes ? p.ops[oi + 1].lane : 0) == lane) return TDRN_OK;
        TDRN_TRY(launch_offset_conv_multi(oq, n_oq, s));
        for (int i = 0; i + 1 < n_oq; ++i) TDRN_TRY(record(p.ops[oq_op[i]].out, s));
        n_oq = 0;
        return TDRN_OK;
    }

    int run_deform(size_t oi, hipStream_t s)
    {
        const Op &o = p.ops[oi];
        const Tensor &ti = p.tensors[o.in];
        const Tensor &tf = p.tensors[o.off_t];
        DeformArgs a;
        a.in = tptr(o.in); a.zero_page = wb; a.n_branches = o.n_branches;
        const float *off = (const float *)tptr(o.off_t);
        a.br[0] = DeformBranch{off + o.off_c0[0], tf.C, wb + o.w_off, 3, 3, 1, 1, 1, o.G};
        if (o.n_branches == 2) a.br[1] = DeformBranch{off + o.off_c0[1], tf.C, wb + o.w2_off, 5, 5, 2, 1, 1, o.G};
        if (Bk < B)
            for (int k = 0; k < o.n_branches; ++k) a.br[k].off_rows = Bk * ti.H * ti.W;
        a.B = B; a.H = ti.H; a.W = ti.W; a.Cin = o.Cin; a.Ho = ti.H; a.Wo = ti.W; a.Cout = o.Cout; a.Npad = o.Npad;
        a.out0 = loc_out(o) + (size_t)p.scale_off[o.scale] * 4; a.o0_bs = (long long)p.P * 4; a.o0_ps = 12;
        a.out1 = io->conf + (size_t)p.scale_off[o.scale] * C; a.o1_bs = (long long)p.P * C; a.o1_ps = 3 * C;
        a.split = 12; a.dtype = p.cfg.dtype;
        dargs[n_dargs++] = a;
        if (o.y_t >= 0) ts_op[n_dargs - 1] = (int)oi;
        if (p.launch_continues(oi) && n_dargs < 4) return TDRN_OK;
        const int rc = o.y_t >= 0 ? run_deform_ts(s) : run_deform_gather(o, s);
        n_dargs = 0;
        return rc;
    }

    int run_deform_ts(hipStream_t s)
    {
        int Bc = B;
        size_t per_frame = 0;
        for (int i = 0; i < n_dargs; ++i) {
            const Op &d = p.ops[ts_op[i]];
            const int fit = deform_ts_max_batch(dargs[i].H, dargs[i].W, d.y_cols, d.taps);
            Bc = fit < Bc ? fit : Bc;
            per_frame += (size_t)dargs[i].H * dargs[i].W * d.y_cols * p.es;
        }
        if (Bc < 1) return TDRN_E_UNSUPPORTED;
        constexpr size_t kRangeBytes = (size_t)192 << 20;
        if (per_frame > 0 && !(p.kdisable & KOFF_TS_RANGES)) {
            long long fit = (long long)kRangeBytes / (long long)per_frame;
            fit = fit < 1 ? 1 : fit;
            if (fit < Bc) Bc = (int)fit;
        }
        const int n_groups = p.ops[ts_op[0]].y_groups;
        for (int b0 = 0; b0 < B; b0 += Bc)
            for (int yg = 0; yg < n_groups; ++yg) TDRN_TRY(run_deform_ts_range(b0, B - b0 < Bc ? B - b0 : Bc, yg, n_groups, s));
        return TDRN_OK;
    }

    int run_deform_ts_range(int b0, int nb, int yg, int n_groups, hipStream_t s)
    {
        DeformArgs ca[4];
        YGemmProblem yq[4];
        const void *ts_y[4] = {nullptr, nullptr, nullptr, nullptr};
        int ts_cs[4] = {0, 0, 0, 0}, n_yq = 0;
        const int es = p.es, dtype = p.cfg.dtype;
        bool all_ygemm = true;
        for (int i = 0; i < n_dargs; ++i) all_ygemm = all_ygemm && ygemm_supported(p.ops[ts_op[i]].Cin, p.ops[ts_op[i]].y_cols, dtype);
        for (int i = 0; i < n_dargs; ++i) {
            const Op &d = p.ops[ts_op[i]];
            DeformArgs &c = ca[i];
            c = dargs[i];
            const size_t px0 = (size_t)b0 * c.H * c.W;
            c.B = nb;
            c.in = (const char *)c.in + px0 * c.Cin * es;
            for (int k = 0; k < c.n_branches; ++k) {
                if (c.br[k].off_rows) c.br[k].off_row0 = (int)(px0 % (size_t)c.br[k].off_rows);
                else c.br[k].off += px0 * c.br[k].off_stride;
            }
            c.out0 += (size_t)b0 * c.o0_bs;
            c.out1 += (size_t)b0 * c.o1_bs;
            if (d.y_groups != n_groups) return TDRN_E_STATE;
            void *ybuf = tptr(d.y_t) + (size_t)yg * d.y_cols * c.H * c.W * es * B;
            const char *wty = wb + d.wt_off + (size_t)yg * d.y_cols * d.Cin * es;
            const int y_taps = p.y_tap_major ? d.taps : 0;
            c.Cout = d.Cout - 80 * yg < 80 ? d.Cout - 80 * yg : 80;
            if (yg > 0) { c.split = 0; c.out1 += 80 * yg - 12; }
            if (all_ygemm) {
                yq[n_yq++] = YGemmProblem{c.in, wty, ybuf, (long long)nb * c.H * c.W, d.y_cols, d.y_cols, y_taps};
            } else if (ygemm_supported(d.Cin, d.y_cols, dtype)) {
                TDRN_TRY(launch_ygemm(c.in, wty, ybuf, (long long)nb * c.H * c.W, d.y_cols, d.y_cols, dtype, s, y_taps));
            } else {
                ConvArgs g;
                p.conv_geometry(d, nb, g);
                g.Cout = g.Npad = d.y_cols; g.kh = g.kw = 1; g.pad = 0;
                g.in = c.in; g.w = wty; g.bias = (const float *)(wb + d.bt_off); g.zero_page = wb; g.out = ybuf;
                g.o_cs = d.y_cols; g.o_rs = (long long)c.W * d.y_cols; g.o_bs = (long long)c.H * c.W * d.y_cols;
                TDRN_TRY(launch_conv(g, s));
            }
            ts_y[i] = ybuf; ts_cs[i] = d.y_cols;
        }
        if (n_yq > 0) TDRN_TRY(launch_ygemm_multi(yq, n_yq, dtype, s, p.kdisable));
        return launch_deform_sample_multi(ca, ts_y, ts_cs, n_dargs, s, p.y_tap_major ? 1 : 0);
    }

    int run_deform_gather(const Op &o, hipStream_t s)
    {
        if (o.split) {
            if (zeroed_early) TDRN_HIP_TRY(hipStreamWaitEvent(s, n.ev_zero, 0));
            else TDRN_TRY(zero_split_outputs(o, s));
        }
        if (dargs[0].Npad <= 128) return launch_deform_multi(dargs, n_dargs, s, o.split);
        for (int c0 = 0; c0 < dargs[0].Cout; c0 += 128) {
            DeformArgs ga[4];
            for (int i = 0; i < n_dargs; ++i) {
                ga[i] = dargs[i];
                const int cols = dargs[i].Cout - c0 < 128 ? dargs[i].Cout - c0 : 128;
                ga[i].Cout = cols; ga[i].Npad = deform_n_pad(cols);
                for (int k = 0; k < ga[i].n_branches; ++k)
                    ga[i].br[k].w = (const char *)dargs[i].br[k].w + (size_t)c0 * dargs[i].br[k].kh * dargs[i].br[k].kw * dargs[i].Cin * p.es;
                if (c0 > 0) { ga[i].out1 += c0 - dargs[i].split; ga[i].split = 0; }
            }
            TDRN_TRY(launch_deform_multi(ga, n_dargs, s, o.split));
        }
        return TDRN_OK;
    }

    int run_op(size_t oi)
    {
        const Op &o = p.ops[oi];
        if (skipped(oi)) return TDRN_OK;
        int lane;
        hipStream_t s;
        TDRN_TRY(stream_for(o, lane, s));
        if (n.profile && !launch_open(o)) TDRN_HIP_TRY(hipEventRecord(n.ev[evi], s));
        const Tensor *ti = o.in >= 0 ? &p.tensors[o.in] : nullptr;
        switch (o.kind) {
            case OP_FIRST:
                TDRN_TRY(ensure_f32_input(s));
                TDRN_TRY(launch_first(o, s));
                break;
            case OP_CONV: TDRN_TRY(o.chain >= 0 ? run_conv_chain(s) : run_conv(oi, s)); break;
            case OP_POOL:
                TDRN_TRY(launch_maxpool2(tptr(o.in), tptr(o.out), B, ti->H, ti->W, ti->Cpad, o.ceil, p.cfg.dtype, s));
                break;
            case OP_L2NORM:
                TDRN_TRY(launch_l2norm(tptr(o.in), (const float *)(wb + o.w_off), tptr(o.out), (long long)B * ti->H * ti->W, ti->Cpad, p.cfg.dtype, s));
                break;
            case OP_DW: TDRN_TRY(run_dw(oi, s)); break;
            case OP_REFLOC_IN:
                if (!io->ref_loc[o.scale]) return TDRN_E_ARG;
                if (io->reserved[2]) TDRN_HIP_TRY(hipStreamWaitEvent(s, (hipEvent_t)io->reserved[2], 0));
                TDRN_TRY(launch_nchw_to_nhwc(io->ref_loc[o.scale], tptr(o.out), Bk, 12, o.hw, 12, TDRN_F32, s));
                break;
            case OP_OFFSET: TDRN_TRY(run_offset(oi, lane, s)); break;
            case OP_DEFORM: TDRN_TRY(run_deform(oi, s)); break;
            case OP_SOFTMAX: TDRN_TRY(launch_softmax_rows(io->conf, io->conf, (long long)B * p.P, C, s)); break;
            case OP_OFF_OUT:
                TDRN_TRY(launch_nhwc_to_nchw_f32((const float *)tptr(o.in), (long long)ti->H * ti->W * ti->C, ti->C, io->offsets[o.scale], Bk, o.Cout,
                                                 ti->H * ti->W, s));
                break;
            case OP_LOC_OUT:
                TDRN_TRY(launch_nhwc_to_nchw_f32(io->arm_loc + (size_t)p.scale_off[o.scale] * 4, (long long)p.P * 4, 12, io->loc_maps[o.scale], B, 12,
                                                 p.fm[o.scale] * p.fm[o.scale], s));
                break;
        }
        offset_ops_enqueued += o.kind == OP_OFFSET;
        if (!launch_open(o)) TDRN_TRY(record(o.out, s));
        TDRN_TRY(record(o.pool_t, s));
        if (n.profile && !launch_open(o)) {
            TDRN_HIP_TRY(hipEventRecord(n.ev[evi + 1], s));
            n.ev_stat.push_back(o.stat);
            n.ev_op.push_back((int)oi);
            evi += 2;
        }
        return TDRN_OK;
    }
};

}

int run_forward(tdrn_net &n, const void *blob, void *ws, size_t ws_bytes, const tdrn_net_io *io, hipStream_t s0)
{
    Run r(n, blob, ws, ws_bytes, io, s0);
    TDRN_TRY(r.prologue());
    for (size_t oi = 0; oi < n.ops.size(); ++oi) TDRN_TRY(r.run_op(oi));
    return r.epilogue();
}

}
```

Baseline: 12210 frames/s.

## Fuse offset computation and conf softmax into the deformable sampling kernel

The deformable sampling kernel can now compute its own per-tap offsets from arm_loc with a small 12-input dot product, and can apply the class softmax to the confidence outputs before writing them. This removes the separate offset-conv and softmax launches and their global round trips. It also adds a variant that issues 8 gather loads per batch instead of 6. The plan enables this when the deform ops are contiguous and no external offsets or ref_loc are supplied. The cost is redundant offset arithmetic per wave and more template instantiations with higher register use.

```diff
diff --git a/include/tdrn_hip.h b/include/tdrn_hip.h
--- a/include/tdrn_hip.h
+++ b/include/tdrn_hip.h
@@ -223,6 +223,7 @@
 #define TDRN_PLAN_NO_HEAD3X3   32768
 #define TDRN_PLAN_TS_ONE_RANGE  65536
 #define TDRN_PLAN_NO_PATCH_TAIL 131072
+#define TDRN_PLAN_NO_SAMPLE_FUSED 262144
 #define TDRN_PLAN_FAULT_HANDOFF 256
 
 typedef struct tdrn_net tdrn_net;
@@ -262,6 +263,10 @@
 
 TDRN_API int tdrn_net_forward(tdrn_net *net, const void *weights_dev, void *workspace,
                               size_t workspace_bytes, const tdrn_net_io *io, void *stream);
+#define TDRN_SAMPLE_OFFSETS 1
+#define TDRN_SAMPLE_SOFTMAX 2
+#define TDRN_SAMPLE_LOADS8  4
+TDRN_API int tdrn_net_sample_form(const tdrn_net *net, const tdrn_net_io *io);
 
 TDRN_API int tdrn_net_check(tdrn_net *net, unsigned *detail);
 
@@ -291,6 +296,7 @@
     int fused_dw;
     char w[48], b[48], bn[48], w2[48], b2[48];
     int y_groups;
+    int sample_fused;
 } tdrn_op_info;
 TDRN_API int tdrn_net_op_count(const tdrn_net *net);
 TDRN_API int tdrn_net_op_info(const tdrn_net *net, int index, tdrn_op_info *out);
diff --git a/tdrn_amd/_lib.py b/tdrn_amd/_lib.py
--- a/tdrn_amd/_lib.py
+++ b/tdrn_amd/_lib.py
@@ -29,7 +29,8 @@
 PLAN_NO_FUSE_FIRST, PLAN_NO_LATE_SIDE, PLAN_ONE_STREAM, PLAN_NO_DEFORM_TS, PLAN_CHAIN = 1, 2, 4, 8, 16
 PLAN_NO_CONV_PP, PLAN_NO_PP_SK, PLAN_NO_CONV_PATCH, PLAN_FAULT_HANDOFF, PLAN_DWPW, PLAN_NO_PW1X1 = 32, 64, 128, 256, 512, 1024
 PLAN_NO_DW_SLIDE, PLAN_DW_SLIDE_ALL, PLAN_NO_CONV_WS, PLAN_NO_YGEMM_V2, PLAN_NO_HEAD3X3, PLAN_TS_ONE_RANGE = 2048, 4096, 8192, 16384, 32768, 65536
-PLAN_NO_PATCH_TAIL = 131072
+PLAN_NO_PATCH_TAIL, PLAN_NO_SAMPLE_FUSED = 131072, 262144
+SAMPLE_OFFSETS, SAMPLE_SOFTMAX, SAMPLE_LOADS8 = 1, 2, 4
 E_DEVICE = -8
 
 
@@ -55,7 +56,7 @@
                 ("ceil_mode", C.c_int), ("splitk", C.c_int), ("groups", C.c_int), ("out_kind", C.c_int), ("level", C.c_int),
                 ("n_branches", C.c_int), ("k2", C.c_int), ("pad2", C.c_int), ("off_c0", C.c_int * 2), ("y_tap_major", C.c_int),
                 ("fused_first", C.c_int), ("fused_dw", C.c_int), ("w", C.c_char * 48), ("b", C.c_char * 48), ("bn", C.c_char * 48), ("w2", C.c_char * 48),
-                ("b2", C.c_char * 48), ("y_groups", C.c_int)]
+                ("b2", C.c_char * 48), ("y_groups", C.c_int), ("sample_fused", C.c_int)]
 
 
 class AugmentParams(C.Structure):
@@ -146,6 +147,7 @@
     "tdrn_net_pack_weights": (C.c_int, [C.c_void_p, C.c_void_p, C.c_size_t, C.c_void_p]),
     "tdrn_net_adopt_weights": (C.c_int, [C.c_void_p]),
     "tdrn_net_forward": (C.c_int, [C.c_void_p, C.c_void_p, C.c_void_p, C.c_size_t, C.POINTER(NetIO), C.c_void_p]),
+    "tdrn_net_sample_form": (C.c_int, [C.c_void_p, C.POINTER(NetIO)]),
     "tdrn_net_check": (C.c_int, [C.c_void_p, C.POINTER(C.c_uint)]),
     "tdrn_net_op_count": (C.c_int, [C.c_void_p]),
     "tdrn_net_op_info": (C.c_int, [C.c_void_p, C.c_int, C.POINTER(OpInfo)]),
diff --git a/tdrn_amd/csrc/common.h b/tdrn_amd/csrc/common.h
--- a/tdrn_amd/csrc/common.h
+++ b/tdrn_amd/csrc/common.h
@@ -112,6 +112,20 @@
     return r;
 }
 
+template <bool WAVE>
+__device__ __forceinline__ void softmax_row(float *row, int C, int c0, int cs)
+{
+    float m = row[0];
+    for (int c = 1; c < C; ++c) m = fmaxf(m, row[c]);
+    if (WAVE) __builtin_amdgcn_wave_barrier();
+    for (int c = c0; c < C; c += cs) row[c] = expf(row[c] - m);
+    if (WAVE) { __builtin_amdgcn_s_waitcnt(0xC07F); __builtin_amdgcn_wave_barrier(); }
+    float ssum = 0.f;
+    for (int c = 0; c < C; ++c) ssum += row[c];
+    if (WAVE) __builtin_amdgcn_wave_barrier();
+    for (int c = c0; c < C; c += cs) row[c] = row[c] / ssum;
+}
+
 inline int hip_status(hipError_t e) { return e == hipSuccess ? TDRN_OK : (int)e; }
 #define TDRN_HIP_TRY(expr)                                   \
     do {                                                     \
diff --git a/tdrn_amd/csrc/deform.hip b/tdrn_amd/csrc/deform.hip
--- a/tdrn_amd/csrc/deform.hip
+++ b/tdrn_amd/csrc/deform.hip
@@ -347,6 +347,9 @@
     const float *off;
     int off_stride, kh, kw, pad_h, pad_w, dil_h, dil_w, col0;
     int off_rows, off_row0;
+    const float *loc;
+    long long loc_bs, loc_ps;
+    const float *ow, *ob;
 };
 struct SampleParams {
     const char *y;
@@ -354,6 +357,7 @@
     int n_branches, n_taps;
     int M, H, W, ycs, Cout, split;
     int tap_major;
+    int softmax_C;
     float *out0, *out1;
     long long o0_bs, o0_ps, o1_bs, o1_ps;
 };
@@ -364,7 +368,7 @@
 };
 constexpr int kSampleCols = 80;
 
-template <typename DT>
+template <typename DT, int U, bool OFFK, bool SMAX>
 __global__ __launch_bounds__(256) void deform_sample_kernel(const SampleMulti mp)
 {
     const int nblk = (int)gridDim.x, xq = nblk >> 3, xr = nblk & 7, xcd = (int)blockIdx.x & 7;
@@ -375,9 +379,11 @@
         if (i < mp.n && blk >= mp.block_start[i]) prob = i;
     const SampleParams &p = mp.p[prob];
     constexpr int MAXR = 34 * 4;
+    constexpr int RB = 6 * U;
+    static_assert((MAXR + RB - 1) / RB * RB <= MAXR + 8, "the padded row table must fit s_ow");
     __shared__ uint2 s_ow[4][MAXR + 8];
     __shared__ float s_red[4][6][kSampleCols];
-    const int lane = threadIdx.x & 63, wave = threadIdx.x >> 6;
+    const int lane = threadIdx.x & 63, wave = __builtin_amdgcn_readfirstlane((int)threadIdx.x >> 6);
     const int m = (blk - mp.block_start[prob]) * 4 + wave;
     if (m >= p.M) return;
     const int HW = p.H * p.W;
@@ -388,9 +394,27 @@
         const SampleBranchP &B = p.br[brn];
         const int tl = lane - (brn ? p.br[0].kh * p.br[0].kw : 0);
         const int ti = tl / B.kw, tj = tl - ti * B.kw;
-        const int orow = B.off_rows ? (m + B.off_row0) % B.off_rows : m;
-        const float *op = B.off + (size_t)orow * B.off_stride + 2 * tl;
-        const float offset_h = op[0], offset_w = op[1];
+        float offset_h, offset_w;
+        if (OFFK) {
+            const float *lp = p.br[0].loc + b * p.br[0].loc_bs + rem * p.br[0].loc_ps;
+            const float *wr = B.ow + 24 * tl;
+            offset_h = B.ob[2 * tl];
+            offset_w = B.ob[2 * tl + 1];
+#pragma unroll
+            for (int jj = 0; jj < 12; ++jj) {
+                const float l = lp[jj];
+                offset_h = fmaf(wr[jj], l, offset_h);
+                offset_w = fmaf(wr[12 + jj], l, offset_w);
+            }
+            float *op = const_cast<float *>(B.off) + (size_t)m * B.off_stride + 2 * tl;
+            op[0] = offset_h;
+            op[1] = offset_w;
+        } else {
+            const int orow = B.off_rows ? (m + B.off_row0) % B.off_rows : m;
+            const float *op = B.off + (size_t)orow * B.off_stride + 2 * tl;
+            offset_h = op[0];
+            offset_w = op[1];
+        }
         float w1 = 0.f, w2 = 0.f, w3 = 0.f, w4 = 0.f;
         int q1 = 0, q2 = 0, q3 = 0, q4 = 0;
         const int h_in = ho - B.pad_h, w_in = wo - B.pad_w;
@@ -418,26 +442,26 @@
         s_ow[wave][4 * lane + 2] = make_uint2((img + q3) * rowb + colb, __float_as_uint(w3));
         s_ow[wave][4 * lane + 3] = make_uint2((img + q4) * rowb + colb, __float_as_uint(w4));
         if (lane == p.n_taps - 1)
-            for (int r = nrows; r < 36 * ((nrows + 35) / 36); ++r) s_ow[wave][r] = make_uint2((img + q4) * rowb + colb, 0u);
+            for (int r = nrows; r < RB * ((nrows + RB - 1) / RB); ++r) s_ow[wave][r] = make_uint2((img + q4) * rowb + colb, 0u);
     }
     __builtin_amdgcn_s_waitcnt(0xC07F);
     __builtin_amdgcn_wave_barrier();
     const int j = lane / 10, c = lane - 10 * j;
     float acc[8] = {0.f, 0.f, 0.f, 0.f, 0.f, 0.f, 0.f, 0.f};
     if (lane < 60) {
-        const int nb = (nrows + 35) / 36;
+        const int nb = (nrows + RB - 1) / RB;
         const __attribute__((address_space(1))) char *yb = (const __attribute__((address_space(1))) char *)p.y;
         for (int ib = 0; ib < nb; ++ib) {
-            u32x4 raw[6];
-            float wgt[6];
-#pragma unroll
-            for (int u = 0; u < 6; ++u) {
-                const uint2 ow = s_ow[wave][6 * (6 * ib + u) + j];
+            u32x4 raw[U];
+            float wgt[U];
+#pragma unroll
+            for (int u = 0; u < U; ++u) {
+                const uint2 ow = s_ow[wave][6 * (U * ib + u) + j];
                 wgt[u] = __uint_as_float(ow.y);
                 raw[u] = *(const __attribute__((address_space(1))) u32x4 *)(yb + (ow.x + (unsigned)(c * 16)));
             }
 #pragma unroll
-            for (int u = 0; u < 6; ++u) {
+            for (int u = 0; u < U; ++u) {
                 float v[8];
                 unpack16<DT>(raw[u], v);
 #pragma unroll
@@ -453,8 +477,26 @@
         float v = s_red[wave][0][co];
 #pragma unroll
         for (int jj = 1; jj < 6; ++jj) v += s_red[wave][jj][co];
-        float *dst = co < p.split ? p.out0 + b * p.o0_bs + rem * p.o0_ps + co : p.out1 + b * p.o1_bs + rem * p.o1_ps + (co - p.split);
-        *dst = v;
+        if (SMAX) {
+            s_red[wave][0][co] = v;
+        } else {
+            float *dst = co < p.split ? p.out0 + b * p.o0_bs + rem * p.o0_ps + co : p.out1 + b * p.o1_bs + rem * p.o1_ps + (co - p.split);
+            *dst = v;
+        }
+    }
+    if (SMAX) {
+        __builtin_amdgcn_s_waitcnt(0xC07F);
+        __builtin_amdgcn_wave_barrier();
+        const int C = p.softmax_C;
+        const bool own = lane < p.Cout - p.split;
+        const int r = own ? lane / C : 0;
+        softmax_row<true>(&s_red[wave][0][p.split + r * C], C, own ? lane - r * C : C, C);
+        __builtin_amdgcn_s_waitcnt(0xC07F);
+        __builtin_amdgcn_wave_barrier();
+        for (int co = lane; co < p.Cout; co += 64) {
+            float *dst = co < p.split ? p.out0 + b * p.o0_bs + rem * p.o0_ps + co : p.out1 + b * p.o1_bs + rem * p.o1_ps + (co - p.split);
+            *dst = s_red[wave][0][co];
+        }
     }
 }
 
@@ -862,16 +904,38 @@
     return (int)(b > (1 << 20) ? (1 << 20) : b);
 }
 
-int launch_deform_sample_multi(const DeformArgs *args, const void *const *y, const int *ycs, int n, hipStream_t s, int tap_major)
+template <typename DT>
+static void launch_sample_dt(const SampleMulti &mp, dim3 grid, hipStream_t s, bool loads8, bool offk, bool smax)
+{
+#define L(U, O, S) hipLaunchKernelGGL((deform_sample_kernel<DT, U, O, S>), grid, dim3(256), 0, s, mp)
+    if (loads8) {
+        if (offk) { if (smax) L(8, true, true); else L(8, true, false); }
+        else { if (smax) L(8, false, true); else L(8, false, false); }
+    } else {
+        if (offk) { if (smax) L(6, true, true); else L(6, true, false); }
+        else { if (smax) L(6, false, true); else L(6, false, false); }
+    }
+#undef L
+}
+
+int launch_deform_sample_multi(const DeformArgs *args, const void *const *y, const int *ycs, int n, hipStream_t s, int tap_major, int variant)
 {
     if (!args || n < 1 || n > 4) return TDRN_E_ARG;
     SampleMulti mp;
     mp.n = 0;
     mp.block_start[0] = 0;
+    const bool offk = args[0].br[0].loc != nullptr, smax = args[0].softmax_C > 0;
     for (int i = 0; i < n; ++i) {
         const DeformArgs &a = args[i];
         const int taps = deform_sample_supported(a);
         if (!taps || a.dtype != args[0].dtype) return TDRN_E_UNSUPPORTED;
+        if ((a.softmax_C > 0) != smax) return TDRN_E_ARG;
+        if (smax && (a.split < 0 || a.split > a.Cout || a.Cout - a.split > 64 || (a.Cout - a.split) % a.softmax_C != 0)) return TDRN_E_UNSUPPORTED;
+        for (int k = 0; k < a.n_branches; ++k) {
+            const DeformBranch &b = a.br[k];
+            if ((b.loc != nullptr) != offk) return TDRN_E_ARG;
+            if (offk && (!b.ow || !b.ob || !b.off || b.off_rows || b.loc != a.br[0].loc || b.loc_bs != a.br[0].loc_bs || b.loc_ps != a.br[0].loc_ps)) return TDRN_E_ARG;
+        }
         if ((long long)a.B * a.H * a.W * ycs[i] * 2 >= (1ll << 32)) return TDRN_E_UNSUPPORTED;
         SampleParams p;
         p.y = (const char *)y[i];
@@ -879,12 +943,14 @@
         int col0 = 0;
         for (int k = 0; k < a.n_branches; ++k) {
             const DeformBranch &b = a.br[k];
-            p.br[k] = SampleBranchP{b.off, b.off_stride, b.kh, b.kw, b.pad, b.pad_w < 0 ? b.pad : b.pad_w, b.dil, b.dil_w < 1 ? b.dil : b.dil_w, col0, b.off_rows, b.off_row0};
+            p.br[k] = SampleBranchP{b.off, b.off_stride, b.kh, b.kw, b.pad, b.pad_w < 0 ? b.pad : b.pad_w, b.dil, b.dil_w < 1 ? b.dil : b.dil_w, col0, b.off_rows, b.off_row0,
+                                    b.loc, b.loc_bs, b.loc_ps, b.ow, b.ob};
             col0 += b.kh * b.kw;
         }
         if (a.n_branches == 1) p.br[1] = p.br[0];
         p.M = a.B * a.H * a.W; p.H = a.H; p.W = a.W; p.ycs = ycs[i]; p.Cout = a.Cout; p.tap_major = tap_major;
         p.split = a.split > a.Cout ? a.Cout : a.split;
+        p.softmax_C = a.softmax_C;
         p.out0 = a.out0; p.out1 = a.out1;
         p.o0_bs = a.o0_bs; p.o0_ps = a.o0_ps; p.o1_bs = a.o1_bs; p.o1_ps = a.o1_ps;
         if (p.M <= 0) continue;
@@ -895,8 +961,8 @@
     if (mp.n == 0) return TDRN_OK;
     for (int i = mp.n; i < 4; ++i) { mp.p[i] = mp.p[0]; mp.block_start[i + 1] = mp.block_start[mp.n]; }
     dim3 grid((unsigned)mp.block_start[mp.n]);
-    if (args[0].dtype == TDRN_BF16) hipLaunchKernelGGL((deform_sample_kernel<bf16_t>), grid, dim3(256), 0, s, mp);
-    else hipLaunchKernelGGL((deform_sample_kernel<f16_t>), grid, dim3(256), 0, s, mp);
+    if (args[0].dtype == TDRN_BF16) launch_sample_dt<bf16_t>(mp, grid, s, (variant & SAMPLE_LOADS8) != 0, offk, smax);
+    else launch_sample_dt<f16_t>(mp, grid, s, (variant & SAMPLE_LOADS8) != 0, offk, smax);
     return hip_status(hipGetLastError());
 }
 
diff --git a/tdrn_amd/csrc/kernels.h b/tdrn_amd/csrc/kernels.h
--- a/tdrn_amd/csrc/kernels.h
+++ b/tdrn_amd/csrc/kernels.h
@@ -136,6 +136,9 @@
     int kh = 3, kw = 3, pad = 1, stride = 1, dil = 1, G = 1;
     int pad_w = -1, stride_w = -1, dil_w = -1;
     int off_rows = 0, off_row0 = 0;
+    const float *loc = nullptr;
+    long long loc_bs = 0, loc_ps = 0;
+    const float *ow = nullptr, *ob = nullptr;
 };
 struct DeformArgs {
     const void *in = nullptr, *zero_page = nullptr;
@@ -146,6 +149,7 @@
     int split = 0;
     long long o0_bs = 0, o0_ps = 0, o1_bs = 0, o1_ps = 0;
     int dtype = TDRN_BF16;
+    int softmax_C = 0;
 };
 int launch_deform(const DeformArgs &a, hipStream_t s);
 int launch_deform_multi(const DeformArgs *args, int n, hipStream_t s, int split_branches);
@@ -178,7 +182,8 @@
 int deform_sample_cols(int taps);
 constexpr int deform_y_col(int tap) { return (tap / 3) * 256 + (tap % 3) * 80; }
 int deform_ts_max_batch(int H, int W, int ycs, int taps);
-int launch_deform_sample_multi(const DeformArgs *args, const void *const *y, const int *ycs, int n, hipStream_t s, int tap_major = 0);
+enum { SAMPLE_LOADS8 = 1 };
+int launch_deform_sample_multi(const DeformArgs *args, const void *const *y, const int *ycs, int n, hipStream_t s, int tap_major = 0, int variant = 0);
 int ygemm_supported(int Cin, int ycols, int dtype);
 int launch_ygemm(const void *x, const void *w, void *y, long long M, int N, int ycs, int dtype, hipStream_t s, int taps = 0);
 struct YGemmProblem { const void *x, *w; void *y; long long M; int N, ycs, taps; };
diff --git a/tdrn_amd/csrc/layers.hip b/tdrn_amd/csrc/layers.hip
--- a/tdrn_amd/csrc/layers.hip
+++ b/tdrn_amd/csrc/layers.hip
@@ -623,18 +623,7 @@
     const int ld = C | 1;
     for (int i = threadIdx.x; i < n; i += 256) sm[(i / C) * ld + (i % C)] = in[r0 * C + i];
     __syncthreads();
-    if ((int)threadIdx.x < rows) {
-        float *row = sm + threadIdx.x * ld;
-        float m = row[0];
-        for (int c = 1; c < C; ++c) m = fmaxf(m, row[c]);
-        float ssum = 0.f;
-        for (int c = 0; c < C; ++c) {
-            const float e = expf(row[c] - m);
-            row[c] = e;
-            ssum += e;
-        }
-        for (int c = 0; c < C; ++c) row[c] = row[c] / ssum;
-    }
+    if ((int)threadIdx.x < rows) softmax_row<false>(sm + threadIdx.x * ld, C, 0, 1);
     __syncthreads();
     for (int i = threadIdx.x; i < n; i += 256) out[r0 * C + i] = sm[(i / C) * ld + (i % C)];
 }
diff --git a/tdrn_amd/csrc/net.h b/tdrn_amd/csrc/net.h
--- a/tdrn_amd/csrc/net.h
+++ b/tdrn_amd/csrc/net.h
@@ -10,6 +10,7 @@
     std::vector<int> ev_op;
     tdrn_kernel_stat stats[tdrn::ST_COUNT];
     int last_batch = 0;
+    int last_form = 0;
     const void *offs_ws = nullptr;
     int offs_batch = 0, offs_key_batch = 0;
     int dev = -1;
diff --git a/tdrn_amd/csrc/net.hip b/tdrn_amd/csrc/net.hip
--- a/tdrn_amd/csrc/net.hip
+++ b/tdrn_amd/csrc/net.hip
@@ -92,9 +92,11 @@
     }
     for (size_t i = 0; i < ops.size(); ++i) {
         const Op &o = ops[i];
-        if (launch_head(i)) stats[o.stat].launches += 1;
-        stats[o.stat].flops += o.flops * last_batch;
-        stats[o.stat].bytes += o.bytes * last_batch;
+        const bool in_sample = (o.kind == OP_OFFSET && (last_form & TDRN_SAMPLE_OFFSETS)) || (o.kind == OP_SOFTMAX && (last_form & TDRN_SAMPLE_SOFTMAX));
+        const int st = in_sample ? (int)ST_DEFORM : o.stat;
+        if (launch_head(i) && !in_sample) stats[st].launches += 1;
+        stats[st].flops += o.flops * last_batch;
+        stats[st].bytes += o.bytes * last_batch;
     }
     for (size_t i = 0; i < ev_stat.size(); ++i) {
         float ms = 0.f;
@@ -199,6 +201,12 @@
 {
     if (!net) return TDRN_E_ARG;
     return run_forward(*net, weights_dev, workspace, workspace_bytes, io, (hipStream_t)stream);
+}
+
+int tdrn_net_sample_form(const tdrn_net *net, const tdrn_net_io *io)
+{
+    if (!net || !io) return TDRN_E_ARG;
+    return net->sample_form(io, 0);
 }
 
 int tdrn_net_check(tdrn_net *net, unsigned *detail)
@@ -232,6 +240,9 @@
         out->y_tap_major = net->y_tap_major ? 1 : 0;
         out->y_groups = o.y_groups;
     }
+    if (o.kind == OP_DEFORM && net->sample_fused) out->sample_fused = TDRN_SAMPLE_OFFSETS | TDRN_SAMPLE_LOADS8 | (net->sample_softmax ? TDRN_SAMPLE_SOFTMAX : 0);
+    if (o.kind == OP_OFFSET) out->sample_fused = net->sample_fused ? 1 : 0;
+    if (o.kind == OP_SOFTMAX) out->sample_fused = net->sample_softmax ? 1 : 0;
     out->fused_first = (index == net->fuse_first) ? 1 : 0;
     out->fused_dw = o.fused_dw;
     auto cp = [](char *d, const std::string &v) { strncpy(d, v.c_str(), 47); };
@@ -308,11 +319,21 @@
                 k.flops += net->ops[net->chain_ops[j]].flops * net->last_batch;
                 k.bytes += net->ops[net->chain_ops[j]].bytes * net->last_batch;
             }
-        if (o.kind == OP_DEFORM)
+        if (o.kind == OP_DEFORM) {
             for (int j = net->ev_op[i] - 1; j >= 0 && net->ops[j].kind == OP_DEFORM; --j) {
                 k.flops += net->ops[j].flops * net->last_batch;
                 k.bytes += net->ops[j].bytes * net->last_batch;
             }
+            for (const Op &f : net->ops) {
+                if (!((f.kind == OP_OFFSET && (net->last_form & TDRN_SAMPLE_OFFSETS)) || (f.kind == OP_SOFTMAX && (net->last_form & TDRN_SAMPLE_SOFTMAX)))) continue;
+                k.flops += f.flops * net->last_batch;
+                k.bytes += f.bytes * net->last_batch;
+            }
+            if (net->last_form & TDRN_SAMPLE_OFFSETS) name += "+offset";
+            if (net->last_form & TDRN_SAMPLE_SOFTMAX) name += "+softmax";
+            memset(k.name, 0, sizeof(k.name));
+            strncpy(k.name, name.c_str(), sizeof(k.name) - 1);
+        }
         k.ms = ms;
     }
     return n;
diff --git a/tdrn_amd/csrc/net_plan.h b/tdrn_amd/csrc/net_plan.h
--- a/tdrn_amd/csrc/net_plan.h
+++ b/tdrn_amd/csrc/net_plan.h
@@ -66,11 +66,13 @@
     bool late_side = true;
     bool use_lanes = true;
     bool y_tap_major = true;
+    bool sample_fused = false, sample_softmax = false;
     int kdisable = 0, fault_handoff = 0;
     std::vector<int> tensor_lane;
     std::vector<char> tensor_shared;
 
     int build();
+    int sample_form(const tdrn_net_io *io, int first_op) const;
     int producer_of(int t) const;
     int readers_of(int t) const;
     void conv_geometry(const Op &o, int B, ConvArgs &a) const;
@@ -127,6 +129,7 @@
     void place_splitk_slabs();
     void plan_dwpw();
     void plan_workspace_tail();
+    void plan_sample_fused();
     void mark_shared_tensors();
 };
 
diff --git a/tdrn_amd/csrc/net_plan.hip b/tdrn_amd/csrc/net_plan.hip
--- a/tdrn_amd/csrc/net_plan.hip
+++ b/tdrn_amd/csrc/net_plan.hip
@@ -626,6 +626,44 @@
         pp_sk_planned = pp_sk_planned || pp_takes_geometry(a);
     }
     if (pp_sk_planned || !chain_ops.empty()) ws_fixed = kTailCtl + (pp_sk_planned ? align_up(conv_pp_sk_bytes(), 256) : 1024);
+}
+
+#ifndef TDRN_SAMPLE_PARTS
+#define TDRN_SAMPLE_PARTS (TDRN_SAMPLE_OFFSETS | TDRN_SAMPLE_SOFTMAX | TDRN_SAMPLE_LOADS8)
+#endif
+
+void Plan::plan_sample_fused()
+{
+    sample_fused = sample_softmax = false;
+    if (cfg.plan_flags & TDRN_PLAN_NO_SAMPLE_FUSED) return;
+    int first = -1, last = -1, n_deform = 0;
+    for (size_t i = 0; i < ops.size(); ++i)
+        if (ops[i].kind == OP_DEFORM) { if (first < 0) first = (int)i; last = (int)i; ++n_deform; }
+    if (first < 0 || last - first + 1 != n_deform || n_deform > 4) return;
+    for (int i = first; i <= last; ++i) {
+        const Op &d = ops[i];
+        if (d.y_t < 0 || d.y_groups != 1) return;
+        const int prod = producer_of(d.off_t);
+        if (prod < 0 || ops[prod].kind != OP_OFFSET || ops[prod].in >= 0 || ops[prod].scale != d.scale) return;
+        for (const Op &r : ops)
+            if (&r != &d && r.kind != OP_OFF_OUT && (r.in == d.off_t || r.res == d.off_t || r.off_t == d.off_t)) return;
+    }
+    sample_fused = true;
+    bool other_conf = false, levels[4] = {false, false, false, false};
+    for (const Op &o : ops) other_conf = other_conf || (o.kind == OP_CONV && o.out_kind == OUT_CONF);
+    for (int i = first; i <= last; ++i)
+        if (ops[i].scale >= 0 && ops[i].scale < 4) levels[ops[i].scale] = true;
+    sample_softmax = last + 2 == (int)ops.size() && ops[last + 1].kind == OP_SOFTMAX && !other_conf && levels[0] && levels[1] && levels[2] && levels[3] &&
+                     3 * cfg.num_classes <= 64;
+}
+
+int Plan::sample_form(const tdrn_net_io *io, int first_op) const
+{
+    if (!sample_fused || !io || first_op != 0) return 0;
+    if (io->reserved[0] || io->reserved[1]) return 0;
+    for (int i = 0; i < 4; ++i)
+        if (io->offsets[i] || io->ref_loc[i]) return 0;
+    return (TDRN_SAMPLE_OFFSETS | TDRN_SAMPLE_LOADS8 | (sample_softmax ? TDRN_SAMPLE_SOFTMAX : 0)) & TDRN_SAMPLE_PARTS;
 }
 
 void Plan::mark_shared_tensors()
@@ -684,6 +722,15 @@
     y_tap_major = true;
     for (const Op &d : ops)
         if (d.kind == OP_DEFORM && d.y_t >= 0 && !ygemm_supported(d.Cin, d.y_cols, cfg.dtype)) y_tap_major = false;
+    plan_sample_fused();
+    if (const char *pd = getenv("TDRN_PLAN_DUMP")) {
+        if (atoi(pd)) {
+            int launches = 0;
+            for (size_t i = 0; i < ops.size(); ++i) launches += launch_head(i) && !(sample_fused && ops[i].kind == OP_OFFSET) && !(sample_softmax && ops[i].kind == OP_SOFTMAX);
+            fprintf(stderr, "plan: deform heads: offsets in the sampling launch %d  softmax in the sampling launch %d  launches of a forward without offsets out %d\n",
+                    sample_fused ? 1 : 0, sample_softmax ? 1 : 0, launches);
+        }
+    }
     mark_shared_tensors();
     return TDRN_OK;
 }
diff --git a/tdrn_amd/csrc/net_run.hip b/tdrn_amd/csrc/net_run.hip
--- a/tdrn_amd/csrc/net_run.hip
+++ b/tdrn_amd/csrc/net_run.hip
@@ -11,6 +11,7 @@
     const tdrn_u8_frames *u8 = nullptr;
     const float *xin = nullptr;
     int B = 0, C = 0;
+    int form = 0;
     int Bk = 0;
     bool lanes = false, join_on = false, reuse_offsets = false;
     bool lane_used[kLanes] = {true, false, false, false};
@@ -150,6 +151,8 @@
         }
         if (reuse_offsets && n.offs_key_batch != Bk) return TDRN_E_STATE;
         if (p.cfg.deform && !reuse_offsets) { n.offs_ws = nullptr; n.offs_batch = 0; n.offs_key_batch = 0; }
+        form = p.sample_form(io, n.first_op);
+        n.last_form = form;
         return TDRN_OK;
     }
 
@@ -182,6 +185,11 @@
         if (o.kind == OP_FIRST && p.fuse_first >= 0) return true;
         if (o.kind == OP_CONV && o.chain > 0) return true;
         return (int)oi < n.first_op;
+    }
+
+    bool in_sample_launch(const Op &o) const
+    {
+        return (o.kind == OP_OFFSET && (form & TDRN_SAMPLE_OFFSETS)) || (o.kind == OP_SOFTMAX && (form & TDRN_SAMPLE_SOFTMAX));
     }
 
     int stream_for(const Op &o, int &lane, hipStream_t &s)
@@ -357,6 +365,15 @@
         a.out0 = loc_out(o) + (size_t)p.scale_off[o.scale] * 4; a.o0_bs = (long long)p.P * 4; a.o0_ps = 12;
         a.out1 = io->conf + (size_t)p.scale_off[o.scale] * C; a.o1_bs = (long long)p.P * C; a.o1_ps = 3 * C;
         a.split = 12; a.dtype = p.cfg.dtype;
+        if (form & TDRN_SAMPLE_OFFSETS) {
+            const Op &f = p.ops[p.producer_of(o.off_t)];
+            for (int k = 0; k < o.n_branches; ++k) {
+                a.br[k].loc = io->arm_loc + (size_t)p.scale_off[f.scale] * 4; a.br[k].loc_bs = (long long)p.P * 4; a.br[k].loc_ps = 12;
+                a.br[k].ow = (const float *)(wb + f.w_off) + (size_t)o.off_c0[k] * 12;
+                a.br[k].ob = (const float *)(wb + f.b_off) + o.off_c0[k];
+            }
+        }
+        if (form & TDRN_SAMPLE_SOFTMAX) a.softmax_C = C;
         dargs[n_dargs++] = a;
         if (o.y_t >= 0) ts_op[n_dargs - 1] = (int)oi;
         if (p.launch_continues(oi) && n_dargs < 4) return TDRN_OK;
@@ -407,6 +424,7 @@
             for (int k = 0; k < c.n_branches; ++k) {
                 if (c.br[k].off_rows) c.br[k].off_row0 = (int)(px0 % (size_t)c.br[k].off_rows);
                 else c.br[k].off += px0 * c.br[k].off_stride;
+                if (c.br[k].loc) c.br[k].loc += (size_t)b0 * c.br[k].loc_bs;
             }
             c.out0 += (size_t)b0 * c.o0_bs;
             c.out1 += (size_t)b0 * c.o1_bs;
@@ -431,7 +449,7 @@
             ts_y[i] = ybuf; ts_cs[i] = d.y_cols;
         }
         if (n_yq > 0) TDRN_TRY(launch_ygemm_multi(yq, n_yq, dtype, s, p.kdisable));
-        return launch_deform_sample_multi(ca, ts_y, ts_cs, n_dargs, s, p.y_tap_major ? 1 : 0);
+        return launch_deform_sample_multi(ca, ts_y, ts_cs, n_dargs, s, p.y_tap_major ? 1 : 0, (form & TDRN_SAMPLE_LOADS8) ? SAMPLE_LOADS8 : 0);
     }
 
     int run_deform_gather(const Op &o, hipStream_t s)
@@ -463,6 +481,7 @@
         int lane;
         hipStream_t s;
         TDRN_TRY(stream_for(o, lane, s));
+        if (in_sample_launch(o)) return record(o.out, s);
         if (n.profile && !launch_open(o)) TDRN_HIP_TRY(hipEventRecord(n.ev[evi], s));
         const Tensor *ti = o.in >= 0 ? &p.tensors[o.in] : nullptr;
         switch (o.kind) {
```

Result: no change. 12230 frames/s (median of 6 runs) (+0.1%).
